# Innoptech/OpenFDCM

Measured on NVIDIA B200. Metric: template_matches_per_sec, higher is better.
Workload: dtype f32

## Files before the change

### include/fdcm_b200.h

```cpp
#ifndef FDCM_B200_H
#define FDCM_B200_H

#include <stdint.h>

#ifdef __cplusplus
extern "C" {
#endif

#define FDCM_B200_ABI_VERSION 3

typedef enum fdcm_status {
    FDCM_OK = 0,
    FDCM_ERR_INVALID = 1,
    FDCM_ERR_CUDA = 2,
    FDCM_ERR_NOMEM = 3,
    FDCM_ERR_OUT_OF_RANGE = 4,
    FDCM_ERR_CAPACITY = 5
} fdcm_status;

typedef enum fdcm_distance { FDCM_L2 = 0, FDCM_L2_SQUARED = 1, FDCM_L1 = 2 } fdcm_distance;

typedef struct fdcm_dt3_params {
    int32_t depth;
    float dt3_coeff;
    float padding;
    int32_t distance;
} fdcm_dt3_params;

typedef struct fdcm_match {
    int32_t tmpl_idx;
    float score;
    float transform[6];
} fdcm_match;

typedef enum fdcm_penalty_kind { FDCM_PENALTY_NONE = 0, FDCM_PENALTY_DEFAULT = 1, FDCM_PENALTY_EXPONENTIAL = 2 } fdcm_penalty_kind;

typedef struct fdcm_search_params {
    int32_t max_tmpl_lines;
    int32_t max_scene_lines;
    int32_t batch_size;
    int32_t penalty_kind;
    float penalty_tau;
    int32_t top_k;
    int32_t tmpl_idx_base;
    int32_t concentric;
    float center_x, center_y, low_radius, high_radius;
} fdcm_search_params;

typedef struct fdcm_dt3_info {
    int32_t depth;
    int32_t width, height;
    int32_t pitch;
    float scene_translation[2];
    int32_t distance;
    int32_t device;
    int32_t n_scene_lines;
    int32_t exact_dt_path;
} fdcm_dt3_info;

typedef struct fdcm_search_stats {
    int64_t n_hypotheses;
    int64_t n_valid;
    int64_t n_evaluations;
    int64_t n_lookups;
} fdcm_search_stats;

typedef struct fdcm_dt3 fdcm_dt3;
typedef struct fdcm_templates fdcm_templates;
typedef struct fdcm_comm fdcm_comm;
typedef struct fdcm_scene_batch fdcm_scene_batch;

const char* fdcm_last_error(void);
int32_t fdcm_abi_version(void);
fdcm_status fdcm_device_count(int32_t* n);
fdcm_status fdcm_set_stream(int32_t device, void* cuda_stream);

fdcm_status fdcm_dt3_build(const float* scene_xyxy, int32_t n_lines, const fdcm_dt3_params* params, int32_t device,
                           int32_t stage, fdcm_dt3** out);
fdcm_status fdcm_dt3_rebuild(fdcm_dt3* map, const float* scene_xyxy, int32_t n_lines);
fdcm_status fdcm_dt3_rebuild_async(fdcm_dt3* map, const float* scene_xyxy, int32_t n_lines);
fdcm_status fdcm_dt3_rerun(fdcm_dt3* map);
fdcm_status fdcm_dt3_rerun_async(fdcm_dt3* map);
fdcm_status fdcm_dt3_retain(fdcm_dt3* map);
fdcm_status fdcm_dt3_release(fdcm_dt3* map);
fdcm_status fdcm_dt3_get_info(const fdcm_dt3* map, fdcm_dt3_info* info);
fdcm_status fdcm_dt3_angles(const fdcm_dt3* map, float* keys);
fdcm_status fdcm_dt3_download_plane(const fdcm_dt3* map, int32_t plane, float* dst);
fdcm_status fdcm_dt3_download_mask(const fdcm_dt3* map, int32_t plane, uint8_t* dst);
fdcm_status fdcm_dt3_scene_bins(const fdcm_dt3* map, int32_t* bins);
fdcm_status fdcm_dt3_device_ptr(const fdcm_dt3* map, void** planes, uint64_t* n_bytes);

fdcm_status fdcm_dt3_minmax_translation(const fdcm_dt3* map, const float* tmpl_xyxy, int32_t n_lines,
                                        const float align_vec[2], float out_min_max[2]);
fdcm_status fdcm_dt3_evaluate(const fdcm_dt3* map, const float* tmpl_lines, const int32_t* tmpl_offsets, int32_t n_tmpl,
                              const float* translations, const int32_t* transl_offsets, float* scores);
fdcm_status fdcm_dt3_classify(const fdcm_dt3* map, const float* lines_xyxy, int32_t n_lines, int32_t* bins);

fdcm_status fdcm_templates_create(const float* tmpl_lines, const int32_t* tmpl_offsets, int32_t n_tmpl, int32_t device,
                                  fdcm_templates** out);
fdcm_status fdcm_templates_release(fdcm_templates* t);
fdcm_status fdcm_templates_lengths(const fdcm_templates* t, float* lengths);

#define FDCM_SCENE_RESIDENT (-1)
fdcm_status fdcm_search(const fdcm_dt3* map, const fdcm_templates* templates, const float* scene_xyxy, int32_t n_scene,
                        const fdcm_search_params* params, fdcm_match* out, int64_t capacity, int64_t* n_out);
#define FDCM_SELECT_MAX_ACROSS 1024
typedef struct fdcm_select_params {
    int32_t max_per_template;
    float radius;
    float max_angle;
    int32_t across_templates;
} fdcm_select_params;
fdcm_status fdcm_search_select(const fdcm_dt3* map, const fdcm_templates* templates, const float* scene_xyxy, int32_t n_scene,
                               const fdcm_search_params* params, const fdcm_select_params* select,
                               fdcm_match* out, int64_t capacity, int64_t* n_out);
fdcm_status fdcm_template_anchors(const float* tmpl_lines, const int32_t* tmpl_offsets, int32_t n_tmpl, float* anchors_xy);

#define FDCM_REFINE_MAX_STEPS 15
typedef struct fdcm_refine_params {
    int32_t levels;
    int32_t rot_steps;
    float rot_step;
    int32_t trans_steps;
    float trans_step;
} fdcm_refine_params;
fdcm_status fdcm_refine_matches(const fdcm_dt3* map, const fdcm_templates* templates, int32_t tmpl_idx_base, int32_t penalty_kind,
                                float penalty_tau, const fdcm_refine_params* refine, const fdcm_match* in, int64_t n,
                                fdcm_match* out);
fdcm_status fdcm_search_refine(const fdcm_dt3* map, const fdcm_templates* templates, const float* scene_xyxy, int32_t n_scene,
                               const fdcm_search_params* params, const fdcm_select_params* select,
                               const fdcm_refine_params* refine, fdcm_match* out, int64_t capacity, int64_t* n_out);
fdcm_status fdcm_refine_poses(const float transform[6], const float anchor[2], const fdcm_refine_params* refine, int32_t level,
                              float* out);

#define FDCM_DENSE_MAX_ROTATIONS 4096
typedef struct fdcm_dense_params {
    int32_t rotations;
    float rot_start;
    float rot_step;
    int32_t stride;
    int32_t cell;
    int32_t roi_on;
    float roi[4];
} fdcm_dense_params;
fdcm_status fdcm_search_dense(const fdcm_dt3* map, const fdcm_templates* templates, const fdcm_dense_params* dense, int32_t penalty_kind,
                              float penalty_tau, int32_t top_k, int32_t tmpl_idx_base, const fdcm_select_params* select,
                              const fdcm_refine_params* refine, fdcm_match* out, int64_t capacity, int64_t* n_out);
fdcm_status fdcm_dense_poses(const fdcm_dense_params* dense, const float anchor[2], const float shift[2], int32_t width, int32_t height,
                             int32_t rotation, float* out, int64_t capacity, int64_t* n_out, int32_t grid_wh[2]);

fdcm_status fdcm_optimize(const fdcm_dt3* map, const float* tmpl_lines, const int32_t* tmpl_offsets, int32_t n_tmpl,
                          const float* alignments, int32_t batch_size, uint8_t* has_value, float* scores,
                          float* translations);
fdcm_status fdcm_search_host(const fdcm_dt3* map, const float* tmpl_lines, const int32_t* tmpl_offsets, int32_t n_tmpl,
                             const float* scene_xyxy, int32_t n_scene, const fdcm_search_params* params,
                             fdcm_match* out, int64_t capacity, int64_t* n_out);
fdcm_status fdcm_search_last_hypotheses(const fdcm_dt3* map, int32_t* out, int64_t capacity, int64_t* n_out);
fdcm_status fdcm_search_last_stats(const fdcm_dt3* map, fdcm_search_stats* stats);

fdcm_status fdcm_default_search(const float* tmpl_xyxy, int32_t n_tmpl_lines, const float* scene_xyxy, int32_t n_scene,
                                int32_t max_tmpl_lines, int32_t max_scene_lines, int32_t* out_pairs, int32_t capacity,
                                int32_t* n_out);

fdcm_status fdcm_concentric_search(const float* tmpl_xyxy, int32_t n_tmpl_lines, const float* scene_xyxy, int32_t n_scene,
                                   int32_t max_tmpl_lines, int32_t max_scene_lines, float center_x, float center_y,
                                   float low_radius, float high_radius, int32_t* out_pairs, int32_t capacity, int32_t* n_out);

fdcm_status fdcm_debug_dt_rows(const uint16_t* g_rows, int32_t n_rows, int32_t n, int32_t literal, int32_t device, float* out);

fdcm_status fdcm_debug_sqrt_check(int32_t device, int64_t* n_mismatches, uint32_t* first_mismatch);

fdcm_status fdcm_orientation_bins(int32_t depth, const float* lines_xyxy, int32_t n_lines, int32_t* bins_atanf,
                                  int32_t* bins_table);

fdcm_status fdcm_penalize(int32_t penalty_kind, float tau, fdcm_match* matches, int64_t n, const float* lengths,
                          int64_t n_lengths);
fdcm_status fdcm_sort_matches(fdcm_match* matches, int64_t n);
fdcm_status fdcm_template_lengths(const float* tmpl_lines, const int32_t* tmpl_offsets, int32_t n_tmpl, float* lengths);

fdcm_status fdcm_scene_batch_create(const fdcm_dt3_params* params, int32_t device, fdcm_scene_batch** out);
fdcm_status fdcm_scene_batch_destroy(fdcm_scene_batch* batch);
fdcm_status fdcm_search_scenes(fdcm_scene_batch* batch, const float* scene_lines, const int32_t* scene_offsets, int32_t n_scenes,
                               const fdcm_templates* templates, const fdcm_search_params* params, fdcm_match* out, int32_t* n_out);
fdcm_status fdcm_search_scenes_select(fdcm_scene_batch* batch, const float* scene_lines, const int32_t* scene_offsets, int32_t n_scenes,
                                      const fdcm_templates* templates, const fdcm_search_params* params,
                                      const fdcm_select_params* select, fdcm_match* out, int32_t* n_out);

#define FDCM_COMM_ID_BYTES 128
fdcm_status fdcm_comm_unique_id(uint8_t id[FDCM_COMM_ID_BYTES]);
fdcm_status fdcm_comm_init(const uint8_t id[FDCM_COMM_ID_BYTES], int32_t rank, int32_t world, int32_t device, fdcm_comm** out);
fdcm_status fdcm_comm_destroy(fdcm_comm* comm);
fdcm_status fdcm_comm_info(const fdcm_comm* comm, int32_t* rank, int32_t* world);
fdcm_status fdcm_comm_shard(int32_t n_items, int32_t rank, int32_t world, int32_t* begin, int32_t* end);
fdcm_status fdcm_comm_search_topk(fdcm_comm* comm, const fdcm_dt3* map, const fdcm_templates* shard, const float* scene_xyxy,
                                  int32_t n_scene, const fdcm_search_params* params, fdcm_match* out, int64_t capacity,
                                  int64_t* n_out);
fdcm_status fdcm_comm_search_select(fdcm_comm* comm, const fdcm_dt3* map, const fdcm_templates* shard, const float* scene_xyxy,
                                    int32_t n_scene, const fdcm_search_params* params, const fdcm_select_params* select,
                                    fdcm_match* out, int64_t capacity, int64_t* n_out);
fdcm_status fdcm_comm_search_host_topk(fdcm_comm* comm, const fdcm_dt3* map, const float* tmpl_lines, const int32_t* tmpl_offsets,
                                       int32_t n_tmpl, const float* scene_xyxy, int32_t n_scene, const fdcm_search_params* params,
                                       fdcm_match* out, int64_t capacity, int64_t* n_out);
fdcm_status fdcm_comm_rebuild_broadcast(fdcm_comm* comm, fdcm_dt3* map, const float* scene_xyxy, int32_t n_lines, int32_t root);
fdcm_status fdcm_set_host_threads(int32_t n);

fdcm_status fdcm_profile_enable(int32_t on);
fdcm_status fdcm_profile_reset(void);
fdcm_status fdcm_profile_get(int32_t index, char* name, int32_t name_cap, double* total_ms, int64_t* launches,
                             double* bytes_per_launch);
fdcm_status fdcm_profile_count(int32_t* n);
int64_t fdcm_kernel_launch_count(void);

#ifdef __cplusplus
}
#endif
#endif
```

### openfdcm_b200/__init__.py

```python
import ctypes as C
import enum
import math

import numpy as np

from . import _lib
from .io import read, write
from ._lib import MATCH_DTYPE, FdcmError, check, lib, ptr

__all__ = [
    "distance", "Dt3CudaParameters", "Dt3Cuda", "build_cuda_featuremap", "ThreadPool", "DefaultSearch", "ConcentricRangeStrategy",
    "BatchOptimize", "DefaultOptimize", "DefaultMatch", "DefaultPenalty", "ExponentialPenalty", "Match",
    "TemplateSet", "SceneBatch", "DistinctMatches", "PoseRefinement", "DenseSearch", "search", "search_topk", "search_dense",
    "refine_matches", "penalize", "get_template_lengths",
    "get_template_anchors", "sort_matches", "evaluate",
    "minmax_translation", "get_feature_size", "establish_search_strategy", "optimize", "read", "write", "FdcmError", "MATCH_DTYPE",
]


class distance(enum.IntEnum):
    L2 = 0
    L2_SQUARED = 1
    L1 = 2


def _records(lines):
    a = np.asarray(lines, dtype=np.float32)
    if a.size == 0:
        return np.zeros((0, 4), np.float32)
    if a.ndim == 1 and a.size == 4:
        a = a.reshape(4, 1)
    if a.ndim != 2 or a.shape[0] != 4:
        raise ValueError(f"expected a (4,N) line array, got shape {a.shape}")
    return np.ascontiguousarray(a.T)


def _pack(templates):
    recs = [_records(t) for t in templates]
    off = np.zeros(len(recs) + 1, np.int32)
    for i, r in enumerate(recs):
        off[i + 1] = off[i] + r.shape[0]
    flat = np.concatenate(recs, axis=0) if recs else np.zeros((0, 4), np.float32)
    return np.ascontiguousarray(flat, np.float32), off


class Dt3CudaParameters:

    def __init__(self, depth=30, dt3Coeff=5.0, padding=2.2, distance=distance.L2, device=0):
        self.depth = int(depth)
        self.dt3_coeff = float(dt3Coeff)
        self.padding = float(padding)
        self.distance = distance
        self.device = int(device)

    def __repr__(self):
        return f"<Dt3CudaParameters: depth={self.depth}, dt3_coeff={self.dt3_coeff}, padding={self.padding}>"


class Dt3Cuda:

    def __init__(self, handle):
        self._h = C.c_void_p(handle)
        self._refresh()

    def _refresh(self):
        info = _lib.Dt3Info()
        check(lib().fdcm_dt3_get_info(self._h, C.byref(info)))
        self.info = info
        self.depth, self.width, self.height, self.pitch = info.depth, info.width, info.height, info.pitch
        self.device = info.device

    def __del__(self):
        h, self._h = getattr(self, "_h", None), None
        if h and lib is not None:
            lib().fdcm_dt3_release(h)

    def __copy__(self):
        check(lib().fdcm_dt3_retain(self._h))
        return Dt3Cuda(self._h.value)

    def get_scene_translation(self):
        return np.array(self.info.scene_translation[:], np.float32)

    def get_feature_size(self):
        return np.array([self.width, self.height], np.uint64)

    def angles(self):
        k = np.zeros(self.depth, np.float32)
        if self.depth:
            check(lib().fdcm_dt3_angles(self._h, ptr(k)))
        return k

    def plane(self, i):
        out = np.zeros((self.height, self.width), np.float32)
        check(lib().fdcm_dt3_download_plane(self._h, int(i), ptr(out)))
        return out

    def mask(self, i):
        out = np.zeros((self.height, self.width), np.uint8)
        check(lib().fdcm_dt3_download_mask(self._h, int(i), ptr(out)))
        return out

    def scene_bins(self):
        b = np.zeros(self.info.n_scene_lines, np.int32)
        if b.size:
            check(lib().fdcm_dt3_scene_bins(self._h, ptr(b)))
        return b

    def classify(self, lines):
        r = _records(lines)
        b = np.zeros(r.shape[0], np.int32)
        check(lib().fdcm_dt3_classify(self._h, ptr(r), r.shape[0], ptr(b)))
        return b

    def get_dt3_map(self):
        return {float(a): self.plane(i) for i, a in enumerate(self.angles())}

    def device_ptr(self):
        p, n = C.c_void_p(0), C.c_uint64(0)
        check(lib().fdcm_dt3_device_ptr(self._h, C.byref(p), C.byref(n)))
        return p.value, n.value

    def rebuild(self, scene, wait=True):
        r = _records(scene)
        check((lib().fdcm_dt3_rebuild if wait else lib().fdcm_dt3_rebuild_async)(self._h, ptr(r), r.shape[0]))
        self._refresh()

    def rerun(self, wait=True):
        check((lib().fdcm_dt3_rerun if wait else lib().fdcm_dt3_rerun_async)(self._h))

    def last_search_stats(self):
        st = _lib.SearchStats()
        check(lib().fdcm_search_last_stats(self._h, C.byref(st)))
        return {"n_hypotheses": st.n_hypotheses, "n_valid": st.n_valid, "n_evaluations": st.n_evaluations,
                "n_lookups": st.n_lookups}

    def last_hypotheses(self):
        n = C.c_int64(0)
        lib().fdcm_search_last_hypotheses(self._h, None, 0, C.byref(n))
        out = np.zeros((n.value, 4), np.int32)
        if n.value:
            check(lib().fdcm_search_last_hypotheses(self._h, ptr(out), n.value, C.byref(n)))
        return out

    def __repr__(self):
        t = self.info.scene_translation
        return f"<Dt3Cuda: scene translation=({t[0]}, {t[1]}), feature size=({self.width}, {self.height})>"


def build_cuda_featuremap(scene, params=None, pool=None, *, stage=0):
    params = params or Dt3CudaParameters()
    p = _lib.Dt3Params(params.depth, params.dt3_coeff, params.padding, int(params.distance))
    r = _records(scene)
    h = C.c_void_p(0)
    check(lib().fdcm_dt3_build(ptr(r), r.shape[0], C.byref(p), params.device, int(stage), C.byref(h)))
    return Dt3Cuda(h.value)


class ThreadPool:

    def __init__(self, num_threads=0):
        self.num_threads = int(num_threads)

    def get_thread_count(self):
        return self.num_threads


class DefaultSearch:

    def __init__(self, max_tmpl_lines, max_scene_lines):
        self.max_tmpl_lines, self.max_scene_lines = int(max_tmpl_lines), int(max_scene_lines)

    def get_max_tmpl_lines(self):
        return self.max_tmpl_lines

    def get_max_scene_lines(self):
        return self.max_scene_lines


class ConcentricRangeStrategy(DefaultSearch):

    def __init__(self, max_tmpl_lines, max_scene_lines, center_position, low_boundary, high_boundary):
        super().__init__(max_tmpl_lines, max_scene_lines)
        c = np.asarray(center_position, np.float32).reshape(2)
        self.center_position = c
        self.low_boundary, self.high_boundary = float(low_boundary), float(high_boundary)

    def get_center_position(self):
        return self.center_position

    def get_low_radius_boundary(self):
        return self.low_boundary

    def get_high_radius_boundary(self):
        return self.high_boundary


class BatchOptimize:

    def __init__(self, batch_size, pool=None, num_threads=None):
        if int(batch_size) < 1:
            raise ValueError("batch_size must be >= 1")
        self.batch_size = int(batch_size)

    def get_batch_size(self):
        return self.batch_size


class DefaultOptimize:
    batch_size = 0

    def __init__(self, pool=None, num_threads=None):
        pass


class DefaultMatch:
    """matchstrategies/defaultmatch.h."""


class DefaultPenalty:
    kind, tau = 1, 0.0


class ExponentialPenalty:
    kind = 2

    def __init__(self, tau):
        self.tau = float(tau)

    def get_tau(self):
        return self.tau


class Match:
    __slots__ = ("tmpl_idx", "score", "transform")

    def __init__(self, tmpl_idx, score, transform):
        self.tmpl_idx = int(tmpl_idx)
        self.score = float(score)
        self.transform = np.asarray(transform, np.float32).reshape(2, 3)

    def __repr__(self):
        return f"<Match tmplIdx={self.tmpl_idx}, score={self.score}, transform=\n{self.transform}>"


def _to_matches(rec):
    return [Match(r["tmpl_idx"], r["score"], r["transform"]) for r in rec]


def _to_records(matches):
    if isinstance(matches, np.ndarray) and matches.dtype == MATCH_DTYPE:
        return np.ascontiguousarray(matches).copy()
    rec = np.zeros(len(matches), MATCH_DTYPE)
    for i, m in enumerate(matches):
        rec[i] = (m.tmpl_idx, m.score, np.asarray(m.transform, np.float32).reshape(6))
    return rec


class TemplateSet:

    def __init__(self, templates, device=0):
        flat, off = _pack(templates)
        self.n_tmpl = len(off) - 1
        self.n_lines = int(off[-1])
        self.max_lines = int(np.diff(off).max()) if self.n_tmpl else 0
        h = C.c_void_p(0)
        check(lib().fdcm_templates_create(ptr(flat), ptr(off), self.n_tmpl, int(device), C.byref(h)))
        self._h = h
        self.device = int(device)

    def __del__(self):
        h, self._h = getattr(self, "_h", None), None
        if h and lib is not None:
            lib().fdcm_templates_release(h)
# ... 276 lines not shown
```

### openfdcm_b200/_lib.py

```python
import ctypes as C
import os

import numpy as np

_HERE = os.path.dirname(os.path.abspath(__file__))
LIB_PATH = os.path.join(_HERE, "libfdcm_b200.so")

FDCM_OK = 0
FDCM_ERR_INVALID, FDCM_ERR_CUDA, FDCM_ERR_NOMEM, FDCM_ERR_OUT_OF_RANGE, FDCM_ERR_CAPACITY = 1, 2, 3, 4, 5
FDCM_SCENE_RESIDENT = -1

MATCH_DTYPE = np.dtype([("tmpl_idx", "<i4"), ("score", "<f4"), ("transform", "<f4", (6,))])
assert MATCH_DTYPE.itemsize == 32


class Dt3Params(C.Structure):
    _fields_ = [("depth", C.c_int32), ("dt3_coeff", C.c_float), ("padding", C.c_float), ("distance", C.c_int32)]


class SearchParams(C.Structure):
    _fields_ = [("max_tmpl_lines", C.c_int32), ("max_scene_lines", C.c_int32), ("batch_size", C.c_int32),
                ("penalty_kind", C.c_int32), ("penalty_tau", C.c_float), ("top_k", C.c_int32),
                ("tmpl_idx_base", C.c_int32), ("concentric", C.c_int32), ("center_x", C.c_float), ("center_y", C.c_float),
                ("low_radius", C.c_float), ("high_radius", C.c_float)]


class SelectParams(C.Structure):
    _fields_ = [("max_per_template", C.c_int32), ("radius", C.c_float), ("max_angle", C.c_float), ("across_templates", C.c_int32)]


class RefineParams(C.Structure):
    _fields_ = [("levels", C.c_int32), ("rot_steps", C.c_int32), ("rot_step", C.c_float), ("trans_steps", C.c_int32),
                ("trans_step", C.c_float)]


class DenseParams(C.Structure):
    _fields_ = [("rotations", C.c_int32), ("rot_start", C.c_float), ("rot_step", C.c_float), ("stride", C.c_int32), ("cell", C.c_int32),
                ("roi_on", C.c_int32), ("roi", C.c_float * 4)]


class Dt3Info(C.Structure):
    _fields_ = [("depth", C.c_int32), ("width", C.c_int32), ("height", C.c_int32), ("pitch", C.c_int32),
                ("scene_translation", C.c_float * 2), ("distance", C.c_int32), ("device", C.c_int32),
                ("n_scene_lines", C.c_int32), ("exact_dt_path", C.c_int32)]


class SearchStats(C.Structure):
    _fields_ = [("n_hypotheses", C.c_int64), ("n_valid", C.c_int64), ("n_evaluations", C.c_int64),
                ("n_lookups", C.c_int64)]


_P = C.c_void_p
SIGNATURES = {
    "fdcm_last_error": (C.c_char_p, []),
    "fdcm_abi_version": (C.c_int32, []),
    "fdcm_device_count": (C.c_int, [C.POINTER(C.c_int32)]),
    "fdcm_set_stream": (C.c_int, [C.c_int32, _P]),
    "fdcm_dt3_build": (C.c_int, [_P, C.c_int32, C.POINTER(Dt3Params), C.c_int32, C.c_int32, C.POINTER(_P)]),
    "fdcm_dt3_rebuild": (C.c_int, [_P, _P, C.c_int32]),
    "fdcm_dt3_rebuild_async": (C.c_int, [_P, _P, C.c_int32]),
    "fdcm_dt3_rerun": (C.c_int, [_P]),
    "fdcm_dt3_rerun_async": (C.c_int, [_P]),
    "fdcm_dt3_retain": (C.c_int, [_P]),
    "fdcm_dt3_release": (C.c_int, [_P]),
    "fdcm_dt3_get_info": (C.c_int, [_P, C.POINTER(Dt3Info)]),
    "fdcm_dt3_angles": (C.c_int, [_P, _P]),
    "fdcm_dt3_download_plane": (C.c_int, [_P, C.c_int32, _P]),
    "fdcm_dt3_download_mask": (C.c_int, [_P, C.c_int32, _P]),
    "fdcm_dt3_scene_bins": (C.c_int, [_P, _P]),
    "fdcm_dt3_device_ptr": (C.c_int, [_P, C.POINTER(_P), C.POINTER(C.c_uint64)]),
    "fdcm_dt3_minmax_translation": (C.c_int, [_P, _P, C.c_int32, _P, _P]),
    "fdcm_dt3_evaluate": (C.c_int, [_P, _P, _P, C.c_int32, _P, _P, _P]),
    "fdcm_dt3_classify": (C.c_int, [_P, _P, C.c_int32, _P]),
    "fdcm_templates_create": (C.c_int, [_P, _P, C.c_int32, C.c_int32, C.POINTER(_P)]),
    "fdcm_templates_release": (C.c_int, [_P]),
    "fdcm_templates_lengths": (C.c_int, [_P, _P]),
    "fdcm_search": (C.c_int, [_P, _P, _P, C.c_int32, C.POINTER(SearchParams), _P, C.c_int64, C.POINTER(C.c_int64)]),
    "fdcm_search_select": (C.c_int, [_P, _P, _P, C.c_int32, C.POINTER(SearchParams), C.POINTER(SelectParams), _P, C.c_int64,
                                     C.POINTER(C.c_int64)]),
    "fdcm_template_anchors": (C.c_int, [_P, _P, C.c_int32, _P]),
    "fdcm_refine_matches": (C.c_int, [_P, _P, C.c_int32, C.c_int32, C.c_float, C.POINTER(RefineParams), _P, C.c_int64, _P]),
    "fdcm_search_refine": (C.c_int, [_P, _P, _P, C.c_int32, C.POINTER(SearchParams), C.POINTER(SelectParams), C.POINTER(RefineParams), _P,
                                     C.c_int64, C.POINTER(C.c_int64)]),
    "fdcm_refine_poses": (C.c_int, [_P, _P, C.POINTER(RefineParams), C.c_int32, _P]),
    "fdcm_search_dense": (C.c_int, [_P, _P, C.POINTER(DenseParams), C.c_int32, C.c_float, C.c_int32, C.c_int32, C.POINTER(SelectParams),
                                    C.POINTER(RefineParams), _P, C.c_int64, C.POINTER(C.c_int64)]),
    "fdcm_dense_poses": (C.c_int, [C.POINTER(DenseParams), _P, _P, C.c_int32, C.c_int32, C.c_int32, _P, C.c_int64, C.POINTER(C.c_int64),
                                   _P]),
    "fdcm_optimize": (C.c_int, [_P, _P, _P, C.c_int32, _P, C.c_int32, _P, _P, _P]),
    "fdcm_search_host": (C.c_int, [_P, _P, _P, C.c_int32, _P, C.c_int32, C.POINTER(SearchParams), _P, C.c_int64,
                                   C.POINTER(C.c_int64)]),
    "fdcm_search_last_hypotheses": (C.c_int, [_P, _P, C.c_int64, C.POINTER(C.c_int64)]),
    "fdcm_search_last_stats": (C.c_int, [_P, C.POINTER(SearchStats)]),
    "fdcm_default_search": (C.c_int, [_P, C.c_int32, _P, C.c_int32, C.c_int32, C.c_int32, _P, C.c_int32,
                                      C.POINTER(C.c_int32)]),
    "fdcm_debug_dt_rows": (C.c_int, [_P, C.c_int32, C.c_int32, C.c_int32, C.c_int32, _P]),
    "fdcm_debug_sqrt_check": (C.c_int, [C.c_int32, C.POINTER(C.c_int64), C.POINTER(C.c_uint32)]),
    "fdcm_concentric_search": (C.c_int, [_P, C.c_int32, _P, C.c_int32, C.c_int32, C.c_int32, C.c_float, C.c_float, C.c_float,
                                         C.c_float, _P, C.c_int32, C.POINTER(C.c_int32)]),
    "fdcm_orientation_bins": (C.c_int, [C.c_int32, _P, C.c_int32, _P, _P]),
    "fdcm_penalize": (C.c_int, [C.c_int32, C.c_float, _P, C.c_int64, _P, C.c_int64]),
    "fdcm_sort_matches": (C.c_int, [_P, C.c_int64]),
    "fdcm_template_lengths": (C.c_int, [_P, _P, C.c_int32, _P]),
    "fdcm_profile_enable": (C.c_int, [C.c_int32]),
    "fdcm_profile_reset": (C.c_int, []),
    "fdcm_profile_get": (C.c_int, [C.c_int32, C.c_char_p, C.c_int32, C.POINTER(C.c_double), C.POINTER(C.c_int64),
                                   C.POINTER(C.c_double)]),
    "fdcm_profile_count": (C.c_int, [C.POINTER(C.c_int32)]),
    "fdcm_kernel_launch_count": (C.c_int64, []),
    "fdcm_comm_unique_id": (C.c_int, [_P]),
    "fdcm_comm_init": (C.c_int, [_P, C.c_int32, C.c_int32, C.c_int32, C.POINTER(_P)]),
    "fdcm_comm_destroy": (C.c_int, [_P]),
    "fdcm_comm_info": (C.c_int, [_P, C.POINTER(C.c_int32), C.POINTER(C.c_int32)]),
    "fdcm_comm_shard": (C.c_int, [C.c_int32, C.c_int32, C.c_int32, C.POINTER(C.c_int32), C.POINTER(C.c_int32)]),
    "fdcm_comm_search_topk": (C.c_int, [_P, _P, _P, _P, C.c_int32, C.POINTER(SearchParams), _P, C.c_int64, C.POINTER(C.c_int64)]),
    "fdcm_comm_search_select": (C.c_int, [_P, _P, _P, _P, C.c_int32, C.POINTER(SearchParams), C.POINTER(SelectParams), _P, C.c_int64,
                                          C.POINTER(C.c_int64)]),
    "fdcm_comm_search_host_topk": (C.c_int, [_P, _P, _P, _P, C.c_int32, _P, C.c_int32, C.POINTER(SearchParams), _P, C.c_int64,
                                             C.POINTER(C.c_int64)]),
    "fdcm_comm_rebuild_broadcast": (C.c_int, [_P, _P, _P, C.c_int32, C.c_int32]),
    "fdcm_set_host_threads": (C.c_int, [C.c_int32]),
    "fdcm_scene_batch_create": (C.c_int, [C.POINTER(Dt3Params), C.c_int32, C.POINTER(_P)]),
    "fdcm_scene_batch_destroy": (C.c_int, [_P]),
    "fdcm_search_scenes": (C.c_int, [_P, _P, _P, C.c_int32, _P, C.POINTER(SearchParams), _P, _P]),
    "fdcm_search_scenes_select": (C.c_int, [_P, _P, _P, C.c_int32, _P, C.POINTER(SearchParams), C.POINTER(SelectParams), _P, _P]),
}


class FdcmError(RuntimeError):
    def __init__(self, status, message):
        super().__init__(f"libfdcm_b200 status {status}: {message}")
        self.status = status


_lib = None


def lib():
    global _lib
    if _lib is None:
        if not os.path.exists(LIB_PATH):
            raise ImportError(f"{LIB_PATH} is missing: build it with `make -C openfdcm_b200/csrc` "
                              "(or __graft_entry__.build()); there is no CPU fallback")
        l = C.CDLL(LIB_PATH)
        for name, (res, args) in SIGNATURES.items():
            fn = getattr(l, name)
            fn.restype = res
            fn.argtypes = args
        _lib = l
    return _lib


def check(status):
    if status != FDCM_OK:
        msg = lib().fdcm_last_error()
        raise FdcmError(status, msg.decode() if msg else "")


def ptr(a):
    return a.ctypes.data_as(C.c_void_p) if a is not None else None
```

### openfdcm_b200/csrc/common.cuh

```cuda
#pragma once
#include <cuda_runtime.h>
#include <cfloat>
#include <cstdint>

namespace fdcm {

constexpr int kMaxDepthDev = 64;
constexpr int kMaxPropSteps = 4 * kMaxDepthDev;
constexpr uint16_t kNoEdge16 = 0xFFFFu;

struct MapDims {
    int D, H, W, pitch;
    int wwords;
    size_t plane_elems;
};

struct PropParams {
    int n_steps;
    float w[kMaxPropSteps];
    uint8_t c1[kMaxPropSteps];
    uint8_t c2[kMaxPropSteps];
};

struct IntegralParams {
    float rx[kMaxDepthDev], ry[kMaxDepthDev];
    int mode[kMaxDepthDev];
};

struct SlopeTableDev {
    int n_thr;
    int nan_bin;
    float thr[kMaxDepthDev + 8];
    uint8_t piece_bin[kMaxDepthDev + 9];
};

__device__ __forceinline__ long long round_to_ll(float x) { return (long long)roundf(x); }

__device__ __forceinline__ float signed_pick_dev(float x, bool negate) { return x == 0.f ? 0.f : (negate ? -x : x); }

__device__ __forceinline__ void rasterize_vector_dev(float vx, float vy, float& ox, float& oy) {
    const float t = vy / vx;
    if (t >= -1.0f && t < 1.0f) {
        const bool c = vx < 0;
        ox = c ? -1.f : 1.f;
        oy = signed_pick_dev(t, c);
        return;
    }
    const bool c = vy < 0;
    const float inv = 1.f / t;
    ox = signed_pick_dev(inv, c);
    oy = c ? -1.f : 1.f;
}

__device__ __forceinline__ int bin_of_slope_dev(const SlopeTableDev& t, float slope) {
    if (slope != slope) return t.nan_bin;
    int lo = 0, hi = t.n_thr;
    while (lo < hi) {
        const int mid = (lo + hi) >> 1;
        if (t.thr[mid] <= slope) lo = mid + 1; else hi = mid;
    }
    return t.piece_bin[lo];
}

}
```

### openfdcm_b200/csrc/dt3_kernels.cu

```cuda
#include <cstdlib>

#include "common.cuh"
#include "kernels.h"

namespace fdcm {

__device__ __forceinline__ int outcode_dev(float x, float y, float xmax, float ymax) {
    int code = 0;
    if (x < 0.f) code |= 1; else if (x > xmax) code |= 2;
    if (y < 0.f) code |= 4; else if (y > ymax) code |= 8;
    return code;
}

__device__ bool clip_line_dev(float& x1, float& y1, float& x2, float& y2, float xmax, float ymax) {
    int c1 = outcode_dev(x1, y1, xmax, ymax);
    int c2 = outcode_dev(x2, y2, xmax, ymax);
    for (int it = 0; it < 16; ++it) {
        if (c1 == 0 && c2 == 0) return true;
        if (c1 & c2) return false;
        if (c1 != 0) {
            if (c1 & 8)      { x1 = x1 + (x2 - x1) * (ymax - y1) / (y2 - y1); y1 = ymax; }
            else if (c1 & 4) { x1 = x1 + (x2 - x1) * (0.f - y1) / (y2 - y1); y1 = 0.f; }
            else if (c1 & 2) { y1 = y1 + (y2 - y1) * (xmax - x1) / (x2 - x1); x1 = xmax; }
            else if (c1 & 1) { y1 = y1 + (y2 - y1) * (0.f - x1) / (x2 - x1); x1 = 0.f; }
// ... 51 lines not shown
    if (rel_eq_zero(rx)) {
        const int size = (int)(lvy / ry) + 1;
        const LinSpacedDev ly(size, p1y, p2y);
        const long long x = round_to_ll(p1x);
        for (int i = lane; i < size; i += 32) set_edge(mask, dm, plane, x, round_to_ll(ly.at(i)));
        return;
    }
    if (rel_eq_zero(ry)) {
        const int size = (int)(lvx / rx) + 1;
        const LinSpacedDev lx(size, p1x, p2x);
        const long long y = round_to_ll(p1y);
        for (int i = lane; i < size; i += 32) set_edge(mask, dm, plane, round_to_ll(lx.at(i)), y);
        return;
    }
    const float a = lvx / rx, b = lvy / ry;
    const int size = (int)((a < b) ? b : a) + 1;
    const LinSpacedDev lx(size, p1x, p2x), ly(size, p1y, p2y);
    for (int i = lane; i < size; i += 32) set_edge(mask, dm, plane, round_to_ll(lx.at(i)), round_to_ll(ly.at(i)));
}


struct EnvEntry { int v; float z; };
enum { kSrcPlane = 0, kSrcMask = 1, kSrcG16 = 2 };

template <int kSrc>
__global__ void __launch_bounds__(128) dt_pass_literal_kernel(const void* __restrict__ src, float* planes, MapDims dm,
                                                              EnvEntry* stack, int n, int n_lines, size_t elem_stride,
                                                              size_t line_stride) {
    const int l = blockIdx.x * blockDim.x + threadIdx.x;
    const int d = blockIdx.y;
    if (l >= n_lines) return;
    const size_t base = (size_t)d * dm.plane_elems + (size_t)l * line_stride;
    float* out = planes + base;
    const uint16_t* gin = kSrc == kSrcG16 ? reinterpret_cast<const uint16_t*>(src) + base : nullptr;
    const uint32_t* mrow = kSrc == kSrcMask ? reinterpret_cast<const uint32_t*>(src) + (size_t)d * dm.H * dm.wwords + (l >> 5) : nullptr;
    const uint32_t mbit = 1u << (l & 31);
    EnvEntry* st = stack + base;
    auto F = [&](int q) -> float {
        if (kSrc == kSrcG16) {
            const unsigned gv = gin[(size_t)q * elem_stride];
            return gv == kNoEdge16 ? FLT_MAX : (float)(gv * gv);
        }
        if (kSrc == kSrcMask) return (mrow[(size_t)q * dm.wwords] & mbit) ? 0.f : FLT_MAX;
        return out[(size_t)q * elem_stride];
    };
    int k = 0, vk = 0;
    float fvk = F(0), zk = -INFINITY;
    st[0] = EnvEntry{0, -INFINITY};
    for (int q = 1; q < n; ++q) {
        const float fq = F(q);
        const float sqq = (float)((long long)q * q);
        while (true) {
            const float s = (fq + sqq - fvk - (float)((long long)vk * vk)) / (float)(2LL * q - 2LL * vk);
            if (s > zk) {
                ++k;
                st[(size_t)k * elem_stride] = EnvEntry{q, s};
                vk = q; fvk = fq; zk = s;
                break;
            }
            --k;
            const EnvEntry e = st[(size_t)k * elem_stride];
            vk = e.v; zk = e.z; fvk = F(vk);
        }
    }
    int k2 = 0, v = 0;
    float znext = (k >= 1) ? st[elem_stride].z : INFINITY;
    for (int q = 0; q < n; ++q) {
        while (znext < (float)q) {
            ++k2;
            v = st[(size_t)k2 * elem_stride].v;
            znext = (k2 + 1 <= k) ? st[(size_t)(k2 + 1) * elem_stride].z : INFINITY;
        }
        const long long dq = (long long)q - v;
        const float srcv = (kSrc != kSrcPlane && v >= q) ? F(v) : out[(size_t)v * elem_stride];
        out[(size_t)q * elem_stride] = srcv + (float)(dq * dq);
    }
}

__global__ void __launch_bounds__(256) transpose_square_kernel(float* __restrict__ planes, MapDims dm, int ntiles) {
    __shared__ float A[32][33], B[32][33];
    int t = blockIdx.x, ti = 0;
    while (t >= ntiles - ti) { t -= ntiles - ti; ++ti; }
    const int tj = ti + t;
    float* P = planes + (size_t)blockIdx.y * dm.plane_elems;
    const int lx = threadIdx.x & 31, ly = threadIdx.x >> 5;
    const int n = dm.W;
    for (int r = ly; r < 32; r += 8) {
        const int ya = ti * 32 + r, xa = tj * 32 + lx;
        const int yb = tj * 32 + r, xb = ti * 32 + lx;
        A[r][lx] = (ya < n && xa < n) ? P[(size_t)ya * dm.pitch + xa] : 0.f;
        B[r][lx] = (yb < n && xb < n) ? P[(size_t)yb * dm.pitch + xb] : 0.f;
    }
    __syncthreads();
    for (int r = ly; r < 32; r += 8) {
        const int ya = ti * 32 + r, xa = tj * 32 + lx;
        const int yb = tj * 32 + r, xb = ti * 32 + lx;
        if (ya < n && xa < n) P[(size_t)ya * dm.pitch + xa] = B[lx][r];
        if (ti != tj && yb < n && xb < n) P[(size_t)yb * dm.pitch + xb] = A[lx][r];
    }
}

__global__ void __launch_bounds__(256) sqrt_kernel(float* __restrict__ planes, size_t total) {
    const size_t i = (size_t)blockIdx.x * blockDim.x + threadIdx.x;
    if (i < total) planes[i] = sqrtf(planes[i]);
}

template <int D>
__global__ void __launch_bounds__(128) propagate_kernel(float* __restrict__ planes, MapDims dm,
                                                        const __grid_constant__ PropParams pp, int sqrt_first) {
    const size_t i = (size_t)blockIdx.x * blockDim.x + threadIdx.x;
    if (i >= dm.plane_elems || (int)(i % dm.pitch) >= dm.W) return;
    float v[D];
#pragma unroll
    for (int d = 0; d < D; ++d) v[d] = planes[(size_t)d * dm.plane_elems + i];
    if (sqrt_first) {
#pragma unroll
        for (int d = 0; d < D; ++d) v[d] = sqrtf(v[d]);
    }
    constexpr int fwd = (3 * D + 1) / 2;
    constexpr int bwd = D + (3 * D) / 2;
#pragma unroll
    for (int c = 0; c < fwd; ++c) {
        const int c1 = (D + ((c - 1) % D)) % D;
        const int c2 = c % D;
        v[c2] = fminf(v[c2], v[c1] + pp.w[c]);
    }
#pragma unroll
    for (int j = 0; j < bwd; ++j) {
        const int c = D - j;
        const int c1 = (D + ((c + 1) % D)) % D;
        const int c2 = (D + (c % D)) % D;
        v[c2] = fminf(v[c2], v[c1] + pp.w[fwd + j]);
    }
#pragma unroll
    for (int d = 0; d < D; ++d) planes[(size_t)d * dm.plane_elems + i] = v[d];
}

__global__ void __launch_bounds__(128) propagate_generic_kernel(float* __restrict__ planes, MapDims dm,
                                                                const __grid_constant__ PropParams pp, int sqrt_first) {
    const size_t i = (size_t)blockIdx.x * blockDim.x + threadIdx.x;
    if (i >= dm.plane_elems || (int)(i % dm.pitch) >= dm.W) return;
    float v[kMaxDepthDev];
    for (int d = 0; d < dm.D; ++d) {
        const float x = planes[(size_t)d * dm.plane_elems + i];
        v[d] = sqrt_first ? sqrtf(x) : x;
    }
    for (int s = 0; s < pp.n_steps; ++s) {
        const int c1 = pp.c1[s], c2 = pp.c2[s];
        v[c2] = fminf(v[c2], v[c1] + pp.w[s]);
    }
    for (int d = 0; d < dm.D; ++d) planes[(size_t)d * dm.plane_elems + i] = v[d];
}

static inline unsigned cdiv(size_t a, size_t b) { return (unsigned)((a + b - 1) / b); }

void launch_raster(const float* d_lines, const int32_t* d_bins, int n_lines, const MapDims& dm, uint32_t* d_mask,
                   cudaStream_t s) {
    if (n_lines <= 0) return;
    raster_kernel<<<cdiv((size_t)n_lines * 32, 256), 256, 0, s>>>(reinterpret_cast<const float4*>(d_lines), d_bins, n_lines,
                                                                   dm, d_mask);
}

void launch_dt_pass_literal(int src_kind, bool along_rows, const void* d_src, float* d_planes, const MapDims& dm, void* d_stack,
                            cudaStream_t s) {
    const int n = along_rows ? dm.W : dm.H;
    const int n_lines = along_rows ? dm.H : dm.W;
    const size_t es = along_rows ? 1 : (size_t)dm.pitch;
    const size_t ls = along_rows ? (size_t)dm.pitch : 1;
    dim3 grid(cdiv(n_lines, 128), dm.D);
    if (src_kind == kSrcG16)
        dt_pass_literal_kernel<kSrcG16><<<grid, 128, 0, s>>>(d_src, d_planes, dm, (EnvEntry*)d_stack, n, n_lines, es, ls);
    else if (src_kind == kSrcMask)
        dt_pass_literal_kernel<kSrcMask><<<grid, 128, 0, s>>>(d_src, d_planes, dm, (EnvEntry*)d_stack, n, n_lines, es, ls);
    else
        dt_pass_literal_kernel<kSrcPlane><<<grid, 128, 0, s>>>(d_src, d_planes, dm, (EnvEntry*)d_stack, n, n_lines, es, ls);
}

void launch_transpose_square(float* d_planes, const MapDims& dm, cudaStream_t s) {
    const int nt = (dm.W + 31) / 32;
    dim3 grid((unsigned)((size_t)nt * (nt + 1) / 2), dm.D);
    transpose_square_kernel<<<grid, 256, 0, s>>>(d_planes, dm, nt);
}

void launch_sqrt(float* d_planes, const MapDims& dm, cudaStream_t s) {
    const size_t total = (size_t)dm.D * dm.plane_elems;
    sqrt_kernel<<<cdiv(total, 256), 256, 0, s>>>(d_planes, total);
}

void launch_propagate(float* d_planes, const MapDims& dm, const PropParams& pp, bool sqrt_first, cudaStream_t s) {
    const unsigned grid = cdiv(dm.plane_elems, 128);
    switch (dm.D) {
        case 30: propagate_kernel<30><<<grid, 128, 0, s>>>(d_planes, dm, pp, sqrt_first ? 1 : 0); break;
        case 4: propagate_kernel<4><<<grid, 128, 0, s>>>(d_planes, dm, pp, sqrt_first ? 1 : 0); break;
        default: propagate_generic_kernel<<<grid, 128, 0, s>>>(d_planes, dm, pp, sqrt_first ? 1 : 0); break;
    }
}

}
```

### openfdcm_b200/csrc/fdcm_api.cu

```cuda
#include <algorithm>
#include <atomic>
#include <condition_variable>
#include <functional>
#include <cmath>
#include <cstdio>
#include <cstdlib>
#include <cstring>
#include <map>
#include <mutex>
#include <string>
#include <thread>
#include <vector>

#include "host_math.hpp"
#include "kernels.h"

using namespace fdcm;

static thread_local std::string g_last_error;

static fdcm_status fail(fdcm_status st, const std::string& msg) {
    g_last_error = msg;
    return st;
}
// ... 63 lines not shown
        CUDA_TRY(cudaStreamCreateWithPriority(&ns, cudaStreamNonBlocking, prio_hi));
        o = g_aux_streams.emplace(device, ns).first;
    }
    *s = o->second;
    return FDCM_OK;
}

extern "C" fdcm_status fdcm_set_stream(int32_t device, void* cuda_stream) {
    std::lock_guard<std::mutex> lk(g_mutex);
    if (cuda_stream) g_user_streams[device] = (cudaStream_t)cuda_stream;
    else g_user_streams.erase(device);
    return FDCM_OK;
}

struct ProfEntry { double total_ms = 0; long long launches = 0; double bytes = 0; };
struct ProfPending { const char* name; cudaEvent_t a, b; double bytes; int device; };
static bool g_prof_on = false;
static std::vector<std::string> g_prof_order;
static std::map<std::string, ProfEntry> g_prof;
static std::vector<ProfPending> g_prof_pending;
static std::map<int, std::vector<cudaEvent_t>> g_prof_events;
static cudaEvent_t prof_event_get(int device) {
    auto& pool = g_prof_events[device];
    cudaEvent_t e = nullptr;
    if (!pool.empty()) {
        e = pool.back();
        pool.pop_back();
    } else {
        cudaEventCreate(&e);
    }
    return e;
}
static void prof_event_put(int device, cudaEvent_t e) { g_prof_events[device].push_back(e); }

struct KernelScope {
    cudaStream_t s;
    bool on;
    ProfPending p;
    KernelScope(const char* name, double bytes, cudaStream_t stream, int n_kernels = 1) : s(stream), on(g_prof_on) {
        g_launches.fetch_add(n_kernels, std::memory_order_relaxed);
        if (on) {
            p.name = name;
            p.bytes = bytes;
            p.device = 0;
            cudaGetDevice(&p.device);
            {
                std::lock_guard<std::mutex> lk(g_mutex);
                p.a = prof_event_get(p.device);
                p.b = prof_event_get(p.device);
            }
            cudaEventRecord(p.a, s);
        }
    }
    ~KernelScope() {
        if (on) {
            cudaEventRecord(p.b, s);
            std::lock_guard<std::mutex> lk(g_mutex);
            g_prof_pending.push_back(p);
        }
    }
};

extern "C" fdcm_status fdcm_profile_enable(int32_t on) { g_prof_on = on != 0; return FDCM_OK; }
extern "C" fdcm_status fdcm_profile_reset(void) {
    std::lock_guard<std::mutex> lk(g_mutex);
    g_prof.clear();
    g_prof_order.clear();
    return FDCM_OK;
}
static void prof_resolve() {
    std::lock_guard<std::mutex> lk(g_mutex);
    std::vector<ProfPending> keep;
    bool not_ready = false;
    for (auto& p : g_prof_pending) {
        if (cudaEventQuery(p.b) != cudaSuccess) { keep.push_back(p); not_ready = true; continue; }
        float ms = 0.f;
        if (cudaEventElapsedTime(&ms, p.a, p.b) == cudaSuccess) {
            if (!g_prof.count(p.name)) g_prof_order.push_back(p.name);
            auto& e = g_prof[p.name];
            e.total_ms += ms;
            e.launches += 1;
            e.bytes = p.bytes;
        }
        prof_event_put(p.device, p.a);
        prof_event_put(p.device, p.b);
    }
    g_prof_pending.swap(keep);
    if (not_ready && cudaPeekAtLastError() == cudaErrorNotReady) cudaGetLastError();
}

extern "C" fdcm_status fdcm_profile_count(int32_t* n) {
    if (!n) return fail(FDCM_ERR_INVALID, "n is null");
    prof_resolve();
    std::lock_guard<std::mutex> lk(g_mutex);
    *n = (int32_t)g_prof_order.size();
    return FDCM_OK;
}
extern "C" fdcm_status fdcm_profile_get(int32_t index, char* name, int32_t name_cap, double* total_ms, int64_t* launches,
                                        double* bytes_per_launch) {
    std::lock_guard<std::mutex> lk(g_mutex);
    if (index < 0 || index >= (int32_t)g_prof_order.size()) return fail(FDCM_ERR_INVALID, "profile index out of range");
    const std::string& nm = g_prof_order[index];
    const ProfEntry& e = g_prof[nm];
    if (name && name_cap > 0) {
        std::strncpy(name, nm.c_str(), name_cap - 1);
        name[name_cap - 1] = 0;
    }
    if (total_ms) *total_ms = e.total_ms;
    if (launches) *launches = e.launches;
    if (bytes_per_launch) *bytes_per_launch = e.bytes;
    return FDCM_OK;
}
extern "C" int64_t fdcm_kernel_launch_count(void) { return g_launches.load(); }

struct DevBuf {
    void* p = nullptr;
    size_t cap = 0;
    cudaError_t reserve(size_t bytes) {
        if (bytes <= cap) return cudaSuccess;
        if (p) cudaFree(p);
        p = nullptr;
        cap = 0;
        cudaError_t e = cudaMalloc(&p, bytes);
        if (e == cudaSuccess) cap = bytes;
        return e;
    }
    void release() {
        if (p) cudaFree(p);
        p = nullptr;
        cap = 0;
    }
    template <class T> T* as() const { return reinterpret_cast<T*>(p); }
};

struct fdcm_dt3 {
    std::atomic<int> refs{1};
    fdcm_dt3_params params{};
    int device = 0;
    int stage = 0;
    MapDims dm{};
    float shift[2] = {0.f, 0.f};
    bool exact = true;
    int col_lo = 0, col_hi = 0;
    int row_lo = 0, row_hi = 0;
    int tables_depth = -1;
    float tables_coeff = 0.f;
    int n_lines = 0;
    std::vector<float> keys;
    std::vector<int32_t> scene_bins;
    SlopeTable table;
    SlopeTableDev table_dev{};
    PropParams prop{};
    IntegralParams integ{};
    DevBuf planes, mask, stack, lines, bins, band_info, band_spill, integ_items;
    IntegralPlanDev integ_plan{};
    int plan_W = -1, plan_H = -1, plan_D = -1, plan_pitch = -1;
    const void* plan_planes = nullptr;
    int plan_tables_depth = -1;
    int n_sms = 148;
    cudaEvent_t ev_fork = nullptr, ev_join = nullptr;
    cudaEvent_t ev_written = nullptr;
    bool band_path = false, band_l1 = false;
    mutable std::mutex search_mutex;
    mutable DevBuf s_scene, s_sorted_len, s_sorted_idx, s_hyp_off, s_rec, s_valid, s_hyp, s_counters, s_topk_score, s_topk_idx,
        s_topk_out, s_topk_n, s_keys, s_keys2, s_idx, s_perm, s_sort_tmp;
    mutable DevBuf s_sel_keys, s_sel_keys2, s_sel_vals, s_sel_vals2, s_sel_surv, s_sel_acc, s_sel_tmp;
    mutable DevBuf s_ref_state, s_ref_keys, s_ref_io;
    mutable DevBuf s_denom;
    mutable uint64_t denom_set = 0;
    mutable int denom_kind = -1;
    mutable float denom_tau = 0.f;
    mutable DevBuf s_dense_keys, s_dense_rot;
    mutable float s_scene_min[2] = {0.f, 0.f}, s_scene_max[2] = {0.f, 0.f};
    mutable std::mutex host_tset_mutex;
    mutable fdcm_templates* host_tset = nullptr;
    mutable int32_t s_scene_n = 0;
    mutable int32_t s_sorted_n = 0;
    mutable bool s_resident_is_build = false;
    mutable bool s_filter_on = false;
    mutable float s_filter[4] = {0.f, 0.f, 0.f, 0.f};
    std::vector<float> h_build_scene;
    mutable int64_t last_n_hyp = 0;
    mutable fdcm_search_stats last_stats{};
    mutable void* h_scene_stage = nullptr;
    mutable size_t h_scene_stage_cap = 0;
    mutable cudaEvent_t scene_stage_ev = nullptr;
    mutable void* h_pinned = nullptr;
    mutable size_t h_pinned_cap = 0;

    ~fdcm_dt3() {
        cudaSetDevice(device);
        for (DevBuf* b : {&planes, &mask, &stack, &lines, &bins, &band_info, &band_spill, &integ_items, &s_scene, &s_sorted_len, &s_sorted_idx, &s_hyp_off, &s_rec,
                          &s_valid, &s_hyp, &s_counters, &s_topk_score, &s_topk_idx, &s_topk_out, &s_topk_n, &s_keys, &s_keys2, &s_idx,
                          &s_perm, &s_sort_tmp, &s_sel_keys, &s_sel_keys2, &s_sel_vals, &s_sel_vals2, &s_sel_surv, &s_sel_acc,
                          &s_sel_tmp, &s_ref_state, &s_ref_keys, &s_ref_io, &s_denom, &s_dense_keys, &s_dense_rot})
            b->release();
        if (h_pinned) cudaFreeHost(h_pinned);
        if (ev_fork) cudaEventDestroy(ev_fork);
        if (ev_join) cudaEventDestroy(ev_join);
        if (ev_written) cudaEventDestroy(ev_written);
        if (h_scene_stage) cudaFreeHost(h_scene_stage);
        if (scene_stage_ev) cudaEventDestroy(scene_stage_ev);
        destroy_host_tset();
    }
    void destroy_host_tset();
};

constexpr int64_t kMaxSide = 16384;

struct SceneFilter { bool on; float cx, cy, lo, hi; };

static fdcm_status map_wait(const fdcm_dt3* m, cudaStream_t s) {
    if (m->ev_written) CUDA_TRY(cudaStreamWaitEvent(s, m->ev_written, 0));
    return FDCM_OK;
}
static fdcm_status map_written(fdcm_dt3* m, cudaStream_t s) {
    if (!m->ev_written) CUDA_TRY(cudaEventCreateWithFlags(&m->ev_written, cudaEventDisableTiming));
    CUDA_TRY(cudaEventRecord(m->ev_written, s));
    return FDCM_OK;
}

static std::vector<int32_t> filter_in_range(const float* lines, int32_t n, const SceneFilter& f) {
    std::vector<int32_t> idx;
    for (int32_t i = 0; i < n; ++i) {
        const float* l = lines + 4 * (size_t)i;
        const float mx = (l[2] + l[0]) / 2 - f.cx, my = (l[3] + l[1]) / 2 - f.cy;
        const float rad = std::sqrt(mx * mx + my * my);
        if (rad > (f.lo - std::numeric_limits<float>::epsilon()) && rad < f.hi) idx.push_back(i);
    }
    return idx;
}

static fdcm_status upload_search_scene(const fdcm_dt3* m, const float* scene, int32_t n_scene, const SceneFilter& flt, cudaStream_t s) {
    std::vector<int32_t> subset;
    if (flt.on) subset = filter_in_range(scene, n_scene, flt);
    else {
        subset.resize((size_t)n_scene);
        for (int i = 0; i < n_scene; ++i) subset[(size_t)i] = i;
    }
    const int ns = (int)subset.size();
    std::vector<float> slen((size_t)ns);
    for (int i = 0; i < ns; ++i) slen[(size_t)i] = line_length(scene + 4 * (size_t)subset[(size_t)i]);
    const std::vector<long> sidx = argsort_desc(slen.data(), ns);
    std::vector<float> sorted_len((size_t)ns);
    std::vector<int32_t> sorted_idx((size_t)ns);
    for (int i = 0; i < ns; ++i) {
        sorted_len[(size_t)i] = slen[(size_t)sidx[(size_t)i]];
        sorted_idx[(size_t)i] = subset[(size_t)sidx[(size_t)i]];
    }
    m->s_scene_n = 0;
    m->s_sorted_n = 0;
    m->s_scene_min[0] = m->s_scene_max[0] = scene[0];
    m->s_scene_min[1] = m->s_scene_max[1] = scene[1];
    for (int64_t i = 0; i < 2 * (int64_t)n_scene; ++i)
        for (int a = 0; a < 2; ++a) {
            const float v = scene[2 * i + a];
            if (v < m->s_scene_min[a]) m->s_scene_min[a] = v;
            if (v > m->s_scene_max[a]) m->s_scene_max[a] = v;
        }
    CUDA_TRY(m->s_scene.reserve((size_t)n_scene * 16));
    CUDA_TRY(m->s_sorted_len.reserve(std::max<size_t>(4, (size_t)ns * 4)));
    CUDA_TRY(m->s_sorted_idx.reserve(std::max<size_t>(4, (size_t)ns * 4)));
    const size_t need = (size_t)n_scene * 16 + (size_t)ns * 8;
    if (!m->scene_stage_ev) CUDA_TRY(cudaEventCreateWithFlags(&m->scene_stage_ev, cudaEventDisableTiming));
    else CUDA_TRY(cudaEventSynchronize(m->scene_stage_ev));
    if (m->h_scene_stage_cap < need) {
        if (m->h_scene_stage) cudaFreeHost(m->h_scene_stage);
        m->h_scene_stage = nullptr;
        m->h_scene_stage_cap = 0;
        CUDA_TRY(cudaMallocHost(&m->h_scene_stage, need));
        m->h_scene_stage_cap = need;
    }
    unsigned char* st = static_cast<unsigned char*>(m->h_scene_stage);
    std::memcpy(st, scene, (size_t)n_scene * 16);
    CUDA_TRY(cudaMemcpyAsync(m->s_scene.p, st, (size_t)n_scene * 16, cudaMemcpyHostToDevice, s));
    if (ns) {
        std::memcpy(st + (size_t)n_scene * 16, sorted_len.data(), (size_t)ns * 4);
        std::memcpy(st + (size_t)n_scene * 16 + (size_t)ns * 4, sorted_idx.data(), (size_t)ns * 4);
        CUDA_TRY(cudaMemcpyAsync(m->s_sorted_len.p, st + (size_t)n_scene * 16, (size_t)ns * 4, cudaMemcpyHostToDevice, s));
        CUDA_TRY(cudaMemcpyAsync(m->s_sorted_idx.p, st + (size_t)n_scene * 16 + (size_t)ns * 4, (size_t)ns * 4, cudaMemcpyHostToDevice, s));
    }
    CUDA_TRY(cudaEventRecord(m->scene_stage_ev, s));
    m->s_scene_n = n_scene;
    m->s_sorted_n = ns;
    m->s_filter_on = flt.on;
    m->s_filter[0] = flt.cx; m->s_filter[1] = flt.cy; m->s_filter[2] = flt.lo; m->s_filter[3] = flt.hi;
    return FDCM_OK;
}

static fdcm_status run_build_kernels(fdcm_dt3* m, cudaStream_t s);

namespace fdcm {
bool encode_planes_map(CUtensorMap* out, const void* planes, int W, int H, int D, int pitch, int bx, int by, int bz) {
    typedef CUresult (*EncodeFn)(CUtensorMap*, CUtensorMapDataType, cuuint32_t, void*, const cuuint64_t*, const cuuint64_t*,
                                 const cuuint32_t*, const cuuint32_t*, CUtensorMapInterleave, CUtensorMapSwizzle,
                                 CUtensorMapL2promotion, CUtensorMapFloatOOBfill);
    static EncodeFn fn = [] {
        void* p = nullptr;
        cudaDriverEntryPointQueryResult q;
        if (cudaGetDriverEntryPoint("cuTensorMapEncodeTiled", &p, cudaEnableDefault, &q) != cudaSuccess || q != cudaDriverEntryPointSuccess)
            p = nullptr;
        return (EncodeFn)p;
    }();
    if (!fn) return false;
    const cuuint64_t dims[3] = {(cuuint64_t)W, (cuuint64_t)H, (cuuint64_t)D};
    const cuuint64_t strides[2] = {(cuuint64_t)pitch * 4, (cuuint64_t)pitch * 4 * (cuuint64_t)H};
    const cuuint32_t box[3] = {(cuuint32_t)bx, (cuuint32_t)by, (cuuint32_t)bz};
    const cuuint32_t estr[3] = {1, 1, 1};
    return fn(out, CU_TENSOR_MAP_DATA_TYPE_FLOAT32, 3, const_cast<void*>(planes), dims, strides, box, estr, CU_TENSOR_MAP_INTERLEAVE_NONE,
              CU_TENSOR_MAP_SWIZZLE_NONE, CU_TENSOR_MAP_L2_PROMOTION_L2_128B, CU_TENSOR_MAP_FLOAT_OOB_FILL_NONE) == CUDA_SUCCESS;
}
}

static fdcm_status build_integral_plan(fdcm_dt3* m, cudaStream_t s) {
    const MapDims& dm = m->dm;
    const bool same = m->plan_W == dm.W && m->plan_H == dm.H && m->plan_D == dm.D && m->plan_pitch == dm.pitch &&
                      m->plan_planes == m->planes.p && m->plan_tables_depth == m->tables_depth;
    if (same) return FDCM_OK;
    m->plan_W = -1;
    const int rlen = std::max(dm.W, dm.H);
    std::vector<int32_t> rtab((size_t)dm.D * rlen);
    struct Item { int work; int4 it; };
    std::vector<Item> items;
    const int CW = integral_strip_chains(), RB = integral_tile_steps();
    for (int d = 0; d < dm.D; ++d) {
        const int mode = m->integ.mode[d];
        const float r = mode == 1 ? m->integ.ry[d] : m->integ.rx[d];
        int32_t* R = rtab.data() + (size_t)d * rlen;
        for (int i = 0; i < rlen; ++i) R[i] = (int32_t)(long long)std::round((float)i * r);
        if (mode != 1 && mode != 2) continue;
        const int n_major = mode == 1 ? dm.W : dm.H, n_minor = mode == 1 ? dm.H : dm.W;
        const int Rend = R[n_major - 1];
        const int cmin = Rend > 0 ? -Rend : 0, cmax = (Rend < 0 ? -Rend : 0) + n_minor - 1;
        const int nblk = (n_major + RB - 1) / RB;
        for (int c0 = cmin; c0 <= cmax; c0 += CW) {
            int b_lo = nblk, b_hi = 0;
            for (int b = 0; b < nblk; ++b) {
                const int i0 = b * RB, i1 = std::min(n_major, i0 + RB);
                const int rlo = std::min(R[i0], R[i1 - 1]), rhi = std::max(R[i0], R[i1 - 1]);
                if (c0 + CW - 1 + rhi >= 0 && c0 + rlo <= n_minor - 1) { b_lo = std::min(b_lo, b); b_hi = std::max(b_hi, b + 1); }
            }
            if (b_lo < b_hi) items.push_back(Item{b_hi - b_lo, make_int4(d, c0, b_lo, b_hi)});
        }
    }
    std::stable_sort(items.begin(), items.end(), [](const Item& a, const Item& b) { return a.work > b.work; });
    std::vector<int4> flat(items.size());
    for (size_t i = 0; i < items.size(); ++i) flat[i] = items[i].it;
    CUDA_TRY(m->integ_items.reserve(std::max<size_t>(16, flat.size() * sizeof(int4))));
    if (!flat.empty()) CUDA_TRY(cudaMemcpyAsync(m->integ_items.p, flat.data(), flat.size() * sizeof(int4), cudaMemcpyHostToDevice, s));
    CUDA_TRY(cudaStreamSynchronize(s));
    IntegralPlanDev& pl = m->integ_plan;
    pl.items4 = m->integ_items.as<int4>();
    pl.n_items = (int)flat.size();
    if (!integral_tma_encode(m->planes.p, dm, &pl.map_y, &pl.map_x))
        return fail(FDCM_ERR_CUDA, "cuTensorMapEncodeTiled failed for the feature-map planes");
    int sms = 0;
    if (cudaDeviceGetAttribute(&sms, cudaDevAttrMultiProcessorCount, m->device) == cudaSuccess && sms > 0) m->n_sms = sms;
    m->plan_W = dm.W; m->plan_H = dm.H; m->plan_D = dm.D; m->plan_pitch = dm.pitch;
    m->plan_planes = m->planes.p;
    m->plan_tables_depth = m->tables_depth;
    return FDCM_OK;
}

static fdcm_status prepare_and_upload(fdcm_dt3* m, const float* scene, int32_t n_lines, cudaStream_t s) {
    m->n_lines = n_lines;
    m->scene_bins.clear();
    if (n_lines == 0) {
        m->s_scene_n = 0;
        m->s_sorted_n = 0;
        m->h_build_scene.clear();
        m->dm = MapDims{0, 0, 0, 0, 0, 0};
        m->shift[0] = m->shift[1] = 0.f;
        m->keys.clear();
        return FDCM_OK;
    }
    int64_t size[2];
    scene_centered_translation(scene, n_lines, m->params.padding, m->shift, size);
    if (size[0] <= 0 || size[0] > kMaxSide || size[1] != size[0])
        return fail(FDCM_ERR_INVALID, "feature size out of the supported range (1.." + std::to_string(kMaxSide) + "): " + std::to_string(size[0]));
    m->keys = angle_keys(m->params.depth);
    const int D = (int)m->keys.size();
    MapDims dm;
    dm.D = D;
    dm.W = (int)size[0];
    dm.H = (int)size[1];
    dm.pitch = (dm.W + 31) / 32 * 32;
    dm.wwords = dm.pitch / 32;
    dm.plane_elems = (size_t)dm.H * dm.pitch;
    m->dm = dm;
    m->exact = 2.0 * (double)(dm.W - 1) * (double)(dm.W - 1) < 16777216.0;

    std::vector<float> ts((size_t)4 * n_lines);
    m->scene_bins.resize(n_lines);
    for (int64_t i = 0; i < 2 * (int64_t)n_lines; ++i) {
        ts[2 * i] = scene[2 * i] + m->shift[0];
        ts[2 * i + 1] = scene[2 * i + 1] + m->shift[1];
    }
    for (int i = 0; i < n_lines; ++i) m->scene_bins[i] = bin_of_line(m->keys.data(), D, &ts[4 * (size_t)i]);
    {
        float mnx = ts[0], mxx = ts[0], mny = ts[1], mxy = ts[1];
        for (int64_t i = 0; i < 2 * (int64_t)n_lines; ++i) {
            mnx = std::min(mnx, ts[2 * i]);
            mxx = std::max(mxx, ts[2 * i]);
            mny = std::min(mny, ts[2 * i + 1]);
            mxy = std::max(mxy, ts[2 * i + 1]);
        }
        {
            const double lo = std::floor((double)mny) - 1.0, hi = std::ceil((double)mxy) + 1.0;
            m->row_lo = (lo < 0.0 || !(lo == lo)) ? 0 : (lo > dm.H - 1 ? dm.H - 1 : (int)lo);
            m->row_hi = (!(hi == hi) || hi > dm.H - 1) ? dm.H - 1 : (hi < 0.0 ? 0 : (int)hi);
        }
        const double lo = std::floor((double)mnx) - 1.0, hi = std::ceil((double)mxx) + 1.0;
        m->col_lo = (lo < 0.0 || !(lo == lo)) ? 0 : (lo > dm.W - 1 ? dm.W - 1 : (int)lo);
        m->col_hi = (!(hi == hi) || hi > dm.W - 1) ? dm.W - 1 : (hi < 0.0 ? 0 : (int)hi);
    }

    if (m->tables_depth != D || m->tables_coeff != m->params.dt3_coeff) {
    m->table = build_slope_table(m->keys.data(), D);
    if ((int)m->table.thr.size() > kMaxDepthDev + 8) return fail(FDCM_ERR_INVALID, "slope table too large");
    m->table_dev.n_thr = (int)m->table.thr.size();
    m->table_dev.nan_bin = m->table.nan_bin;
    for (size_t i = 0; i < m->table.thr.size(); ++i) m->table_dev.thr[i] = m->table.thr[i];
    for (size_t i = 0; i < m->table.piece_bin.size(); ++i) m->table_dev.piece_bin[i] = (uint8_t)m->table.piece_bin[i];
    const std::vector<PropStep> steps = propagation_schedule(m->keys, m->params.dt3_coeff);
    m->prop.n_steps = (int)steps.size();
    for (size_t i = 0; i < steps.size(); ++i) {
        m->prop.w[i] = steps[i].w;
        m->prop.c1[i] = (uint8_t)steps[i].c1;
        m->prop.c2[i] = (uint8_t)steps[i].c2;
    }
    for (int d = 0; d < D; ++d) {
        const IntegralDir id = integral_direction(m->keys[d]);
        m->integ.rx[d] = id.rx;
        m->integ.ry[d] = id.ry;
        m->integ.mode[d] = id.mode;
    }
    m->tables_depth = D;
    m->tables_coeff = m->params.dt3_coeff;
    }

    const size_t n_px = (size_t)D * dm.plane_elems;
    CUDA_TRY(m->planes.reserve(n_px * sizeof(float)));
    CUDA_TRY(m->mask.reserve((size_t)D * dm.H * dm.wwords * sizeof(uint32_t) + 256));
    if (dt_band_smem_bytes(dm) > 200 * 1024) return fail(FDCM_ERR_INVALID, "feature size too large for the band kernels");
    const bool band_path = m->exact && m->params.distance != FDCM_L1;
    const bool band_l1 = m->params.distance == FDCM_L1;
    m->band_path = band_path;
    m->band_l1 = band_l1;
    if (band_path || band_l1) CUDA_TRY(m->band_info.reserve(dt_band_info_bytes(dm)));
    if (band_path) CUDA_TRY(m->band_spill.reserve(dt_band_spill_bytes(dm, m->col_hi - m->col_lo + 1)));
    if (m->params.distance != FDCM_L1 && !band_path) CUDA_TRY(m->stack.reserve(n_px * 8));
    CUDA_TRY(m->lines.reserve((size_t)n_lines * 16));
    CUDA_TRY(m->bins.reserve((size_t)n_lines * 4));
    CUDA_TRY(cudaMemcpyAsync(m->lines.p, ts.data(), (size_t)n_lines * 16, cudaMemcpyHostToDevice, s));
    CUDA_TRY(cudaMemcpyAsync(m->bins.p, m->scene_bins.data(), (size_t)n_lines * 4, cudaMemcpyHostToDevice, s));
    return build_integral_plan(m, s);
}

static fdcm_status upload_build_scene(fdcm_dt3* m, const float* scene, int32_t n_lines, cudaStream_t s) {
    if (n_lines == 0) return FDCM_OK;
    m->h_build_scene.assign(scene, scene + 4 * (size_t)n_lines);
    m->s_resident_is_build = true;
    return upload_search_scene(m, scene, n_lines, SceneFilter{false, 0, 0, 0, 0}, s);
}

static fdcm_status run_build_kernels(fdcm_dt3* m, cudaStream_t s) {
    if (m->n_lines == 0) return FDCM_OK;
    const MapDims& dm = m->dm;
    const double N = (double)dm.D * dm.H * dm.W * 4.0;
    const size_t mask_bytes = (size_t)dm.D * dm.H * dm.wwords * sizeof(uint32_t);
    {
        KernelScope k("mask_clear", (double)mask_bytes, s, 0);
        CUDA_TRY(cudaMemsetAsync(m->mask.p, 0, mask_bytes + 256, s));
    }
    {
        KernelScope k("raster", 0.0, s);
        launch_raster(m->lines.as<float>(), m->bins.as<int32_t>(), m->n_lines, dm, m->mask.as<uint32_t>(), s);
    }
    const int dist = m->params.distance;
    bool fused_propagate = false;
    if (m->band_l1) {
        {
            KernelScope k("dt_col_band", (double)mask_bytes + (double)dt_band_info_bytes(dm), s);
            launch_dt_col_band(m->mask.as<uint32_t>(), dm, m->band_info.p, s);
        }
        fused_propagate = m->stage != 1 && dt_fill_propagate_supported(dm);
        if (fused_propagate) {
            KernelScope k("dt_l1_propagate", (double)dt_band_info_bytes(dm) + N, s);
            launch_dt_l1_propagate(m->band_info.p, m->planes.as<float>(), dm, m->prop, s);
        } else {
            KernelScope k("dt_row_l1_band", (double)dt_band_info_bytes(dm) + N, s);
            launch_dt_row_l1_band(m->band_info.p, m->planes.as<float>(), dm, s);
        }
    } else if (m->band_path) {
        {
            KernelScope k("dt_col_band", (double)mask_bytes + (double)dt_band_info_bytes(dm), s);
            launch_dt_col_band(m->mask.as<uint32_t>(), dm, m->band_info.p, s);
        }
        fused_propagate = m->stage != 1 && dt_fill_propagate_supported(dm);
        int ys0 = 0, ys1 = dm.H;
        dt_band_scene_rows(dm, m->row_lo, m->row_hi, &ys0, &ys1);
        const bool split = fused_propagate && (ys0 > 0 || ys1 < dm.H) && ys1 > ys0;
        if (split) {
            cudaStream_t sa;
            if (fdcm_status st = get_aux_stream(m->device, &sa)) return st;
            if (!m->ev_fork) CUDA_TRY(cudaEventCreateWithFlags(&m->ev_fork, cudaEventDisableTiming));
            if (!m->ev_join) CUDA_TRY(cudaEventCreateWithFlags(&m->ev_join, cudaEventDisableTiming));
            CUDA_TRY(cudaEventRecord(m->ev_fork, s));
            CUDA_TRY(cudaStreamWaitEvent(sa, m->ev_fork, 0));
            {
                KernelScope k("dt_row_envelope", (double)dt_band_info_bytes(dm), sa);
                launch_dt_row_envelope(m->band_info.p, nullptr, dm, m->band_spill.p, m->col_lo, m->col_hi, m->row_lo, m->row_hi, 1, sa);
            }
            {
                KernelScope k("dt_resolve", 2.0 * (double)dt_band_info_bytes(dm), sa);
                launch_dt_resolve(dm, m->band_spill.p, m->col_lo, m->col_hi, ys0, ys1, 0, 0, sa);
            }
            {
                KernelScope k("dt_fill_propagate", N * (double)(ys1 - ys0) / dm.H, sa);
                launch_dt_fill_propagate(m->planes.as<float>(), dm, m->band_spill.p, m->col_lo, m->col_hi, m->prop, dist == FDCM_L2, ys0, ys1, 0,
                                         0, sa);
            }
            CUDA_TRY(cudaEventRecord(m->ev_join, sa));
            {
                KernelScope k("dt_row_envelope_far", (double)dt_band_info_bytes(dm), s);
                launch_dt_row_envelope(m->band_info.p, nullptr, dm, m->band_spill.p, m->col_lo, m->col_hi, m->row_lo, m->row_hi, 2, s);
            }
            {
                KernelScope k("dt_resolve_far", 2.0 * (double)dt_band_info_bytes(dm), s);
                launch_dt_resolve(dm, m->band_spill.p, m->col_lo, m->col_hi, 0, ys0, ys1, dm.H, s);
            }
            {
                KernelScope k("dt_fill_propagate_far", N * (double)(dm.H - (ys1 - ys0)) / dm.H, s);
                launch_dt_fill_propagate(m->planes.as<float>(), dm, m->band_spill.p, m->col_lo, m->col_hi, m->prop, dist == FDCM_L2, 0, ys0, ys1,
                                         dm.H, s);
            }
            CUDA_TRY(cudaStreamWaitEvent(s, m->ev_join, 0));
        } else {
            {
                KernelScope k("dt_row_envelope", (double)dt_band_info_bytes(dm), s);
                launch_dt_row_envelope(m->band_info.p, nullptr, dm, m->band_spill.p, m->col_lo, m->col_hi, m->row_lo, m->row_hi, 0, s);
            }
            if (fused_propagate) {
                {
                    KernelScope k("dt_resolve", 2.0 * (double)dt_band_info_bytes(dm), s);
                    launch_dt_resolve(dm, m->band_spill.p, m->col_lo, m->col_hi, 0, dm.H, 0, 0, s);
                }
                KernelScope k("dt_fill_propagate", N, s);
                launch_dt_fill_propagate(m->planes.as<float>(), dm, m->band_spill.p, m->col_lo, m->col_hi, m->prop, dist == FDCM_L2, 0, dm.H, 0, 0,
                                         s);
            } else {
                KernelScope k("dt_row_fill", N, s);
                launch_dt_row_fill(m->planes.as<float>(), dm, m->band_spill.p, m->col_lo, m->col_hi, s);
            }
        }
    } else {
        {
            KernelScope k("dt_col_literal", (double)mask_bytes + N, s);
            launch_dt_pass_literal(1, false, m->mask.p, m->planes.as<float>(), dm, m->stack.p, s);
        }
        {
            KernelScope k("transpose", 2 * N, s);
            launch_transpose_square(m->planes.as<float>(), dm, s);
        }
        {
            KernelScope k("dt_row_literal", 2 * N, s);
            launch_dt_pass_literal(0, false, nullptr, m->planes.as<float>(), dm, m->stack.p, s);
        }
        {
            KernelScope k("transpose", 2 * N, s);
            launch_transpose_square(m->planes.as<float>(), dm, s);
        }
    }
    const bool need_sqrt = dist == FDCM_L2;
    if (m->stage == 1) {
        if (need_sqrt) {
            KernelScope k("sqrt", 2 * N, s);
            launch_sqrt(m->planes.as<float>(), dm, s);
        }
    } else {
        if (!fused_propagate) {
            KernelScope k("propagate", 2 * N, s);
            launch_propagate(m->planes.as<float>(), dm, m->prop, need_sqrt, s);
        }
        if (m->stage == 0) {
            KernelScope k("integral", 2 * N, s, 1);
            IntegralPlanDev pl = m->integ_plan;
            pl.counter = reinterpret_cast<int*>(m->mask.as<unsigned char>() + mask_bytes);
            launch_integral_tma(m->planes.as<float>(), dm, m->integ, pl, m->n_sms, s);
        }
    }
    CUDA_TRY(cudaGetLastError());
    return FDCM_OK;
}

static fdcm_status validate_params(const fdcm_dt3_params* p) {
    if (!p) return fail(FDCM_ERR_INVALID, "params is null");
    if (p->depth < 1 || p->depth > kMaxDepth) return fail(FDCM_ERR_INVALID, "depth must be in 1..64");
    if (p->distance < 0 || p->distance > 2) return fail(FDCM_ERR_INVALID, "unknown distance");
    return FDCM_OK;
}

extern "C" fdcm_status fdcm_dt3_build(const float* scene_xyxy, int32_t n_lines, const fdcm_dt3_params* params, int32_t device,
                                      int32_t stage, fdcm_dt3** out) {
    if (!out) return fail(FDCM_ERR_INVALID, "out is null");
    *out = nullptr;
    if (fdcm_status st = validate_params(params)) return st;
    if (n_lines < 0 || (n_lines > 0 && !scene_xyxy)) return fail(FDCM_ERR_INVALID, "bad scene");
    if (stage < 0 || stage > 2) return fail(FDCM_ERR_INVALID, "bad stage");
    CUDA_TRY(cudaSetDevice(device));
    cudaStream_t s;
    if (fdcm_status st = get_stream(device, &s)) return st;
    fdcm_dt3* m = new (std::nothrow) fdcm_dt3();
    if (!m) return fail(FDCM_ERR_NOMEM, "host allocation failed");
    m->params = *params;
    m->device = device;
    m->stage = stage;
    fdcm_status st = prepare_and_upload(m, scene_xyxy, n_lines, s);
    if (st == FDCM_OK) st = run_build_kernels(m, s);
    if (st == FDCM_OK) st = upload_build_scene(m, scene_xyxy, n_lines, s);
    if (st == FDCM_OK) st = map_written(m, s);
    if (st == FDCM_OK) {
        cudaError_t e = cudaStreamSynchronize(s);
        if (e != cudaSuccess) st = fail(FDCM_ERR_CUDA, std::string("build: ") + cudaGetErrorString(e));
    }
    prof_resolve();
    if (st != FDCM_OK) {
        delete m;
        return st;
    }
    *out = m;
    return FDCM_OK;
}

static void invalidate_map(fdcm_dt3* m) {
    m->n_lines = 0;
    m->scene_bins.clear();
    m->keys.clear();
    m->dm = MapDims{0, 0, 0, 0, 0, 0};
    m->shift[0] = m->shift[1] = 0.f;
    m->s_scene_n = 0;
    m->s_sorted_n = 0;
    m->s_resident_is_build = false;
    m->h_build_scene.clear();
    m->last_n_hyp = 0;
}

static fdcm_status rebuild_impl(fdcm_dt3* m, const float* scene_xyxy, int32_t n_lines, bool wait) {
    if (!m) return fail(FDCM_ERR_INVALID, "map is null");
    if (n_lines < 0 || (n_lines > 0 && !scene_xyxy)) return fail(FDCM_ERR_INVALID, "bad scene");
    CUDA_TRY(cudaSetDevice(m->device));
    cudaStream_t s;
    if (fdcm_status st = get_stream(m->device, &s)) return st;
    std::lock_guard<std::mutex> lk(m->search_mutex);
    fdcm_status st = map_wait(m, s);
    if (st == FDCM_OK) st = prepare_and_upload(m, scene_xyxy, n_lines, s);
    if (st == FDCM_OK) st = run_build_kernels(m, s);
    if (st == FDCM_OK) st = upload_build_scene(m, scene_xyxy, n_lines, s);
    if (st == FDCM_OK) st = map_written(m, s);
    if (st != FDCM_OK) {
        const std::string msg = g_last_error;
        cudaStreamSynchronize(s);
        invalidate_map(m);
        g_last_error = msg;
    }
    if (st == FDCM_OK && wait) {
        cudaError_t e = cudaStreamSynchronize(s);
        if (e != cudaSuccess) st = fail(FDCM_ERR_CUDA, std::string("rebuild: ") + cudaGetErrorString(e));
        prof_resolve();
    }
    return st;
}

extern "C" fdcm_status fdcm_dt3_rebuild(fdcm_dt3* m, const float* scene_xyxy, int32_t n_lines) {
    return rebuild_impl(m, scene_xyxy, n_lines, true);
}

extern "C" fdcm_status fdcm_dt3_rebuild_async(fdcm_dt3* m, const float* scene_xyxy, int32_t n_lines) {
    return rebuild_impl(m, scene_xyxy, n_lines, false);
}

extern "C" fdcm_status fdcm_dt3_rerun(fdcm_dt3* m) {
    if (!m) return fail(FDCM_ERR_INVALID, "map is null");
    CUDA_TRY(cudaSetDevice(m->device));
    cudaStream_t s;
    if (fdcm_status st = get_stream(m->device, &s)) return st;
    std::lock_guard<std::mutex> lk(m->search_mutex);
    fdcm_status st = map_wait(m, s);
    if (st == FDCM_OK) st = run_build_kernels(m, s);
    if (st == FDCM_OK) st = map_written(m, s);
    if (st == FDCM_OK) {
        cudaError_t e = cudaStreamSynchronize(s);
        if (e != cudaSuccess) st = fail(FDCM_ERR_CUDA, std::string("rerun: ") + cudaGetErrorString(e));
    }
    prof_resolve();
    return st;
}

extern "C" fdcm_status fdcm_dt3_rerun_async(fdcm_dt3* m) {
    if (!m) return fail(FDCM_ERR_INVALID, "map is null");
    CUDA_TRY(cudaSetDevice(m->device));
    cudaStream_t s;
    if (fdcm_status st = get_stream(m->device, &s)) return st;
    std::lock_guard<std::mutex> lk(m->search_mutex);
    if (fdcm_status st = map_wait(m, s)) return st;
    if (fdcm_status st = run_build_kernels(m, s)) return st;
    return map_written(m, s);
}

extern "C" fdcm_status fdcm_dt3_retain(fdcm_dt3* m) {
    if (!m) return fail(FDCM_ERR_INVALID, "map is null");
    m->refs.fetch_add(1);
    return FDCM_OK;
}

extern "C" fdcm_status fdcm_dt3_release(fdcm_dt3* m) {
    if (!m) return FDCM_OK;
    if (m->refs.fetch_sub(1) == 1) delete m;
    return FDCM_OK;
}

extern "C" fdcm_status fdcm_dt3_get_info(const fdcm_dt3* m, fdcm_dt3_info* info) {
    if (!m || !info) return fail(FDCM_ERR_INVALID, "null argument");
    info->depth = m->dm.D;
    info->width = m->dm.W;
    info->height = m->dm.H;
    info->pitch = m->dm.pitch;
    info->scene_translation[0] = m->shift[0];
    info->scene_translation[1] = m->shift[1];
    info->distance = m->params.distance;
    info->device = m->device;
    info->n_scene_lines = m->n_lines;
    info->exact_dt_path = m->exact ? 1 : 0;
    return FDCM_OK;
}

extern "C" fdcm_status fdcm_dt3_angles(const fdcm_dt3* m, float* keys) {
    if (!m || !keys) return fail(FDCM_ERR_INVALID, "null argument");
    std::memcpy(keys, m->keys.data(), m->keys.size() * sizeof(float));
    return FDCM_OK;
}

extern "C" fdcm_status fdcm_dt3_download_plane(const fdcm_dt3* m, int32_t plane, float* dst) {
    if (!m || !dst) return fail(FDCM_ERR_INVALID, "null argument");
    if (plane < 0 || plane >= m->dm.D) return fail(FDCM_ERR_INVALID, "plane out of range");
    CUDA_TRY(cudaSetDevice(m->device));
    cudaStream_t s;
    if (fdcm_status st = get_stream(m->device, &s)) return st;
    std::lock_guard<std::mutex> lk(m->search_mutex);
    if (fdcm_status st = map_wait(m, s)) return st;
    const float* src = m->planes.as<float>() + (size_t)plane * m->dm.plane_elems;
    CUDA_TRY(cudaMemcpy2DAsync(dst, (size_t)m->dm.W * 4, src, (size_t)m->dm.pitch * 4, (size_t)m->dm.W * 4, m->dm.H,
                               cudaMemcpyDeviceToHost, s));
    CUDA_TRY(cudaStreamSynchronize(s));
    return FDCM_OK;
}

extern "C" fdcm_status fdcm_dt3_download_mask(const fdcm_dt3* m, int32_t plane, uint8_t* dst) {
    if (!m || !dst) return fail(FDCM_ERR_INVALID, "null argument");
    if (plane < 0 || plane >= m->dm.D) return fail(FDCM_ERR_INVALID, "plane out of range");
    CUDA_TRY(cudaSetDevice(m->device));
    cudaStream_t s;
    if (fdcm_status st = get_stream(m->device, &s)) return st;
    std::lock_guard<std::mutex> lk(m->search_mutex);
    if (fdcm_status st = map_wait(m, s)) return st;
    std::vector<uint32_t> w((size_t)m->dm.H * m->dm.wwords);
    CUDA_TRY(cudaMemcpyAsync(w.data(), m->mask.as<uint32_t>() + (size_t)plane * m->dm.H * m->dm.wwords, w.size() * 4,
                             cudaMemcpyDeviceToHost, s));
    CUDA_TRY(cudaStreamSynchronize(s));
    for (int y = 0; y < m->dm.H; ++y)
        for (int x = 0; x < m->dm.W; ++x)
            dst[(size_t)y * m->dm.W + x] = (w[(size_t)y * m->dm.wwords + (x >> 5)] >> (x & 31)) & 1u;
    return FDCM_OK;
}

extern "C" fdcm_status fdcm_dt3_scene_bins(const fdcm_dt3* m, int32_t* bins) {
    if (!m || !bins) return fail(FDCM_ERR_INVALID, "null argument");
    std::memcpy(bins, m->scene_bins.data(), m->scene_bins.size() * sizeof(int32_t));
    return FDCM_OK;
}

extern "C" fdcm_status fdcm_dt3_device_ptr(const fdcm_dt3* m, void** planes, uint64_t* n_bytes) {
    if (!m || !planes) return fail(FDCM_ERR_INVALID, "null argument");
    *planes = m->planes.p;
    if (n_bytes) *n_bytes = (uint64_t)m->dm.D * m->dm.plane_elems * 4;
    return FDCM_OK;
}

extern "C" fdcm_status fdcm_dt3_minmax_translation(const fdcm_dt3* m, const float* tmpl, int32_t n_lines, const float align_vec[2],
                                                   float out[2]) {
    if (!m || !align_vec || !out || (n_lines > 0 && !tmpl)) return fail(FDCM_ERR_INVALID, "null argument");
    const int64_t fs[2] = {m->dm.W, m->dm.H};
    minmax_translation(tmpl, n_lines, align_vec, fs, m->shift, out);
    return FDCM_OK;
}

static MapView map_view(const fdcm_dt3* m) {
    MapView v;
    v.planes = m->planes.as<float>();
    v.dm = m->dm;
    v.shift_x = m->shift[0];
    v.shift_y = m->shift[1];
    return v;
}

extern "C" fdcm_status fdcm_dt3_evaluate(const fdcm_dt3* m, const float* tmpl_lines, const int32_t* tmpl_offsets, int32_t n_tmpl,
                                         const float* translations, const int32_t* transl_offsets, float* scores) {
    if (!m || !tmpl_offsets || !transl_offsets) return fail(FDCM_ERR_INVALID, "null argument");
    if (n_tmpl <= 0) return FDCM_OK;
    const int64_t n_lines = tmpl_offsets[n_tmpl], n_scores = transl_offsets[n_tmpl];
    if (n_scores <= 0) return FDCM_OK;
    if (!scores || !translations || (n_lines > 0 && !tmpl_lines)) return fail(FDCM_ERR_INVALID, "null argument");
    if (m->dm.D == 0) return fail(FDCM_ERR_INVALID, "evaluate on an empty feature map");
    CUDA_TRY(cudaSetDevice(m->device));
    cudaStream_t s;
    if (fdcm_status st = get_stream(m->device, &s)) return st;
    std::lock_guard<std::mutex> lk(m->search_mutex);
    if (fdcm_status st = map_wait(m, s)) return st;
    std::vector<int32_t> owner((size_t)n_scores);
    for (int t = 0; t < n_tmpl; ++t)
        for (int i = transl_offsets[t]; i < transl_offsets[t + 1]; ++i) owner[i] = t;
    DevBuf dl, doff, dtr, down, dsc;
    auto cleanup = [&]() { for (DevBuf* b : {&dl, &doff, &dtr, &down, &dsc}) b->release(); };
    cudaError_t e = cudaSuccess;
    if (e == cudaSuccess) e = dl.reserve(std::max<size_t>(16, (size_t)n_lines * 16));
    if (e == cudaSuccess) e = doff.reserve((size_t)(n_tmpl + 1) * 4);
    if (e == cudaSuccess) e = dtr.reserve((size_t)n_scores * 8);
    if (e == cudaSuccess) e = down.reserve((size_t)n_scores * 4);
    if (e == cudaSuccess) e = dsc.reserve((size_t)n_scores * 4);
    if (e == cudaSuccess && n_lines) e = cudaMemcpyAsync(dl.p, tmpl_lines, (size_t)n_lines * 16, cudaMemcpyHostToDevice, s);
    if (e == cudaSuccess) e = cudaMemcpyAsync(doff.p, tmpl_offsets, (size_t)(n_tmpl + 1) * 4, cudaMemcpyHostToDevice, s);
    if (e == cudaSuccess) e = cudaMemcpyAsync(dtr.p, translations, (size_t)n_scores * 8, cudaMemcpyHostToDevice, s);
    if (e == cudaSuccess) e = cudaMemcpyAsync(down.p, owner.data(), (size_t)n_scores * 4, cudaMemcpyHostToDevice, s);
    if (e == cudaSuccess) {
        KernelScope k("evaluate", 0.0, s);
        launch_evaluate(map_view(m), m->table_dev, dl.as<float4>(), doff.as<int32_t>(), dtr.as<float2>(), nullptr, down.as<int32_t>(),
                        n_scores, dsc.as<float>(), s);
    }
    if (e == cudaSuccess) e = cudaGetLastError();
    if (e == cudaSuccess) e = cudaMemcpyAsync(scores, dsc.p, (size_t)n_scores * 4, cudaMemcpyDeviceToHost, s);
    if (e == cudaSuccess) e = cudaStreamSynchronize(s);
    prof_resolve();
    cleanup();
    if (e != cudaSuccess) return fail(FDCM_ERR_CUDA, std::string("evaluate: ") + cudaGetErrorString(e));
    return FDCM_OK;
}

extern "C" fdcm_status fdcm_dt3_classify(const fdcm_dt3* m, const float* lines, int32_t n, int32_t* bins) {
    if (!m || (n > 0 && (!lines || !bins))) return fail(FDCM_ERR_INVALID, "null argument");
    if (n <= 0) return FDCM_OK;
    if (m->dm.D == 0) return fail(FDCM_ERR_INVALID, "classify on an empty feature map");
    CUDA_TRY(cudaSetDevice(m->device));
    cudaStream_t s;
    if (fdcm_status st = get_stream(m->device, &s)) return st;
    std::lock_guard<std::mutex> lk(m->search_mutex);
    if (fdcm_status st = map_wait(m, s)) return st;
    DevBuf dl, db;
    cudaError_t e = dl.reserve((size_t)n * 16);
    if (e == cudaSuccess) e = db.reserve((size_t)n * 4);
    if (e == cudaSuccess) e = cudaMemcpyAsync(dl.p, lines, (size_t)n * 16, cudaMemcpyHostToDevice, s);
    if (e == cudaSuccess) {
        KernelScope k("classify", 0.0, s);
        launch_classify(m->table_dev, dl.as<float4>(), n, db.as<int32_t>(), s);
    }
    if (e == cudaSuccess) e = cudaGetLastError();
    if (e == cudaSuccess) e = cudaMemcpyAsync(bins, db.p, (size_t)n * 4, cudaMemcpyDeviceToHost, s);
    if (e == cudaSuccess) e = cudaStreamSynchronize(s);
    prof_resolve();
    dl.release();
    db.release();
    if (e != cudaSuccess) return fail(FDCM_ERR_CUDA, std::string("classify: ") + cudaGetErrorString(e));
    return FDCM_OK;
}

template <class T>
struct PinnedVec {
    T* p = nullptr;
    size_t cap = 0;
    cudaError_t resize(size_t n) {
        if (n <= cap) return cudaSuccess;
        if (p) cudaFreeHost(p);
        p = nullptr;
        cap = 0;
        const size_t want = n + n / 4 + 64;
        cudaError_t e = cudaMallocHost(reinterpret_cast<void**>(&p), want * sizeof(T));
        if (e == cudaSuccess) cap = want;
        return e;
    }
    T* data() { return p; }
    ~PinnedVec() { if (p) cudaFreeHost(p); }
};

struct fdcm_templates {
    int device = 0;
    int32_t n_tmpl = 0;
    int32_t max_lines = 0;
    int64_t n_lines = 0;
    std::vector<int32_t> offsets;
    std::vector<float> lengths;
    PinnedVec<float> h_line_len;
    PinnedVec<int32_t> h_argsort;
    PinnedVec<float> h_anchors;
    DevBuf lines, offs, argsort, line_len, anchors;
    uint64_t load_id = 0;
    std::mutex mu;
    cudaEvent_t ready = nullptr;
    std::atomic<bool> upload_pending{false};
    void* h_stage = nullptr;
    size_t h_stage_cap = 0;
    cudaError_t stage_reserve(size_t bytes) {
        if (bytes <= h_stage_cap) return cudaSuccess;
        if (h_stage) cudaFreeHost(h_stage);
        h_stage = nullptr;
        h_stage_cap = 0;
        cudaError_t e = cudaMallocHost(&h_stage, bytes);
        if (e == cudaSuccess) h_stage_cap = bytes;
        return e;
    }
    ~fdcm_templates() {
        cudaSetDevice(device);
        if (ready) cudaEventDestroy(ready);
        if (h_stage) cudaFreeHost(h_stage);
        for (DevBuf* b : {&lines, &offs, &argsort, &line_len, &anchors}) b->release();
    }
};

class HostPool {
    std::vector<std::thread> workers_;
    std::mutex mu_;
    std::condition_variable cv_, done_cv_;
    std::function<void(int, int)> job_;
    int n_items_ = 0, chunk_ = 1, generation_ = 0, pending_ = 0;
    std::atomic<int> next_{0};
    bool stop_ = false;

    void run() {
        int seen = 0;
        for (;;) {
            std::function<void(int, int)> job;
            int n, chunk;
            {
                std::unique_lock<std::mutex> lk(mu_);
                cv_.wait(lk, [&] { return stop_ || generation_ != seen; });
                if (stop_) return;
                seen = generation_;
                job = job_;
                n = n_items_;
                chunk = chunk_;
            }
            for (;;) {
                const int b = next_.fetch_add(chunk);
                if (b >= n) break;
// ... 843 lines not shown
    if (fdcm_status st = check_dense(dense)) return st;
    if (penalty_kind < 0 || penalty_kind > 2) return fail(FDCM_ERR_INVALID, "bad penalty kind");
    if (top_k < 1) return fail(FDCM_ERR_INVALID, "dense search: top_k must be >= 1");
    if (sel)
        if (fdcm_status st = check_select(sel, top_k, false)) return st;
    if (sel && sel->max_per_template == 0 && !(sel->radius > 0.f)) sel = nullptr;
    if (ref) {
        if (fdcm_status st = check_refine(ref)) return st;
        if (top_k > kRefineMaxMatches) return fail(FDCM_ERR_INVALID, "pose refinement: top_k must be in 1.." + std::to_string(kRefineMaxMatches));
    }
    if (tc->device != m->device) return fail(FDCM_ERR_INVALID, "templates and feature map live on different devices");
    if (m->stage != 0) return fail(FDCM_ERR_INVALID, "feature map was built with a debug stage");
    fdcm_templates* t = const_cast<fdcm_templates*>(tc);
    if (t->n_tmpl == 0 || m->dm.D == 0 || m->dm.W == 0 || m->dm.H == 0) return FDCM_OK;
    std::lock_guard<std::mutex> lk(m->search_mutex);
    CUDA_TRY(cudaSetDevice(m->device));
    cudaStream_t s;
    if (fdcm_status st = get_stream(m->device, &s)) return st;
    if (fdcm_status st = map_wait(m, s)) return st;
    if (fdcm_status st = templates_ready(t, s)) return st;
    int smem_optin = 0;
    if (fdcm_status st = search_smem_optin(m->device, t->max_lines, &smem_optin)) return st;
    const DenseGrid g = dense_grid(dense, m->shift, m->dm.W, m->dm.H);
    if (g.nx == 0 || g.ny == 0) return FDCM_OK;
    const int cell = std::min(dense->cell, std::max(g.nx, g.ny));
    const int cells_x = (g.nx + cell - 1) / cell, cells_y = (g.ny + cell - 1) / cell;
    const int64_t per_tmpl = (int64_t)dense->rotations * cells_y * cells_x;
    const int64_t limit = ((int64_t)1 << 31) - 1;
    if (per_tmpl > limit || per_tmpl * t->n_tmpl > limit)
        return fail(FDCM_ERR_INVALID, "dense search: " + std::to_string(per_tmpl) + " records per template x " + std::to_string(t->n_tmpl) +
                                          " templates; at most 2^31 - 1 records (use fewer rotations or templates, a larger cell or stride, or a region)");
    const int64_t H = per_tmpl * t->n_tmpl;

    std::vector<int64_t> hyp_off((size_t)t->n_tmpl + 1);
    for (int i = 0; i <= t->n_tmpl; ++i) hyp_off[(size_t)i] = (int64_t)i * per_tmpl;
    std::vector<float> rot(2 * (size_t)dense->rotations);
    for (int r = 0; r < dense->rotations; ++r) dense_rotation(dense, r, &rot[2 * (size_t)r], &rot[2 * (size_t)r + 1]);
    CUDA_TRY(m->s_rec.reserve((size_t)H * sizeof(fdcm_match)));
    CUDA_TRY(m->s_valid.reserve((size_t)H));
    CUDA_TRY(m->s_hyp_off.reserve(hyp_off.size() * 8));
    CUDA_TRY(m->s_dense_keys.reserve((size_t)H * 8));
    CUDA_TRY(m->s_dense_rot.reserve(rot.size() * 4));
    CUDA_TRY(cudaMemcpyAsync(m->s_dense_rot.p, rot.data(), rot.size() * 4, cudaMemcpyHostToDevice, s));
    const float* d_denom = nullptr;
    if (fdcm_status st = stage_uploads(m, t, hyp_off.data(), hyp_off.size(), penalty_kind, penalty_tau, s, &d_denom)) return st;
    DenseLaunch dl;
    dl.lines = t->lines.as<float4>();
    dl.offsets = t->offs.as<int32_t>();
    dl.anchors = t->anchors.as<float2>();
    dl.rot = m->s_dense_rot.as<float2>();
    dl.denom = d_denom;
    dl.n_tmpl = t->n_tmpl;
    dl.rotations = dense->rotations;
    dl.tmpl_idx_base = tmpl_idx_base;
    dl.lo_x = g.lo_x;
    dl.lo_y = g.lo_y;
    dl.stride = dense->stride;
    dl.nx = g.nx;
    dl.ny = g.ny;
    dl.cell = cell;
    dl.cells_x = cells_x;
    dl.cells_y = cells_y;
    const int cell_rows = std::min(cell, g.ny);
    dl.band = std::max(1, std::min(cells_y, (32 + cell_rows - 1) / cell_rows));
    dl.n_bands = (cells_y + dl.band - 1) / dl.band;
    dl.n_rec = H;
    dl.keys = m->s_dense_keys.as<unsigned long long>();
    dl.rec = m->s_rec.as<fdcm_match>();
    dl.valid = m->s_valid.as<uint8_t>();
    CUDA_TRY(cudaMemsetAsync(dl.keys, 0xFF, (size_t)H * 8, s));
    {
        KernelScope k("dense_eval", 0.0, s);
        CUDA_TRY(launch_dense_eval(map_view(m), m->table_dev, dl, t->max_lines, smem_optin, s));
    }
    {
        KernelScope k("dense_finish", (double)H * (8 + sizeof(fdcm_match) + 1), s);
        launch_dense_finish(map_view(m), dl, s);
    }
    const int k = top_k;
    CUDA_TRY(m->s_topk_out.reserve((size_t)k * sizeof(fdcm_match)));
    CUDA_TRY(m->s_topk_n.reserve(4));
    if (sel) {
        fdcm_search_params sp{};
        sp.top_k = k;
        sp.tmpl_idx_base = tmpl_idx_base;
        if (fdcm_status st = run_select(m, t, &sp, sel, H, s)) return st;
    } else {
        const int blocks = topk_ws_blocks(H);
        CUDA_TRY(m->s_topk_score.reserve((size_t)blocks * k * 4));
        CUDA_TRY(m->s_topk_idx.reserve((size_t)blocks * k * 8));
        KernelScope ks("topk", 0.0, s, 2);
        launch_topk(dl.rec, dl.valid, H, k, m->s_topk_score.as<float>(), m->s_topk_idx.as<int64_t>(), blocks, m->s_topk_out.as<fdcm_match>(),
                    m->s_topk_n.as<int>(), s);
    }
    CUDA_TRY(cudaGetLastError());
    if (ref)
        if (fdcm_status st = run_refine(m, t, tmpl_idx_base, d_denom, ref, m->s_topk_out.as<fdcm_match>(), m->s_topk_n.as<int>(), k,
                                        m->s_topk_out.as<fdcm_match>(), smem_optin, s))
            return st;
    const fdcm_status result = finish_topk(m, nullptr, k, s, nullptr, out, capacity, n_out);
    prof_resolve();
    return result;
}

extern "C" fdcm_status fdcm_dense_poses(const fdcm_dense_params* dense, const float anchor[2], const float shift[2], int32_t width,
                                        int32_t height, int32_t rotation, float* out, int64_t capacity, int64_t* n_out, int32_t grid_wh[2]) {
    if (fdcm_status st = check_dense(dense)) return st;
    if (!anchor || !shift || !n_out || !grid_wh) return fail(FDCM_ERR_INVALID, "null argument");
    if (width < 0 || height < 0) return fail(FDCM_ERR_INVALID, "width and height must be >= 0");
    if (rotation < 0 || rotation >= dense->rotations) return fail(FDCM_ERR_INVALID, "rotation must be in 0..rotations - 1");
    const DenseGrid g = dense_grid(dense, shift, width, height);
    grid_wh[0] = g.nx;
    grid_wh[1] = g.ny;
    const int64_t n = (int64_t)g.nx * g.ny;
    *n_out = n;
    if (n > capacity || (n > 0 && !out)) return fail(FDCM_ERR_CAPACITY, "output buffer too small");
    float c, s;
    dense_rotation(dense, rotation, &c, &s);
    for (int v = 0; v < g.ny; ++v)
        for (int u = 0; u < g.nx; ++u)
            dense_pose(c, s, anchor[0], anchor[1], g.lo_x + u * dense->stride, g.lo_y + v * dense->stride, shift[0], shift[1],
                       out + 6 * ((size_t)v * g.nx + u));
    return FDCM_OK;
}

extern "C" fdcm_status fdcm_comm_search_topk(fdcm_comm* comm, const fdcm_dt3* m, const fdcm_templates* shard, const float* scene,
                                             int32_t n_scene, const fdcm_search_params* p, fdcm_match* out, int64_t capacity,
                                             int64_t* n_out) {
    if (!comm) return fail(FDCM_ERR_INVALID, "comm is null");
    return search_impl(m, shard, scene, n_scene, p, out, capacity, n_out, comm, nullptr);
}

extern "C" fdcm_status fdcm_comm_search_select(fdcm_comm* comm, const fdcm_dt3* m, const fdcm_templates* shard, const float* scene,
                                               int32_t n_scene, const fdcm_search_params* p, const fdcm_select_params* select,
                                               fdcm_match* out, int64_t capacity, int64_t* n_out) {
    if (!comm) return fail(FDCM_ERR_INVALID, "comm is null");
    if (!select) return fail(FDCM_ERR_INVALID, "select is null");
    return search_impl(m, shard, scene, n_scene, p, out, capacity, n_out, comm, select);
}

extern "C" fdcm_status fdcm_comm_rebuild_broadcast(fdcm_comm* comm, fdcm_dt3* m, const float* scene_xyxy, int32_t n_lines, int32_t root) {
    if (!comm || !m) return fail(FDCM_ERR_INVALID, "null argument");
    if (root < 0 || root >= comm->world) return fail(FDCM_ERR_INVALID, "bad root");
    if (n_lines < 0 || (n_lines > 0 && !scene_xyxy)) return fail(FDCM_ERR_INVALID, "bad scene");
    if (m->stage != 0) return fail(FDCM_ERR_INVALID, "feature map was built with a debug stage");
    CUDA_TRY(cudaSetDevice(m->device));
    cudaStream_t s;
    if (fdcm_status st = get_stream(m->device, &s)) return st;
    std::lock_guard<std::mutex> lk(m->search_mutex);
    fdcm_status st = map_wait(m, s);
    if (st == FDCM_OK) st = prepare_and_upload(m, scene_xyxy, n_lines, s);
    if (st == FDCM_OK && comm->rank == root) st = run_build_kernels(m, s);
    if (st == FDCM_OK && n_lines > 0) {
        const size_t bytes = (size_t)m->dm.D * m->dm.plane_elems * sizeof(float);
        ncclResult_t r = nccl_api().Broadcast(m->planes.p, m->planes.p, bytes, ncclChar, root, comm->comm, s);
        if (r != ncclSuccess) st = fail(FDCM_ERR_CUDA, std::string("ncclBroadcast: ") + nccl_api().GetErrorString(r));
    }
    if (st == FDCM_OK) st = upload_build_scene(m, scene_xyxy, n_lines, s);
    if (st == FDCM_OK) st = map_written(m, s);
    if (st == FDCM_OK && cudaStreamSynchronize(s) != cudaSuccess) st = fail(FDCM_ERR_CUDA, "rebuild_broadcast: stream failed");
    prof_resolve();
    if (st != FDCM_OK) {
        const std::string msg = g_last_error;
        invalidate_map(m);
        g_last_error = msg;
    }
    return st;
}


struct fdcm_scene_batch {
    int device = 0;
    fdcm_dt3_params params{};
    fdcm_dt3* maps[2] = {nullptr, nullptr};
    cudaStream_t build_stream = nullptr;
    ~fdcm_scene_batch() {
        cudaSetDevice(device);
        for (int i = 0; i < 2; ++i)
            if (maps[i]) fdcm_dt3_release(maps[i]);
        if (build_stream) cudaStreamDestroy(build_stream);
    }
};

extern "C" fdcm_status fdcm_scene_batch_create(const fdcm_dt3_params* params, int32_t device, fdcm_scene_batch** out) {
    if (!out) return fail(FDCM_ERR_INVALID, "out is null");
    *out = nullptr;
    if (fdcm_status st = validate_params(params)) return st;
    CUDA_TRY(cudaSetDevice(device));
    fdcm_scene_batch* b = new (std::nothrow) fdcm_scene_batch();
    if (!b) return fail(FDCM_ERR_NOMEM, "host allocation failed");
    b->device = device;
    b->params = *params;
    cudaError_t e = cudaStreamCreateWithFlags(&b->build_stream, cudaStreamNonBlocking);
    for (int i = 0; i < 2 && e == cudaSuccess; ++i) {
        b->maps[i] = new (std::nothrow) fdcm_dt3();
        if (!b->maps[i]) { delete b; return fail(FDCM_ERR_NOMEM, "host allocation failed"); }
        b->maps[i]->params = *params;
        b->maps[i]->device = device;
        b->maps[i]->stage = 0;
    }
    if (e != cudaSuccess) {
        delete b;
        return fail(FDCM_ERR_CUDA, std::string("scene_batch_create: ") + cudaGetErrorString(e));
    }
    *out = b;
    return FDCM_OK;
}

extern "C" fdcm_status fdcm_scene_batch_destroy(fdcm_scene_batch* b) {
    delete b;
    return FDCM_OK;
}

static fdcm_status batch_queue_build(fdcm_scene_batch* b, int slot, const float* scene, int32_t n_lines) {
    fdcm_dt3* m = b->maps[slot];
    std::lock_guard<std::mutex> lk(m->search_mutex);
    fdcm_status st = map_wait(m, b->build_stream);
    if (st == FDCM_OK) st = prepare_and_upload(m, scene, n_lines, b->build_stream);
    if (st == FDCM_OK) st = run_build_kernels(m, b->build_stream);
    if (st == FDCM_OK) st = upload_build_scene(m, scene, n_lines, b->build_stream);
    if (st == FDCM_OK) st = map_written(m, b->build_stream);
    if (st != FDCM_OK) {
        const std::string msg = g_last_error;
        cudaStreamSynchronize(b->build_stream);
        invalidate_map(m);
        g_last_error = msg;
        return st;
    }
    return FDCM_OK;
}

static fdcm_status search_scenes_impl(fdcm_scene_batch* b, const float* scene_lines, const int32_t* scene_offsets, int32_t n_scenes,
                                      const fdcm_templates* templates, const fdcm_search_params* p, const fdcm_select_params* sel,
                                      fdcm_match* out, int32_t* n_out) {
    if (!b || !p || n_scenes < 0) return fail(FDCM_ERR_INVALID, "bad argument");
    if (n_scenes == 0) return FDCM_OK;
    if (!scene_offsets || !templates || !out || !n_out) return fail(FDCM_ERR_INVALID, "null argument");
    if (p->top_k <= 0) return fail(FDCM_ERR_INVALID, "fdcm_search_scenes needs top_k > 0 (fixed-size result per scene)");
    for (int s = 0; s < n_scenes; ++s)
        if (scene_offsets[s + 1] < scene_offsets[s]) return fail(FDCM_ERR_INVALID, "scene offsets must be non-decreasing");
    if (scene_offsets[n_scenes] > 0 && !scene_lines) return fail(FDCM_ERR_INVALID, "scene_lines is null");
    CUDA_TRY(cudaSetDevice(b->device));
    auto scene_ptr = [&](int s) { return scene_lines + 4 * (size_t)scene_offsets[s]; };
    auto scene_n = [&](int s) { return scene_offsets[s + 1] - scene_offsets[s]; };
    if (fdcm_status st = batch_queue_build(b, 0, scene_ptr(0), scene_n(0))) return st;
    for (int s = 0; s < n_scenes; ++s) {
        const int slot = s & 1;
        if (s + 1 < n_scenes)
            if (fdcm_status st = batch_queue_build(b, slot ^ 1, scene_ptr(s + 1), scene_n(s + 1))) return st;
        int64_t n = 0;
        fdcm_search_params ps = *p;
        const fdcm_status st = search_impl(b->maps[slot], templates, nullptr, FDCM_SCENE_RESIDENT, &ps, out + (size_t)s * p->top_k, p->top_k, &n, nullptr,
                                           sel);
        if (st != FDCM_OK) return st;
        n_out[s] = (int32_t)n;
    }
    return FDCM_OK;
}

extern "C" fdcm_status fdcm_search_scenes(fdcm_scene_batch* b, const float* scene_lines, const int32_t* scene_offsets, int32_t n_scenes,
                                          const fdcm_templates* templates, const fdcm_search_params* p, fdcm_match* out, int32_t* n_out) {
    return search_scenes_impl(b, scene_lines, scene_offsets, n_scenes, templates, p, nullptr, out, n_out);
}

extern "C" fdcm_status fdcm_search_scenes_select(fdcm_scene_batch* b, const float* scene_lines, const int32_t* scene_offsets, int32_t n_scenes,
                                                 const fdcm_templates* templates, const fdcm_search_params* p, const fdcm_select_params* select,
                                                 fdcm_match* out, int32_t* n_out) {
    if (!select) return fail(FDCM_ERR_INVALID, "select is null");
    if (p)
        if (fdcm_status st = check_select(select, p->top_k, false)) return st;
    return search_scenes_impl(b, scene_lines, scene_offsets, n_scenes, templates, p, select, out, n_out);
}

extern "C" fdcm_status fdcm_optimize(const fdcm_dt3* m, const float* tmpl_lines, const int32_t* tmpl_offsets, int32_t n_tmpl,
                                     const float* alignments, int32_t batch_size, uint8_t* has_value, float* scores,
                                     float* translations) {
    if (!m || n_tmpl < 0 || batch_size < 0) return fail(FDCM_ERR_INVALID, "bad argument");
    if (n_tmpl == 0) return FDCM_OK;
    if (!tmpl_offsets || !alignments || !has_value || !scores || !translations) return fail(FDCM_ERR_INVALID, "null argument");
    if (m->dm.D == 0) return fail(FDCM_ERR_INVALID, "optimize on an empty feature map");
    if (m->stage != 0) return fail(FDCM_ERR_INVALID, "feature map was built with a debug stage");
    const int64_t n_lines = tmpl_offsets[n_tmpl];
    if (n_lines > 0 && !tmpl_lines) return fail(FDCM_ERR_INVALID, "tmpl_lines is null");
    CUDA_TRY(cudaSetDevice(m->device));
    cudaStream_t s;
    if (fdcm_status st = get_stream(m->device, &s)) return st;
    std::lock_guard<std::mutex> lk(m->search_mutex);
    if (fdcm_status st = map_wait(m, s)) return st;
    int max_lines = 1;
    for (int t = 0; t < n_tmpl; ++t) max_lines = std::max(max_lines, tmpl_offsets[t + 1] - tmpl_offsets[t]);
    int smem_optin = 0;
    if (fdcm_status st = search_smem_optin(m->device, max_lines, &smem_optin)) return st;
    DevBuf dl, doff, dal, drec, dval, dcnt;
    auto cleanup = [&]() { for (DevBuf* b : {&dl, &doff, &dal, &drec, &dval, &dcnt}) b->release(); };
    std::vector<fdcm_match> rec((size_t)n_tmpl);
    cudaError_t e = dl.reserve(std::max<size_t>(16, (size_t)n_lines * 16));
    if (e == cudaSuccess) e = doff.reserve((size_t)(n_tmpl + 1) * 4);
    if (e == cudaSuccess) e = dal.reserve((size_t)n_tmpl * 8);
    if (e == cudaSuccess) e = drec.reserve((size_t)n_tmpl * sizeof(fdcm_match));
    if (e == cudaSuccess) e = dval.reserve((size_t)n_tmpl);
    if (e == cudaSuccess) e = dcnt.reserve(3 * 8);
    if (e == cudaSuccess && n_lines) e = cudaMemcpyAsync(dl.p, tmpl_lines, (size_t)n_lines * 16, cudaMemcpyHostToDevice, s);
    if (e == cudaSuccess) e = cudaMemcpyAsync(doff.p, tmpl_offsets, (size_t)(n_tmpl + 1) * 4, cudaMemcpyHostToDevice, s);
    if (e == cudaSuccess) e = cudaMemcpyAsync(dal.p, alignments, (size_t)n_tmpl * 8, cudaMemcpyHostToDevice, s);
    if (e == cudaSuccess) e = cudaMemsetAsync(dcnt.p, 0, 3 * 8, s);
    if (e == cudaSuccess) {
        TemplatesView tv{};
        tv.lines = dl.as<float4>();
        tv.offsets = doff.as<int32_t>();
// ... 217 lines not shown
```

### openfdcm_b200/csrc/integral_tma.cu

```cuda
#include "common.cuh"
#include "kernels.h"
#include "tma.cuh"

namespace fdcm {

constexpr int kICW = 128;
constexpr int kIRB = 32;
constexpr int kIYBoxW = kICW + kIRB + 4;
constexpr int kIXBoxW = 36;
constexpr int kIXBoxH = kICW + kIRB;
constexpr int kIStages = 2;
constexpr int kIStageFloats = kIXBoxW * kIXBoxH > kIYBoxW * kIRB ? kIXBoxW * kIXBoxH : kIYBoxW * kIRB;
constexpr int kIConsumerWarps = kICW / 32;
constexpr int kIThreads = kICW + 32;
static_assert((kIStageFloats * 4) % 128 == 0, "TMA destinations must stay 128-byte aligned");

__device__ __forceinline__ float lds_f32(uint32_t addr) {
    float v;
    asm("ld.shared.f32 %0, [%1];" : "=f"(v) : "r"(addr));
    return v;
}

__global__ void __launch_bounds__(kIThreads, 4)
integral_tma_kernel(const __grid_constant__ CUtensorMap map_y, const __grid_constant__ CUtensorMap map_x,
                    float* __restrict__ planes, MapDims dm, const __grid_constant__ IntegralParams ip,
                    const int4* __restrict__ items, int n_items,
                    int* __restrict__ counter) {
    extern __shared__ __align__(128) float stages[];
    __shared__ __align__(8) uint64_t bars[2 * kIStages];
    __shared__ int s_item;
    __shared__ int s_xtbl[kIConsumerWarps][kIRB + 8];
    __shared__ int s_xoff[kIConsumerWarps][kIRB + 8];
    const int tid = threadIdx.x, warp = tid >> 5, lane = tid & 31;
    const uint32_t full0 = smem_u32(bars), empty0 = smem_u32(bars + kIStages);
    const uint32_t stage0 = smem_u32(stages);
    if (tid < kIConsumerWarps * (kIRB + 8)) {
        (&s_xtbl[0][0])[tid] = 0;
        (&s_xoff[0][0])[tid] = 0;
    }
    if (tid == 0) {
        for (int s = 0; s < kIStages; ++s) {
            mbar_init(full0 + 8u * s, 1);
            mbar_init(empty0 + 8u * s, kIConsumerWarps);
        }
        mbar_init_fence();
        prefetch_tensormap(&map_y);
        prefetch_tensormap(&map_x);
    }
    __syncthreads();
    uint32_t it = 0;
    for (;;) {
        if (tid == 0) s_item = atomicAdd(counter, 1);
        __syncthreads();
        const int item = s_item;
        __syncthreads();
        if (item >= n_items) break;
        const int d = items[item].x, c0 = items[item].y, b_lo = items[item].z, b_hi = items[item].w;
        const int mode = ip.mode[d];
        const float rslope = mode == 1 ? ip.ry[d] : ip.rx[d];
        auto R = [&](int i) { return (int)roundf((float)i * rslope); };
        float* P = planes + (size_t)d * dm.plane_elems;
        const int n_major = mode == 1 ? dm.W : dm.H;
        const int nblk = b_hi - b_lo;

        if (warp == kIConsumerWarps) {
            if (lane == 0) {
                const bool rev = (mode == 1 ? ip.rx[d] : ip.ry[d]) < 0;
                auto origin = [&](int b, int& cx, int& cy) {
                    const int i0 = b * kIRB, i1 = min(n_major, i0 + kIRB);
                    const int minor0 = c0 + min(R(i0), R(i1 - 1));
                    const int major0 = rev ? n_major - kIRB - i0 : i0;
                    if (mode == 1) { cx = major0 & ~3; cy = minor0; }
                    else { cx = minor0 & ~3; cy = major0; }
                };
                const CUtensorMap* map = mode == 1 ? &map_x : &map_y;
                const uint32_t bytes = mode == 1 ? kIXBoxW * kIXBoxH * 4 : kIYBoxW * kIRB * 4;
                int cx, cy;
                for (int b = b_lo; b < b_hi; ++b, ++it) {
                    const uint32_t st = it % kIStages, ph = (it / kIStages) & 1u;
                    origin(b, cx, cy);
                    mbar_wait_backoff(empty0 + 8u * st, ph ^ 1u, 200);
                    mbar_arrive_expect_tx(full0 + 8u * st, bytes);
                    tma_load_3d(stage0 + st * (kIStageFloats * 4), map, cx, cy, d, full0 + 8u * st);
                }
            } else {
                it += nblk;
            }
            it = __shfl_sync(0xffffffffu, it, 0);
            continue;
        }

        const int c = c0 + tid;
        float acc = 0.f;
        bool have = false;
        if (mode == 2) {
            const bool rev = ip.ry[d] < 0;
            for (int b = b_lo; b < b_hi; ++b, ++it) {
                const uint32_t st = it % kIStages, ph = (it / kIStages) & 1u;
                const int i0 = b * kIRB, nk = min(dm.H - i0, kIRB);
                const int Rl = R(min(i0 + lane, dm.H - 1));
                const int Ra = __shfl_sync(0xffffffffu, Rl, 0), Rb = __shfl_sync(0xffffffffu, Rl, nk - 1);
                const int Rmin = min(Ra, Rb);
                const float* tile = stages + (size_t)st * kIStageFloats + tid - Rmin + ((c0 + Rmin) & 3);
                const int ystep = rev ? -dm.pitch : dm.pitch;
                float* row = P + (long long)(rev ? dm.H - 1 - i0 : i0) * dm.pitch + c;
                const int tstep = rev ? -kIYBoxW : kIYBoxW;
                tile += rev ? (kIRB - 1) * kIYBoxW : 0;
                const bool inside = (unsigned)(c + Ra) < (unsigned)dm.W && (unsigned)(c + Rb) < (unsigned)dm.W;
                const bool fast = __all_sync(0xffffffffu, inside && have);
                mbar_wait_backoff(full0 + 8u * st, ph, 40);
                uint32_t ta = smem_u32(tile);
                asm volatile("" : "+r"(ta), "+l"(row));
                __builtin_assume(__isGlobal(row));
                const int tsb = rev ? -kIYBoxW * 4 : kIYBoxW * 4;
                constexpr int kHalf = kIRB / 2;
                if (fast && nk == kIRB) {
#pragma unroll
                    for (int k0 = 0; k0 < kIRB; k0 += kHalf) {
                        float v[kHalf];
                        int go[kHalf];
#pragma unroll
                        for (int i = 0; i < kHalf; ++i) {
                            const int k = k0 + i;
                            const int Rk = __shfl_sync(0xffffffffu, Rl, k);
                            v[i] = lds_f32(ta + (uint32_t)(Rk << 2) + (uint32_t)(k * tsb));
                            go[i] = k * ystep + Rk;
                        }
#pragma unroll
                        for (int i = 0; i < kHalf; ++i) {
                            acc = v[i] + acc;
                            row[go[i]] = acc;
                        }
                    }
                } else {
#pragma unroll
                    for (int k0 = 0; k0 < kIRB; k0 += kHalf) {
                        float v[kHalf];
                        int go[kHalf];
                        unsigned in = 0u;
#pragma unroll
                        for (int i = 0; i < kHalf; ++i) {
                            const int k = k0 + i;
                            const int Rk = __shfl_sync(0xffffffffu, Rl, k);
                            const bool ok = k < nk && (unsigned)(c + Rk) < (unsigned)dm.W;
                            v[i] = 0.f;
                            if (ok) v[i] = lds_f32(ta + (uint32_t)(Rk << 2) + (uint32_t)(k * tsb));
                            go[i] = k * ystep + Rk;
                            in |= ok ? 1u << i : 0u;
                        }
#pragma unroll
                        for (int i = 0; i < kHalf; ++i) {
                            const bool ok = (in >> i) & 1u;
                            const bool st_ok = ok && have;
                            acc = st_ok ? v[i] + acc : (ok ? v[i] : acc);
                            if (st_ok) row[go[i]] = acc;
                            if (k0 + i < nk) have = ok;
                        }
                    }
                }
                __syncwarp();
                if (lane == 0) mbar_arrive(empty0 + 8u * st);
            }
        } else {
            const bool fwd = !(ip.rx[d] < 0);
            const int grp = lane >> 3;
            for (int b = b_lo; b < b_hi; ++b, ++it) {
                const uint32_t st = it % kIStages, ph = (it / kIStages) & 1u;
                const int i0 = b * kIRB, ncols = min(dm.W - i0, kIRB);
                const int Rl = R(min(i0 + lane, dm.W - 1));
                const int Ra = __shfl_sync(0xffffffffu, Rl, 0), Rb = __shfl_sync(0xffffffffu, Rl, ncols - 1);
                const int Rmin = min(Ra, Rb);
                const int offl = Rl - Rmin;
                const int ybase = c0 + Rmin;
                float* tile = stages + (size_t)st * kIStageFloats;
                const int xb = fwd ? i0 : dm.W - kIRB - i0;
                const int xoff = xb & 3;
                const int mb = xoff + (fwd ? 0 : kIRB - 1), ms = fwd ? 1 : -1;
                const bool interior = ncols == kIRB && ybase >= 0 && ybase + kIXBoxH <= dm.H;
                const bool fast = __all_sync(0xffffffffu, have) && interior;
                mbar_wait_backoff(full0 + 8u * st, ph, 40);
                if (fast) {
                    s_xtbl[warp][lane + 3] = (offl * kIXBoxW + mb + ms * lane) * 4;
                    __syncwarp();
                    const int* tl = &s_xtbl[warp][3 - grp];
                    char* lb = reinterpret_cast<char*>(tile) + tid * (kIXBoxW * 4);
                    constexpr int kSlots = kIRB + 3, kChunk = 12;
#pragma unroll
                    for (int s0 = 0; s0 < kSlots; s0 += kChunk) {
                        float v[kChunk];
                        float* a[kChunk];
#pragma unroll
                        for (int i = 0; i < kChunk; ++i) {
                            const int s = s0 + i;
                            if (s < kSlots) {
                                const bool ok = (s >= 3 && s < kIRB) || (unsigned)(s - grp) < (unsigned)kIRB;
                                a[i] = reinterpret_cast<float*>(lb + tl[s]);
                                if (ok) v[i] = *a[i];
                            }
                        }
#pragma unroll
                        for (int i = 0; i < kChunk; ++i) {
                            const int s = s0 + i;
                            if (s < kSlots) {
                                const bool ok = (s >= 3 && s < kIRB) || (unsigned)(s - grp) < (unsigned)kIRB;
                                if (ok) { acc = v[i] + acc; v[i] = acc; }
                            }
                        }
#pragma unroll
                        for (int i = 0; i < kChunk; ++i) {
                            const int s = s0 + i;
                            if (s < kSlots) {
                                const bool ok = (s >= 3 && s < kIRB) || (unsigned)(s - grp) < (unsigned)kIRB;
                                if (ok) *a[i] = v[i];
                            }
                        }
                    }
                } else {
                    s_xtbl[warp][lane + 3] = (offl * kIXBoxW + mb + ms * lane) * 4;
                    s_xoff[warp][lane + 3] = offl;
                    __syncwarp();
                    const int* tl = &s_xtbl[warp][3 - grp];
                    const int* ol = &s_xoff[warp][3 - grp];
                    char* lb = reinterpret_cast<char*>(tile) + tid * (kIXBoxW * 4);
                    const int y0 = ybase + tid;
                    constexpr int kSlots = kIRB + 3, kChunk = 12;
#pragma unroll
                    for (int s0 = 0; s0 < kSlots; s0 += kChunk) {
                        float v[kChunk];
                        float* a[kChunk];
                        unsigned in = 0u, jv = 0u;
#pragma unroll
                        for (int i = 0; i < kChunk; ++i) {
                            const int s = s0 + i;
                            if (s < kSlots) {
                                const bool jok = (unsigned)(s - grp) < (unsigned)ncols;
                                const bool ok = jok && (unsigned)(y0 + ol[s]) < (unsigned)dm.H;
                                a[i] = reinterpret_cast<float*>(lb + tl[s]);
                                v[i] = 0.f;
                                if (ok) v[i] = *a[i];
                                jv |= jok ? 1u << i : 0u;
                                in |= ok ? 1u << i : 0u;
                            }
                        }
                        unsigned stm = 0u;
#pragma unroll
                        for (int i = 0; i < kChunk; ++i) {
                            if (s0 + i < kSlots) {
                                const bool ok = (in >> i) & 1u;
                                const bool st_ok = ok && have;
                                acc = st_ok ? v[i] + acc : (ok ? v[i] : acc);
                                v[i] = acc;
                                stm |= st_ok ? 1u << i : 0u;
                                if ((jv >> i) & 1u) have = ok;
                            }
                        }
#pragma unroll
                        for (int i = 0; i < kChunk; ++i) {
                            if (s0 + i < kSlots) {
                                if ((stm >> i) & 1u) *a[i] = v[i];
                            }
                        }
                    }
                }
                named_bar_sync(1, kICW);
                const int jl = fwd ? lane : kIRB - 1 - lane;
                const int off_m = __shfl_sync(0xffffffffu, offl, jl);
                const int x = xb + lane;
                const bool col_ok = jl < ncols;
                if (interior && xoff == 0) {
                    const int off_lo = Ra < Rb ? 0 : Ra - Rb, off_hi = Ra < Rb ? Rb - Ra : 0;
                    const int full_lo = max(off_lo, off_hi), full_hi = kICW + min(off_lo, off_hi);
                    const int sub = lane >> 3, l8 = lane & 7;
                    {
                        constexpr int kG = 4;
                        const int r0 = full_lo + warp * 4 + sub;
                        float* g4 = P + (long long)(ybase + r0) * dm.pitch + xb + 4 * l8;
#pragma unroll
                        for (int h = 0; h < kICW / (kIConsumerWarps * 4 * kG); ++h) {
                            float4 v[kG];
#pragma unroll
                            for (int i = 0; i < kG; ++i) {
                                const int r = r0 + (h * kG + i) * kIConsumerWarps * 4;
                                if (r < full_hi) v[i] = *reinterpret_cast<const float4*>(tile + r * kIXBoxW + 4 * l8);
                            }
#pragma unroll
                            for (int i = 0; i < kG; ++i) {
                                const int r = r0 + (h * kG + i) * kIConsumerWarps * 4;
                                if (r < full_hi) *reinterpret_cast<float4*>(g4 + (h * kG + i) * kIConsumerWarps * 4 * dm.pitch) = v[i];
                            }
                        }
                    }
                    float* gcol = P + (long long)ybase * dm.pitch + x;
#pragma unroll
                    for (int part = 0; part < 2; ++part) {
                        constexpr int kR = kIRB / kIConsumerWarps;
                        const int rb = part == 0 ? warp : full_hi + warp, re = part == 0 ? full_lo : kIXBoxH;
                        float w[kR];
#pragma unroll
                        for (int i = 0; i < kR; ++i) {
                            const int r = rb + i * kIConsumerWarps;
                            if (r < re && (unsigned)(r - off_m) < (unsigned)kICW) w[i] = tile[r * kIXBoxW + lane];
                        }
#pragma unroll
                        for (int i = 0; i < kR; ++i) {
                            const int r = rb + i * kIConsumerWarps;
                            if (r < re && (unsigned)(r - off_m) < (unsigned)kICW) gcol[r * dm.pitch] = w[i];
                        }
                    }
                } else {
                    float* gp = P + (long long)(ybase + warp) * dm.pitch + x;
                    const float* tp = tile + warp * kIXBoxW + lane + xoff;
#pragma unroll 4
                    for (int r = warp; r < kIXBoxH; r += kIConsumerWarps, gp += (size_t)kIConsumerWarps * dm.pitch, tp += kIConsumerWarps * kIXBoxW)
                        if (col_ok && (unsigned)(r - off_m) < (unsigned)kICW && (unsigned)(ybase + r) < (unsigned)dm.H) *gp = *tp;
                }
                fence_proxy_async();
                __syncwarp();
                if (lane == 0) mbar_arrive(empty0 + 8u * st);
            }
        }
    }
}

size_t integral_tma_smem_bytes() { return (size_t)kIStages * kIStageFloats * sizeof(float); }
int integral_strip_chains() { return kICW; }
int integral_tile_steps() { return kIRB; }

bool integral_tma_encode(const void* planes, const MapDims& dm, CUtensorMap* map_y, CUtensorMap* map_x) {
    return encode_planes_map(map_y, planes, dm.W, dm.H, dm.D, dm.pitch, kIYBoxW, kIRB, 1) &&
           encode_planes_map(map_x, planes, dm.W, dm.H, dm.D, dm.pitch, kIXBoxW, kIXBoxH, 1);
}

void launch_integral_tma(float* d_planes, const MapDims& dm, const IntegralParams& ip, const IntegralPlanDev& plan, int n_sms,
                         cudaStream_t s) {
    if (plan.n_items <= 0) return;
    const size_t smem = integral_tma_smem_bytes();
    cudaFuncSetAttribute(integral_tma_kernel, cudaFuncAttributeMaxDynamicSharedMemorySize, (int)smem);
    int per_sm = 2;
    if (cudaOccupancyMaxActiveBlocksPerMultiprocessor(&per_sm, integral_tma_kernel, kIThreads, smem) != cudaSuccess || per_sm < 1) per_sm = 2;
    const int grid = plan.n_items < per_sm * n_sms ? plan.n_items : per_sm * n_sms;
    integral_tma_kernel<<<grid, kIThreads, smem, s>>>(plan.map_y, plan.map_x, d_planes, dm, ip, plan.items4,
                                                      plan.n_items, plan.counter);
}

}
```

### openfdcm_b200/csrc/kernels.h

```cpp
#pragma once
#include <cuda.h>

#include "common.cuh"
#include "../../include/fdcm_b200.h"

namespace fdcm {

void launch_raster(const float* d_lines, const int32_t* d_bins, int n_lines, const MapDims& dm, uint32_t* d_mask, cudaStream_t s);
void launch_dt_pass_literal(int src_kind, bool along_rows, const void* d_src, float* d_planes, const MapDims& dm, void* d_stack,
                            cudaStream_t s);
void launch_transpose_square(float* d_planes, const MapDims& dm, cudaStream_t s);
void launch_sqrt(float* d_planes, const MapDims& dm, cudaStream_t s);
void launch_propagate(float* d_planes, const MapDims& dm, const PropParams& pp, bool sqrt_first, cudaStream_t s);

struct IntegralPlanDev {
    const int4* items4;
    int n_items;
    int* counter;
    CUtensorMap map_y, map_x;
};
size_t integral_tma_smem_bytes();
int integral_strip_chains();
int integral_tile_steps();
bool integral_tma_encode(const void* planes, const MapDims& dm, CUtensorMap* map_y, CUtensorMap* map_x);
void launch_integral_tma(float* d_planes, const MapDims& dm, const IntegralParams& ip, const IntegralPlanDev& plan, int n_sms,
                         cudaStream_t s);

int dt_band_count(const MapDims& dm);
size_t dt_band_info_bytes(const MapDims& dm);
size_t dt_band_spill_bytes(const MapDims& dm, int maxdepth);
void launch_dt_col_band(const uint32_t* d_mask, const MapDims& dm, void* d_info, cudaStream_t s);
void launch_dt_row_envelope(const void* d_info, const uint16_t* d_g, const MapDims& dm, void* d_ws, int win_lo, int win_hi, int row_lo,
                            int row_hi, int which, cudaStream_t s);
void dt_band_scene_rows(const MapDims& dm, int row_lo, int row_hi, int* y0, int* y1);
void launch_dt_row_fill(float* d_planes, const MapDims& dm, void* d_ws, int win_lo, int win_hi, cudaStream_t s);
bool dt_fill_propagate_supported(const MapDims& dm);
void launch_dt_resolve(const MapDims& dm, void* d_ws, int win_lo, int win_hi, int ya0, int ya1, int yb0, int yb1, cudaStream_t s);
void launch_dt_fill_propagate(float* d_planes, const MapDims& dm, void* d_ws, int win_lo, int win_hi, const PropParams& pp,
                              bool sqrt_first, int ya0, int ya1, int yb0, int yb1, cudaStream_t s);

void launch_dt_row_l1_band(const void* d_info, float* d_planes, const MapDims& dm, cudaStream_t s);
void launch_dt_l1_propagate(const void* d_info, float* d_planes, const MapDims& dm, const PropParams& pp, cudaStream_t s);
size_t dt_band_smem_bytes(const MapDims& dm);
cudaError_t run_sqrt_check(unsigned long long* h_bad, uint32_t* h_first, cudaStream_t s);

struct MapView {
    const float* planes;
    MapDims dm;
    float shift_x, shift_y;
};

struct TemplatesView {
    const float4* lines;
    const int32_t* offsets;
    const int32_t* argsort;
    const float* line_len;
    const float* denom;
    int32_t n_tmpl;
    int32_t max_lines;
};

struct SceneView {
    const float4* lines;
    const float* sorted_len;
    const int32_t* sorted_idx;
    int32_t n;
};

struct SearchLaunch {
    int32_t max_tmpl_lines, max_scene_lines, batch;
    int32_t tmpl_idx_base;
    const int64_t* hyp_off;
    int64_t n_hyp;
    const int32_t* perm;
    const int4* hyp_ready;
    const float2* direct_align;
};

struct SearchOutputs {
    fdcm_match* rec;
    uint8_t* valid;
    int4* hyp;
    unsigned long long* counters;
};

constexpr int kSearchCellW = 128, kSearchCellH = 384;
size_t search_order_temp_bytes(int64_t n_hyp);
void launch_search_order(const TemplatesView& tv, const SceneView& sv, const SearchLaunch& sl, uint32_t* d_keys, uint32_t* d_keys_out,
                         int32_t* d_idx, int32_t* d_perm, void* d_temp, size_t temp_bytes, float minx, float miny, int cells_x,
                         int key_bits, int4* d_hyp, cudaStream_t s);

int search_max_template_lines(int smem_optin);
cudaError_t launch_search(const MapView& map, const SlopeTableDev& table, const TemplatesView& tv, const SceneView& sv,
                          const SearchLaunch& sl, const SearchOutputs& out, int smem_optin, cudaStream_t s);

void launch_topk(const fdcm_match* d_rec, const uint8_t* d_valid, int64_t n, int k, float* d_ws_score, int64_t* d_ws_idx,
                 int ws_blocks, fdcm_match* d_out, int* d_n_out, cudaStream_t s);
int topk_ws_blocks(int64_t n);
void launch_topk_merge(const fdcm_match* d_gathered, int n_cand, int k, fdcm_match* d_out, int* d_n_out, cudaStream_t s);
void launch_topk_invalid(fdcm_match* d_out, int k, int* d_n_out, cudaStream_t s);

struct SelectLaunch {
    const fdcm_match* rec;
    const uint8_t* valid;
    const int64_t* hyp_off;
    const float2* anchors;
    int64_t n_hyp;
    int32_t n_tmpl, tmpl_idx_base;
    int32_t top_k;
    int32_t cap;
    int32_t radius_on, any_angle;
    float r2, cos_thr;
};
constexpr int kSelectMaxAcross = FDCM_SELECT_MAX_ACROSS;
size_t select_temp_bytes(int64_t n_hyp);
void launch_select_sort(const SelectLaunch& p, bool by_template, uint64_t* keys_in, uint64_t* keys_out, int32_t* vals_in,
                        int32_t* vals_out, void* d_temp, size_t temp_bytes, cudaStream_t s);
void launch_select_greedy(const SelectLaunch& p, const uint64_t* sorted_keys, const int32_t* sorted_h, uint32_t* surv_keys, float4* acc,
                          cudaStream_t s);
void launch_select_topk(const SelectLaunch& p, const uint32_t* surv_keys, uint32_t* keys_out, const int32_t* vals_in, int32_t* vals_out,
                        void* d_temp, size_t temp_bytes, fdcm_match* d_out, int* d_n_out, cudaStream_t s);
void launch_select_walk(const SelectLaunch& p, const uint64_t* sorted_keys, const int32_t* sorted_h, fdcm_match* d_out, int* d_n_out,
                        cudaStream_t s);

constexpr int kRefineSide = 2 * FDCM_REFINE_MAX_STEPS + 1;
struct RefineLevel {
    float ci[kRefineSide], si[kRefineSide];
    float h;
};
struct RefineState { float c[6]; float raw; int32_t valid; };
struct RefineLaunch {
    const fdcm_match* in;
    const int* d_n;
    int32_t n;
    const float4* lines;
    const int32_t* offsets;
    const float2* anchors;
    const float* denom;
    int32_t tmpl_idx_base;
    int32_t n_r, n_t;
    RefineState* state;
    unsigned long long* keys;
};
struct RefineRot { float r0, r1, r3, r4, bx, by; };
__host__ __device__ inline RefineRot refine_rotation(const float* c, float ax, float ay, int i, float ci, float si) {
    if (i == 0) return RefineRot{c[0], c[1], c[3], c[4], c[2], c[5]};
    const float px = (c[0] * ax + c[1] * ay) + c[2], py = (c[3] * ax + c[4] * ay) + c[5];
    const float ux = c[2] - px, uy = c[5] - py;
    return RefineRot{ci * c[0] - si * c[3], ci * c[1] - si * c[4], si * c[0] + ci * c[3], si * c[1] + ci * c[4],
                     (ci * ux - si * uy) + px, (si * ux + ci * uy) + py};
}
void launch_refine_init(const RefineLaunch& p, cudaStream_t s);
cudaError_t launch_refine_eval(const MapView& map, const SlopeTableDev& table, const RefineLaunch& p, const RefineLevel& lv,
                               int max_lines, int smem_optin, cudaStream_t s);
void launch_refine_advance(const RefineLaunch& p, const RefineLevel& lv, fdcm_match* out, cudaStream_t s);

struct DenseLaunch {
    const float4* lines;
    const int32_t* offsets;
    const float2* anchors;
    const float2* rot;
    const float* denom;
    int32_t n_tmpl, rotations, tmpl_idx_base;
    int32_t lo_x, lo_y, stride;
    int32_t nx, ny;
    int32_t cell, cells_x, cells_y;
    int32_t band;
    int32_t n_bands;
    int64_t n_rec;
    unsigned long long* keys;
    fdcm_match* rec;
    uint8_t* valid;
};
__host__ __device__ inline float dense_tx(float c, float s, float ax, float ay, int gx, float shift_x) {
    return ((float)gx - shift_x) - (c * ax - s * ay);
}
__host__ __device__ inline float dense_ty(float c, float s, float ax, float ay, int gy, float shift_y) {
    return ((float)gy - shift_y) - (s * ax + c * ay);
// ... 16 lines not shown
```

### openfdcm_b200/csrc/search_kernels.cu

```cuda
#include <climits>
#include <cstdlib>

#include <cub/device/device_radix_sort.cuh>

#include "common.cuh"
#include "kernels.h"

namespace fdcm {

struct Rigid { float r00, r01, tx, r10, r11, ty; };

__device__ __forceinline__ void unit_vec_dev(const float4 l, float& ux, float& uy) {
    const float dx = l.z - l.x, dy = l.w - l.y;
    const float z = dx * dx + dy * dy;
    if (z > 0.f) {
        const float n = sqrtf(z);
        ux = dx / n;
        uy = dy / n;
    } else {
        ux = dx;
        uy = dy;
    }
}

// ... 63 lines not shown
        for (int j = 0; j < 4; ++j) {
            const bool sg = signbit(m[j]);
            const float pos = sg ? inf : m[j];
            const float neg = sg ? m[j] : -inf;
            pos_nan |= (pos != pos);
            neg_nan |= (neg != neg);
            if (neg > neg_max) neg_max = neg;
            if (pos < pos_min) pos_min = pos;
        }
        E0[a] = neg_nan ? nan : neg_max;
        E1[a] = pos_nan ? nan : pos_min;
    }
    const bool f0 = isfinite(E0[0]) && isfinite(E1[0]);
    const bool f1 = isfinite(E0[1]) && isfinite(E1[1]);
    if (f0 && f1) { lo = fmaxf(E0[0], E0[1]); hi = fminf(E1[0], E1[1]); }
    else if (f0) { lo = E0[0]; hi = E1[0]; }
    else { lo = E0[1]; hi = E1[1]; }
}

__device__ __forceinline__ long long trunc_ll(float x) { return (long long)x; }

struct HypDecode { int t, l0, L, tline, sline, rev; };
__device__ __forceinline__ HypDecode decode_hypothesis(long long h, const TemplatesView& tv, const SceneView& sv, const SearchLaunch& sl) {
    HypDecode r;
    int lo = 0, hi = tv.n_tmpl;
    while (hi - lo > 1) {
        const int mid = (lo + hi) >> 1;
        if (sl.hyp_off[mid] <= h) lo = mid; else hi = mid;
    }
    r.t = lo;
    const int loc = (int)(h - sl.hyp_off[r.t]);
    r.l0 = tv.offsets[r.t];
    r.L = tv.offsets[r.t + 1] - r.l0;
    const int nS = min(sv.n, sl.max_scene_lines);
    const int rank = loc / (2 * nS);
    const int slot = (loc >> 1) % nS;
    r.rev = loc & 1;
    r.tline = tv.argsort[r.l0 + rank];
    const float value = tv.line_len[r.l0 + r.tline];
    int b0 = 0, b1 = sv.n;
    while (b0 < b1) {
        const int mid = (b0 + b1) >> 1;
        if (sv.sorted_len[mid] > value) b0 = mid + 1; else b1 = mid;
    }
    int closest;
    if (b0 == 0) closest = 0;
    else if (b0 == sv.n) closest = sv.n - 1;
    else closest = fabsf(value - sv.sorted_len[b0]) < fabsf(value - sv.sorted_len[b0 - 1]) ? b0 : b0 - 1;
    int rb = max(0, closest - sl.max_scene_lines / 2);
    const int re = min(rb + sl.max_scene_lines, sv.n);
    rb = max(0, re - sl.max_scene_lines);
    r.sline = sv.sorted_idx[rb + slot];
    return r;
}

__global__ void search_key_kernel(const __grid_constant__ TemplatesView tv, const __grid_constant__ SceneView sv,
                                  const __grid_constant__ SearchLaunch sl, float minx, float miny, int cells_x,
                                  uint32_t* __restrict__ keys, int32_t* __restrict__ idx, int4* __restrict__ hyp) {
    const long long h = (long long)blockIdx.x * blockDim.x + threadIdx.x;
    if (h >= sl.n_hyp) return;
    const HypDecode d = decode_hypothesis(h, tv, sv, sl);
    hyp[h] = make_int4(d.t + sl.tmpl_idx_base, d.tline, d.sline, d.rev);
    const float4 s = sv.lines[d.sline];
    const int cx = min(max((int)(((s.x + s.z) * 0.5f - minx) * (1.f / (float)kSearchCellW)), 0), cells_x - 1);
    const int cy = min(max((int)(((s.y + s.w) * 0.5f - miny) * (1.f / (float)kSearchCellH)), 0), 4095);
    keys[h] = (uint32_t)(cy * cells_x + cx);
    idx[h] = (int32_t)h;
}

size_t search_order_temp_bytes(int64_t n_hyp) {
    size_t bytes = 0;
    cub::DeviceRadixSort::SortPairs(nullptr, bytes, (const uint32_t*)nullptr, (uint32_t*)nullptr, (const int32_t*)nullptr,
                                    (int32_t*)nullptr, (int)n_hyp);
    return bytes;
}

void launch_search_order(const TemplatesView& tv, const SceneView& sv, const SearchLaunch& sl, uint32_t* d_keys, uint32_t* d_keys_out,
                         int32_t* d_idx, int32_t* d_perm, void* d_temp, size_t temp_bytes, float minx, float miny, int cells_x,
                         int key_bits, int4* d_hyp, cudaStream_t s) {
    search_key_kernel<<<(unsigned)((sl.n_hyp + 255) / 256), 256, 0, s>>>(tv, sv, sl, minx, miny, cells_x, d_keys, d_idx, d_hyp);
    cub::DeviceRadixSort::SortPairs(d_temp, temp_bytes, d_keys, d_keys_out, d_idx, d_perm, (int)sl.n_hyp, 0, key_bits, s);
}

__global__ void __launch_bounds__(128, 6) search_warp_kernel(const __grid_constant__ MapView map,
                                                          const __grid_constant__ SlopeTableDev table,
                                                          const __grid_constant__ TemplatesView tv,
                                                          const __grid_constant__ SceneView sv,
                                                          const __grid_constant__ SearchLaunch sl,
                                                          const __grid_constant__ SearchOutputs out) {
    extern __shared__ __align__(16) uint8_t s_raw[];
    const int lane = threadIdx.x & 31, warp = threadIdx.x >> 5;
    const long long slot_idx = (long long)blockIdx.x * (blockDim.x >> 5) + warp;
    if (slot_idx >= sl.n_hyp) return;
    const long long h = sl.perm ? (long long)sl.perm[slot_idx] : slot_idx;
    const size_t per_warp = (size_t)tv.max_lines * 16 + (((size_t)tv.max_lines + 15) & ~(size_t)15);
    float4* apts = reinterpret_cast<float4*>(s_raw + (size_t)warp * per_warp);
    uint8_t* bins = reinterpret_cast<uint8_t*>(apts + tv.max_lines);
    unsigned long long n_eval = 0;
    bool valid = false;

    int t, l0, L;
    float avx, avy;
    Rigid T;
    if (sl.direct_align) {
        t = (int)h;
        l0 = tv.offsets[t];
        L = tv.offsets[t + 1] - l0;
        T = Rigid{1.f, 0.f, 0.f, 0.f, 1.f, 0.f};
        avx = sl.direct_align[h].x;
        avy = sl.direct_align[h].y;
    } else {
        HypDecode d;
        if (sl.hyp_ready) {
            const int4 q = sl.hyp_ready[h];
            d.t = q.x - sl.tmpl_idx_base; d.tline = q.y; d.sline = q.z; d.rev = q.w;
            d.l0 = tv.offsets[d.t];
            d.L = tv.offsets[d.t + 1] - d.l0;
        } else {
            d = decode_hypothesis(h, tv, sv, sl);
            if (lane == 0) out.hyp[h] = make_int4(d.t + sl.tmpl_idx_base, d.tline, d.sline, d.rev);
        }
        t = d.t; l0 = d.l0; L = d.L;
        T = align_dev(tv.lines[l0 + d.tline], sv.lines[d.sline], d.rev, avx, avy);
    }
    const float4* TL = tv.lines + l0;
    const float asum = fabsf(avx) + fabsf(avy);
    const bool null_vec = (double)asum <= (double)FLT_EPSILON + 1e-10 * (double)asum;
    if (!null_vec) {
        float svx, svy;
        rasterize_vector_dev(avx, avy, svx, svy);
        float mnx = INFINITY, mny = INFINITY, mxx = -INFINITY, mxy = -INFINITY;
        for (int i = lane; i < L; i += 32) {
            const float4 p = __ldg(TL + i);
            float ax, ay, bx, by;
            xform(T, p.x, p.y, ax, ay);
            xform(T, p.z, p.w, bx, by);
            mnx = fminf(mnx, fminf(ax, bx)); mxx = fmaxf(mxx, fmaxf(ax, bx));
            mny = fminf(mny, fminf(ay, by)); mxy = fmaxf(mxy, fmaxf(ay, by));
            apts[i] = make_float4(ax, ay, bx, by);
            bins[i] = (uint8_t)bin_of_slope_dev(table, (by - ay) / (bx - ax));
        }
#pragma unroll
        for (int o = 16; o > 0; o >>= 1) {
            mnx = fminf(mnx, __shfl_xor_sync(0xffffffffu, mnx, o)); mxx = fmaxf(mxx, __shfl_xor_sync(0xffffffffu, mxx, o));
            mny = fminf(mny, __shfl_xor_sync(0xffffffffu, mny, o)); mxy = fmaxf(mxy, __shfl_xor_sync(0xffffffffu, mxy, o));
        }
        __syncwarp();
        float min_mul, max_mul;
        minmax_dev(mnx + map.shift_x, mny + map.shift_y, mxx + map.shift_x, mxy + map.shift_y, (float)map.dm.W,
                   (float)map.dm.H, svx, svy, min_mul, max_mul);
        if (isfinite(min_mul) && isfinite(max_mul)) {
            const float* planes = map.planes;
            const unsigned pitch = (unsigned)map.dm.pitch;
            const unsigned last = (unsigned)(map.dm.plane_elems - 1);
            const int maxm = (int)min(max(trunc_ll(max_mul), -70000LL), 70000LL), minm = (int)min(max(trunc_ll(min_mul), -70000LL), 70000LL);
            auto score_of = [&](int mult) -> float {
                const float m = (float)mult;
                const float offx = map.shift_x + m * svx, offy = map.shift_y + m * svy;
                return eigen_sum_lazy(L, [&](int i) {
                    const float4 a = apts[i];
                    const int x1 = (int)(a.x + offx), y1 = (int)(a.y + offy), x2 = (int)(a.z + offx), y2 = (int)(a.w + offy);
                    const unsigned i1 = min((unsigned)y1 * pitch + (unsigned)x1, last), i2 = min((unsigned)y2 * pitch + (unsigned)x2, last);
                    const float* P = planes + (size_t)bins[i] * map.dm.plane_elems;
                    return fabsf(__ldg(P + i1) - __ldg(P + i2));
                });
            };
            int c_lo = 0, c_n = 0;
            float c_score = 0.f;
            auto fill_cache = [&](int lo, int hi) {
                c_lo = lo;
                c_n = hi - lo + 1;
                if (lane < c_n) c_score = score_of(lo + lane);
                __syncwarp();
            };
            const int B = sl.batch;
            const int span = B >= 8 ? min(B, 32) : 32;
            auto score_at = [&](int j, int dir) -> float {
                if (j < c_lo || j >= c_lo + c_n) {
                    if (dir > 0) fill_cache(j, min(maxm, j + span - 1));
                    else fill_cache(max(minm, j - span + 1), j);
                }
                return __shfl_sync(0xffffffffu, c_score, j - c_lo);
            };
            {
                int lo, hi;
                if (2 * span + 1 <= 32) { lo = max(minm, -span); hi = min(maxm, span); }
                else if (span >= 16) { lo = 0; hi = min(maxm, min(span, 31)); }
                else { lo = max(minm, -15); hi = min(maxm, 16); }
                if (lo > 0) lo = 0;
                if (hi < 0) hi = 0;
                fill_cache(lo, hi);
            }
            float back = score_at(0, 1);
            n_eval += 1;
            float best = back, best_tx = 0.f, best_ty = 0.f;
            for (int dir = 1; dir >= -1; dir -= 2) {
                const int lim = dir > 0 ? maxm : -minm;
                for (int kk = 1; kk <= lim; kk += B) {
                    const int jend = min(kk + B - 1, lim);
                    float bmin = 0.f, blast = 0.f;
                    int barg = kk;
                    (void)score_at(dir * kk, dir);
                    const int la = dir * kk - c_lo, lb = dir * jend - c_lo;
                    const bool inside = min(la, lb) >= 0 && max(la, lb) < c_n;
                    const unsigned bmask = inside ? (0xFFFFFFFFu >> (31 - max(la, lb))) & (0xFFFFFFFFu << min(la, lb)) : 0u;
                    const bool in_batch = (bmask >> lane) & 1u;
                    if (inside && __ballot_sync(0xffffffffu, in_batch && !(c_score >= 0.f)) == 0u) {
                        const unsigned key = in_batch ? __float_as_uint(c_score) : 0xFFFFFFFFu;
                        const unsigned kmin = __reduce_min_sync(0xffffffffu, key);
                        const unsigned hit = __ballot_sync(0xffffffffu, in_batch && key == kmin);
                        const int lmin = dir > 0 ? __ffs(hit) - 1 : 31 - __clz(hit);
                        bmin = __uint_as_float(kmin);
                        barg = dir * (c_lo + lmin);
                        blast = __shfl_sync(0xffffffffu, c_score, lb);
                    } else {
                        for (int j = kk; j <= jend; ++j) {
                            const float sj = score_at(dir * j, dir);
                            if (j == kk || sj < bmin) { bmin = sj; barg = j; }
                            blast = sj;
                        }
                    }
                    n_eval += (unsigned long long)(jend - kk + 1);
                    if (bmin > back) break;
                    back = bmin;
                    if (bmin < best) {
                        best = bmin;
                        best_tx = (float)(dir * barg) * svx;
                        best_ty = (float)(dir * barg) * svy;
                    }
                    if (bmin < blast) break;
                }
            }
            valid = true;
            if (lane == 0) {
                fdcm_match m;
                m.tmpl_idx = t + sl.tmpl_idx_base;
                m.score = tv.denom ? best / tv.denom[t] : best;
                m.transform[0] = T.r00; m.transform[1] = T.r01; m.transform[2] = T.tx + best_tx;
                m.transform[3] = T.r10; m.transform[4] = T.r11; m.transform[5] = T.ty + best_ty;
                out.rec[h] = m;
            }
        }
    }
    if (lane == 0) {
        out.valid[h] = valid ? 1 : 0;
        atomicAdd(out.counters + 0, n_eval);
        atomicAdd(out.counters + 1, n_eval * 2ull * (unsigned long long)L);
        atomicAdd(out.counters + 2, valid ? 1ull : 0ull);
    }
}

static size_t search_smem_per_warp(int max_lines) { return (size_t)max_lines * 16 + (((size_t)max_lines + 15) & ~(size_t)15); }

int search_max_template_lines(int smem_optin) {
    int L = smem_optin / 17;
    while (search_smem_per_warp(L + 1) <= (size_t)smem_optin) ++L;
    while (L > 0 && search_smem_per_warp(L) > (size_t)smem_optin) --L;
    return L;
}

cudaError_t launch_search(const MapView& map, const SlopeTableDev& table, const TemplatesView& tv, const SceneView& sv,
                          const SearchLaunch& sl, const SearchOutputs& out, int smem_optin, cudaStream_t s) {
    if (sl.n_hyp <= 0) return cudaSuccess;
    const size_t per_warp = search_smem_per_warp(tv.max_lines);
    int hyps = 4;
    while (hyps > 1 && (size_t)hyps * per_warp > (size_t)smem_optin) hyps >>= 1;
    const size_t smem = (size_t)hyps * per_warp;
    if (smem > (size_t)smem_optin) return cudaErrorInvalidValue;
    if (smem > 48 * 1024) {
        const cudaError_t e = cudaFuncSetAttribute(search_warp_kernel, cudaFuncAttributeMaxDynamicSharedMemorySize, (int)smem);
        if (e != cudaSuccess) return e;
    }
    const unsigned grid = (unsigned)((sl.n_hyp + hyps - 1) / hyps);
    search_warp_kernel<<<grid, hyps * 32, smem, s>>>(map, table, tv, sv, sl, out);
    return cudaGetLastError();
}

struct Key { float s; long long i; };
__device__ __forceinline__ bool key_less(const Key& a, const Key& b) { return a.s < b.s || (a.s == b.s && a.i < b.i); }

__device__ Key block_min_key(Key k, Key* s_keys) {
#pragma unroll
    for (int o = 16; o > 0; o >>= 1) {
        Key other;
        other.s = __shfl_down_sync(0xffffffffu, k.s, o);
        other.i = __shfl_down_sync(0xffffffffu, k.i, o);
        if (key_less(other, k)) k = other;
    }
    const int warp = threadIdx.x >> 5, lane = threadIdx.x & 31;
    if (lane == 0) s_keys[warp] = k;
    __syncthreads();
    if (warp == 0) {
        const int nw = blockDim.x >> 5;
        k = lane < nw ? s_keys[lane] : Key{INFINITY, LLONG_MAX};
#pragma unroll
        for (int o = 16; o > 0; o >>= 1) {
            Key other;
            other.s = __shfl_down_sync(0xffffffffu, k.s, o);
            other.i = __shfl_down_sync(0xffffffffu, k.i, o);
            if (key_less(other, k)) k = other;
        }
        if (lane == 0) s_keys[0] = k;
    }
    __syncthreads();
    k = s_keys[0];
    __syncthreads();
    return k;
}

__global__ void __launch_bounds__(1024) topk_level1_kernel(const fdcm_match* __restrict__ rec, const uint8_t* __restrict__ valid,
                                                           long long n, long long chunk, int k, float* __restrict__ ws_score,
                                                           long long* __restrict__ ws_idx) {
    __shared__ Key s_keys[32];
    const long long begin = (long long)blockIdx.x * chunk;
    const long long end = min(n, begin + chunk);
    Key last{-INFINITY, -1};
// ... 188 lines not shown
        float4 me = make_float4(0.f, 0.f, 0.f, 0.f);
        if (live && p.radius_on) {
            me = match_anchor(p.rec[h], anchor);
            for (int j = 0; j < n_acc && live; ++j) live = !anchors_near(acc[b + j], me, p);
        }
        for (;;) {
            const unsigned alive = __ballot_sync(0xffffffffu, live);
            if (alive == 0u || n_acc == lim) break;
            const int ld = __ffs(alive) - 1;
            const float4 a = make_float4(__shfl_sync(0xffffffffu, me.x, ld), __shfl_sync(0xffffffffu, me.y, ld),
                                         __shfl_sync(0xffffffffu, me.z, ld), __shfl_sync(0xffffffffu, me.w, ld));
            if (lane == ld) {
                surv_keys[h] = key;
                if (p.radius_on) acc[b + n_acc] = me;
                live = false;
            } else if (live && p.radius_on && anchors_near(a, me, p)) {
                live = false;
            }
            ++n_acc;
        }
        __syncwarp();
        if (last_chunk) break;
    }
}

void launch_select_greedy(const SelectLaunch& p, const uint64_t* sorted_keys, const int32_t* sorted_h, uint32_t* surv_keys, float4* acc,
                          cudaStream_t s) {
    cudaMemsetAsync(surv_keys, 0xFF, (size_t)p.n_hyp * 4, s);
    select_greedy_kernel<<<(unsigned)((p.n_tmpl + 3) / 4), 128, 0, s>>>(p, sorted_keys, sorted_h, surv_keys, acc);
}

__global__ void select_gather_kernel(const uint32_t* __restrict__ skeys, const int32_t* __restrict__ sh, long long n,
                                     const fdcm_match* __restrict__ rec, int k, fdcm_match* __restrict__ out, int* __restrict__ n_out) {
    __shared__ int s_n;
    if (threadIdx.x == 0) s_n = 0;
    __syncthreads();
    int mine = 0;
    for (int q = threadIdx.x; q < k; q += blockDim.x) {
        if (q < n && skeys[q] != kInvalidKey) {
            out[q] = rec[sh[q]];
            ++mine;
        } else {
            write_invalid(out + q);
        }
    }
    atomicAdd(&s_n, mine);
    __syncthreads();
    if (threadIdx.x == 0) *n_out = s_n;
}

void launch_select_topk(const SelectLaunch& p, const uint32_t* surv_keys, uint32_t* keys_out, const int32_t* vals_in, int32_t* vals_out,
                        void* d_temp, size_t temp_bytes, fdcm_match* d_out, int* d_n_out, cudaStream_t s) {
    cub::DeviceRadixSort::SortPairs(d_temp, temp_bytes, surv_keys, keys_out, vals_in, vals_out, (int)p.n_hyp, 0, 32, s);
    select_gather_kernel<<<1, 256, 0, s>>>(keys_out, vals_out, p.n_hyp, p.rec, p.top_k, d_out, d_n_out);
}

__global__ void __launch_bounds__(1024) select_walk_kernel(const __grid_constant__ SelectLaunch p, const uint64_t* __restrict__ skeys,
                                                           const int32_t* __restrict__ sh, fdcm_match* __restrict__ out,
                                                           int* __restrict__ n_out) {
    __shared__ float4 s_acc[kSelectMaxAcross];
    __shared__ int s_tmpl[kSelectMaxAcross];
    __shared__ unsigned s_live[32];
    const int tid = threadIdx.x, lane = tid & 31, warp = tid >> 5, n_warps = blockDim.x >> 5;
    int n_acc = 0;
    for (long long base = 0; base < p.n_hyp && n_acc < p.top_k; base += blockDim.x) {
        const long long i = base + tid;
        const uint32_t key = i < p.n_hyp ? (uint32_t)skeys[i] : kInvalidKey;
        bool live = key != kInvalidKey;
        const bool last_chunk = __syncthreads_or(!live) != 0;
        int h = 0, t = -1, same = 0;
        float4 me = make_float4(0.f, 0.f, 0.f, 0.f);
        if (live) {
            h = sh[i];
            const fdcm_match m = p.rec[h];
            t = m.tmpl_idx - p.tmpl_idx_base;
            me = match_anchor(m, p.anchors[t]);
            for (int j = 0; j < n_acc && live; ++j) {
                same += s_tmpl[j] == t;
                live = !(p.radius_on && anchors_near(s_acc[j], me, p));
            }
            if (p.cap > 0 && same >= p.cap) live = false;
        }
        for (;;) {
            const unsigned m = __ballot_sync(0xffffffffu, live);
            if (lane == 0) s_live[warp] = m;
            __syncthreads();
            int ld = -1;
            for (int w = 0; w < n_warps; ++w)
                if (s_live[w]) { ld = w * 32 + __ffs(s_live[w]) - 1; break; }
            if (ld < 0) break;
            if (tid == ld) {
                s_acc[n_acc] = me;
                s_tmpl[n_acc] = t;
                out[n_acc] = p.rec[h];
                live = false;
            }
            __syncthreads();
            const float4 a = s_acc[n_acc];
            const int at = s_tmpl[n_acc];
            ++n_acc;
            if (n_acc == p.top_k) break;
            if (live) {
                same += at == t;
                if ((p.cap > 0 && same >= p.cap) || (p.radius_on && anchors_near(a, me, p))) live = false;
            }
        }
        __syncthreads();
        if (last_chunk) break;
    }
    for (int q = n_acc + tid; q < p.top_k; q += blockDim.x) write_invalid(out + q);
    if (tid == 0) *n_out = n_acc;
}

void launch_select_walk(const SelectLaunch& p, const uint64_t* sorted_keys, const int32_t* sorted_h, fdcm_match* d_out, int* d_n_out,
                        cudaStream_t s) {
    select_walk_kernel<<<1, 1024, 0, s>>>(p, sorted_keys, sorted_h, d_out, d_n_out);
}

constexpr unsigned long long kNoPose = ~0ull;

struct StagedBox { float mnx, mny, mxx, mxy; bool nan; };
__device__ __forceinline__ StagedBox stage_rotated(const float4* __restrict__ lines, int L, float r0, float r1, float r3, float r4,
                                                   bool as_given, const SlopeTableDev& table, float4* apts, uint8_t* bins) {
    const int tid = threadIdx.x, lane = tid & 31;
    bool nan = false;
    for (int q = tid; q < L; q += blockDim.x) {
        const float4 v = __ldg(lines + q);
        float x1 = v.x, y1 = v.y, x2 = v.z, y2 = v.w;
        if (!as_given) {
            x1 = r0 * v.x + r1 * v.y; y1 = r3 * v.x + r4 * v.y;
            x2 = r0 * v.z + r1 * v.w; y2 = r3 * v.z + r4 * v.w;
        }
        nan |= x1 != x1 || y1 != y1 || x2 != x2 || y2 != y2;
        apts[q] = make_float4(x1, y1, x2, y2);
        bins[q] = (uint8_t)bin_of_slope_dev(table, (y2 - y1) / (x2 - x1));
    }
    StagedBox b;
    b.nan = __syncthreads_or(nan) != 0;
    b.mnx = INFINITY; b.mny = INFINITY; b.mxx = -INFINITY; b.mxy = -INFINITY;
    for (int q = lane; q < L; q += 32) {
        const float4 e = apts[q];
        b.mnx = fminf(b.mnx, fminf(e.x, e.z)); b.mxx = fmaxf(b.mxx, fmaxf(e.x, e.z));
        b.mny = fminf(b.mny, fminf(e.y, e.w)); b.mxy = fmaxf(b.mxy, fmaxf(e.y, e.w));
    }
#pragma unroll
    for (int o = 16; o > 0; o >>= 1) {
        b.mnx = fminf(b.mnx, __shfl_xor_sync(0xffffffffu, b.mnx, o)); b.mxx = fmaxf(b.mxx, __shfl_xor_sync(0xffffffffu, b.mxx, o));
        b.mny = fminf(b.mny, __shfl_xor_sync(0xffffffffu, b.mny, o)); b.mxy = fmaxf(b.mxy, __shfl_xor_sync(0xffffffffu, b.mxy, o));
    }
    return b;
}

__device__ __forceinline__ float staged_score(const MapView& map, const float4* apts, const uint8_t* bins, int L, float offx, float offy) {
    const float* planes = map.planes;
    const size_t pitch = (size_t)map.dm.pitch, pe = map.dm.plane_elems;
    return eigen_sum_lazy(L, [&](int q) {
        const float4 e = apts[q];
        const int x1 = (int)(e.x + offx), y1 = (int)(e.y + offy), x2 = (int)(e.z + offx), y2 = (int)(e.w + offy);
        const float* P = planes + (size_t)bins[q] * pe;
        return fabsf(__ldg(P + (size_t)y1 * pitch + x1) - __ldg(P + (size_t)y2 * pitch + x2));
    });
}

__global__ void refine_init_kernel(const __grid_constant__ RefineLaunch p) {
    const int m = blockIdx.x * blockDim.x + threadIdx.x;
    if (m >= (p.d_n ? *p.d_n : p.n)) return;
    RefineState st;
    for (int q = 0; q < 6; ++q) st.c[q] = p.in[m].transform[q];
    st.raw = NAN;
    st.valid = 0;
    p.state[m] = st;
    p.keys[m] = kNoPose;
}

void launch_refine_init(const RefineLaunch& p, cudaStream_t s) {
    refine_init_kernel<<<(unsigned)((p.n + 127) / 128), 128, 0, s>>>(p);
}

__global__ void __launch_bounds__(1024) refine_eval_kernel(const __grid_constant__ MapView map,
                                                           const __grid_constant__ SlopeTableDev table,
                                                           const __grid_constant__ RefineLaunch p,
                                                           const __grid_constant__ RefineLevel lv) {
    extern __shared__ __align__(16) uint8_t s_raw[];
    const int NR = 2 * p.n_r + 1, NT = 2 * p.n_t + 1;
    const int m = blockIdx.x / NR, ir = blockIdx.x % NR;
    if (m >= (p.d_n ? *p.d_n : p.n)) return;
    const int tid = threadIdx.x, lane = tid & 31;
    const RefineState st = p.state[m];
    const int t = p.in[m].tmpl_idx - p.tmpl_idx_base;
    const int l0 = p.offsets[t], L = p.offsets[t + 1] - l0;
    const float2 a = p.anchors[t];
    const RefineRot R = refine_rotation(st.c, a.x, a.y, ir - p.n_r, lv.ci[ir], lv.si[ir]);
    float4* apts = reinterpret_cast<float4*>(s_raw);
    uint8_t* bins = reinterpret_cast<uint8_t*>(apts + L);
    const StagedBox bb = stage_rotated(p.lines + l0, L, R.r0, R.r1, R.r3, R.r4, false, table, apts, bins);
    unsigned long long key = kNoPose;
    if (tid < NT * NT) {
        const int kk = tid / NT, jj = tid - kk * NT;
        const float P2 = R.bx + (float)(jj - p.n_t) * lv.h, P5 = R.by + (float)(kk - p.n_t) * lv.h;
        const float offx = map.shift_x + P2, offy = map.shift_y + P5;
        bool valid = !bb.nan && !(R.r0 != R.r0 || R.r1 != R.r1 || R.r3 != R.r3 || R.r4 != R.r4 || P2 != P2 || P5 != P5);
        if (valid && L > 0)
            valid = 0.f <= bb.mnx + offx && bb.mxx + offx <= (float)(map.dm.W - 1) && 0.f <= bb.mny + offy &&
                    bb.mxy + offy <= (float)(map.dm.H - 1);
        if (valid) {
            const float sc = staged_score(map, apts, bins, L, offx, offy);
            const int di = ir - p.n_r, dk = kk - p.n_t, dj = jj - p.n_t;
            const unsigned order = (unsigned)(di * di + dk * dk + dj * dj) << 15 | (unsigned)((ir * NT + kk) * NT + jj);
            const bool is_nan = sc != sc;
            key = (unsigned long long)(is_nan ? 0x7F800000u : __float_as_uint(sc)) << 32 | (unsigned long long)(order << 1 | (is_nan ? 1u : 0u));
        }
    }
#pragma unroll
    for (int o = 16; o > 0; o >>= 1) {
        const unsigned long long other = __shfl_xor_sync(0xffffffffu, key, o);
        key = other < key ? other : key;
    }
    if (lane == 0 && key != kNoPose) atomicMin(p.keys + m, key);
}

static size_t refine_smem_bytes(int max_lines) { return (size_t)max_lines * 16 + (((size_t)max_lines + 15) & ~(size_t)15); }

cudaError_t launch_refine_eval(const MapView& map, const SlopeTableDev& table, const RefineLaunch& p, const RefineLevel& lv,
                               int max_lines, int smem_optin, cudaStream_t s) {
    const int NR = 2 * p.n_r + 1, NT = 2 * p.n_t + 1;
    const int threads = ((NT * NT + 31) / 32) * 32;
    const size_t smem = refine_smem_bytes(max_lines > 0 ? max_lines : 1);
    if (smem > (size_t)smem_optin) return cudaErrorInvalidValue;
    if (smem > 48 * 1024) {
        const cudaError_t e = cudaFuncSetAttribute(refine_eval_kernel, cudaFuncAttributeMaxDynamicSharedMemorySize, (int)smem);
        if (e != cudaSuccess) return e;
    }
    refine_eval_kernel<<<(unsigned)((int64_t)p.n * NR), threads, smem, s>>>(map, table, p, lv);
    return cudaGetLastError();
}

__global__ void refine_advance_kernel(const __grid_constant__ RefineLaunch p, const __grid_constant__ RefineLevel lv,
                                      fdcm_match* out) {
    const int m = blockIdx.x * blockDim.x + threadIdx.x;
    if (m >= (p.d_n ? *p.d_n : p.n)) return;
    const int tmpl_idx = p.in[m].tmpl_idx;
    const int t = tmpl_idx - p.tmpl_idx_base;
    RefineState st = p.state[m];
    const unsigned long long key = p.keys[m];
    if (key != kNoPose) {
        const unsigned order = (unsigned)key >> 1;
        if ((order >> 15) != 0u) {
            const int NT = 2 * p.n_t + 1, g = (int)(order & 0x7FFFu);
            const int jj = g % NT, kk = (g / NT) % NT, ir = g / (NT * NT);
            const float2 a = p.anchors[t];
            const RefineRot R = refine_rotation(st.c, a.x, a.y, ir - p.n_r, lv.ci[ir], lv.si[ir]);
            st.c[0] = R.r0; st.c[1] = R.r1; st.c[2] = R.bx + (float)(jj - p.n_t) * lv.h;
            st.c[3] = R.r3; st.c[4] = R.r4; st.c[5] = R.by + (float)(kk - p.n_t) * lv.h;
        }
        st.raw = (key & 1ull) ? NAN : __uint_as_float((unsigned)(key >> 32));
        st.valid = 1;
        p.state[m] = st;
        p.keys[m] = kNoPose;
    }
    if (out) {
        fdcm_match r;
        r.tmpl_idx = tmpl_idx;
        r.score = st.valid ? (p.denom ? st.raw / p.denom[t] : st.raw) : NAN;
        for (int q = 0; q < 6; ++q) r.transform[q] = st.c[q];
        out[m] = r;
    }
}

void launch_refine_advance(const RefineLaunch& p, const RefineLevel& lv, fdcm_match* out, cudaStream_t s) {
    refine_advance_kernel<<<(unsigned)((p.n + 127) / 128), 128, 0, s>>>(p, lv, out);
}

constexpr int kDenseThreads = 256;
constexpr int kDenseRowGroup = 8;

template <class Pred>
__device__ __forceinline__ int first_true(int n, Pred pred) {
    int lo = 0, hi = n;
    while (lo < hi) {
        const int mid = (lo + hi) >> 1;
        if (pred(mid)) hi = mid; else lo = mid + 1;
    }
    return lo;
}

__global__ void __launch_bounds__(kDenseThreads) dense_eval_kernel(const __grid_constant__ MapView map,
                                                                   const __grid_constant__ SlopeTableDev table,
                                                                   const __grid_constant__ DenseLaunch p) {
    extern __shared__ __align__(16) uint8_t s_raw[];
    const long long tr = blockIdx.x / p.n_bands;
    const int band = (int)(blockIdx.x - tr * p.n_bands);
    const int r = (int)(tr % p.rotations), t = (int)(tr / p.rotations);
    const int l0 = p.offsets[t], L = p.offsets[t + 1] - l0;
    if (L == 0) return;
    const float2 cs = p.rot[r], a = p.anchors[t];
    const float c = cs.x, s = cs.y;
    float4* apts = reinterpret_cast<float4*>(s_raw);
    uint8_t* bins = reinterpret_cast<uint8_t*>(apts + L);
    const StagedBox bb = stage_rotated(p.lines + l0, L, c, -s, s, c, c == 1.f && s == 0.f, table, apts, bins);
    if (bb.nan) return;
    const float Wm1 = (float)(map.dm.W - 1), Hm1 = (float)(map.dm.H - 1);
    const float shx = map.shift_x, shy = map.shift_y, ax = a.x, ay = a.y;
    const int lo_x = p.lo_x, lo_y = p.lo_y, stride = p.stride;
    auto offx = [=](int u) { return shx + dense_tx(c, s, ax, ay, lo_x + u * stride, shx); };
    auto offy = [=](int v) { return shy + dense_ty(c, s, ax, ay, lo_y + v * stride, shy); };
    const float mnx = bb.mnx, mxx = bb.mxx, mny = bb.mny, mxy = bb.mxy;
    const int ulo = first_true(p.nx, [=](int u) { return 0.f <= mnx + offx(u); });
    const int uhi = first_true(p.nx, [=](int u) { return !(mxx + offx(u) <= Wm1); }) - 1;
    const int vlo = first_true(p.ny, [=](int v) { return 0.f <= mny + offy(v); });
    const int vhi = first_true(p.ny, [=](int v) { return !(mxy + offy(v) <= Hm1); }) - 1;
    if (ulo > uhi || vlo > vhi) return;
    const int lane = threadIdx.x & 31, warp = threadIdx.x >> 5, n_warps = blockDim.x >> 5;
    const int n_chunks = (uhi - ulo + 32) / 32;
    const long long rec0 = ((long long)t * p.rotations + r) * p.cells_y;
    const int cv1 = min(p.cells_y, (band + 1) * p.band);
    for (int cv = band * p.band; cv < cv1; ++cv) {
        const int ra = max(cv * p.cell, vlo), rb = min(cv * p.cell + (p.cell - 1), vhi);
        if (ra > rb) continue;
        const int n_items = ((rb - ra) / kDenseRowGroup + 1) * n_chunks;
        for (int item = warp; item < n_items; item += n_warps) {
            const int grp = item / n_chunks, ch = item - grp * n_chunks;
            const int u = ulo + ch * 32 + lane;
            const int va = ra + grp * kDenseRowGroup, vb = min(va + kDenseRowGroup - 1, rb);
            unsigned long long key = kNoPose;
            if (u <= uhi) {
                const float ox = offx(u);
                for (int v = va; v <= vb; ++v) {
                    const float sc = staged_score(map, apts, bins, L, ox, offy(v));
                    const bool is_nan = sc != sc;
                    const unsigned g = (unsigned)v * (unsigned)p.nx + (unsigned)u;
                    const unsigned long long k =
                        (unsigned long long)(is_nan ? 0x7F800000u : __float_as_uint(sc)) << 32 | (unsigned long long)(g << 1 | (is_nan ? 1u : 0u));
                    key = k < key ? k : key;
                }
            }
            const int cu = u / p.cell;
#pragma unroll
            for (int o = 1; o < 32; o <<= 1) {
                const unsigned long long other = __shfl_down_sync(0xffffffffu, key, o);
                const int ocu = __shfl_down_sync(0xffffffffu, cu, o);
                if (lane + o < 32 && ocu == cu && other < key) key = other;
            }
            const int pcu = __shfl_up_sync(0xffffffffu, cu, 1);
            if ((lane == 0 || pcu != cu) && key != kNoPose) atomicMin(p.keys + (rec0 + cv) * p.cells_x + cu, key);
        }
    }
}

cudaError_t launch_dense_eval(const MapView& map, const SlopeTableDev& table, const DenseLaunch& p, int max_lines, int smem_optin,
                              cudaStream_t s) {
    const size_t smem = refine_smem_bytes(max_lines > 0 ? max_lines : 1);
    if (smem > (size_t)smem_optin) return cudaErrorInvalidValue;
    if (smem > 48 * 1024) {
        const cudaError_t e = cudaFuncSetAttribute(dense_eval_kernel, cudaFuncAttributeMaxDynamicSharedMemorySize, (int)smem);
        if (e != cudaSuccess) return e;
    }
    const long long blocks = (long long)p.n_tmpl * p.rotations * p.n_bands;
    dense_eval_kernel<<<(unsigned)blocks, kDenseThreads, smem, s>>>(map, table, p);
    return cudaGetLastError();
}

__global__ void dense_finish_kernel(const __grid_constant__ MapView map, const __grid_constant__ DenseLaunch p) {
    const long long h = (long long)blockIdx.x * blockDim.x + threadIdx.x;
    if (h >= p.n_rec) return;
    const unsigned long long key = p.keys[h];
    if (key == kNoPose) {
        p.valid[h] = 0;
        return;
    }
    const long long tr = h / ((long long)p.cells_y * p.cells_x);
    const int r = (int)(tr % p.rotations), t = (int)(tr / p.rotations);
    const unsigned g = (unsigned)key >> 1;
    const int u = (int)(g % (unsigned)p.nx), v = (int)(g / (unsigned)p.nx);
    const float2 cs = p.rot[r], a = p.anchors[t];
    fdcm_match m;
    m.tmpl_idx = t + p.tmpl_idx_base;
    const float raw = (key & 1ull) ? NAN : __uint_as_float((unsigned)(key >> 32));
    m.score = p.denom ? raw / p.denom[t] : raw;
    dense_pose(cs.x, cs.y, a.x, a.y, p.lo_x + u * p.stride, p.lo_y + v * p.stride, map.shift_x, map.shift_y, m.transform);
    p.rec[h] = m;
    p.valid[h] = 1;
}

void launch_dense_finish(const MapView& map, const DenseLaunch& p, cudaStream_t s) {
    dense_finish_kernel<<<(unsigned)((p.n_rec + 255) / 256), 256, 0, s>>>(map, p);
}

__global__ void __launch_bounds__(128) evaluate_kernel(const __grid_constant__ MapView map,
                                                       const __grid_constant__ SlopeTableDev table,
                                                       const float4* __restrict__ lines, const int32_t* __restrict__ toff,
                                                       const float2* __restrict__ transl, const int32_t* __restrict__ owner,
                                                       long long n_scores, float* __restrict__ scores) {
    const long long i = (long long)blockIdx.x * blockDim.x + threadIdx.x;
    if (i >= n_scores) return;
    const int t = owner[i];
    const float4* TL = lines + toff[t];
    const int L = toff[t + 1] - toff[t];
    const float2 tr = transl[i];
    const float offx = map.shift_x + tr.x, offy = map.shift_y + tr.y;
    const Rigid I{1.f, 0.f, 0.f, 0.f, 1.f, 0.f};
    scores[i] = eigen_sum_lazy(L, [&](int j) {
        const float4 p = __ldg(TL + j);
        const int bin = bin_of_slope_dev(table, (p.w - p.y) / (p.z - p.x));
        int x1 = (int)(p.x + offx), y1 = (int)(p.y + offy), x2 = (int)(p.z + offx), y2 = (int)(p.w + offy);
        x1 = min(max(x1, 0), map.dm.W - 1); x2 = min(max(x2, 0), map.dm.W - 1);
        y1 = min(max(y1, 0), map.dm.H - 1); y2 = min(max(y2, 0), map.dm.H - 1);
        const float* P = map.planes + (size_t)bin * map.dm.plane_elems;
        return fabsf(__ldg(P + (size_t)y1 * map.dm.pitch + x1) - __ldg(P + (size_t)y2 * map.dm.pitch + x2));
    });
    (void)I;
}

void launch_evaluate(const MapView& map, const SlopeTableDev& table, const float4* d_lines, const int32_t* d_toff,
                     const float2* d_transl, const int32_t* d_troff, const int32_t* d_owner, int64_t n_scores,
                     float* d_scores, cudaStream_t s) {
    (void)d_troff;
    if (n_scores <= 0) return;
    evaluate_kernel<<<(unsigned)((n_scores + 127) / 128), 128, 0, s>>>(map, table, d_lines, d_toff, d_transl, d_owner,
                                                                        n_scores, d_scores);
}

__global__ void classify_kernel(const __grid_constant__ SlopeTableDev table, const float4* __restrict__ lines, int n,
                                int32_t* __restrict__ bins) {
    const int i = blockIdx.x * blockDim.x + threadIdx.x;
    if (i >= n) return;
    const float4 p = lines[i];
    bins[i] = bin_of_slope_dev(table, (p.w - p.y) / (p.z - p.x));
}

void launch_classify(const SlopeTableDev& table, const float4* d_lines, int n, int32_t* d_bins, cudaStream_t s) {
    if (n <= 0) return;
    classify_kernel<<<(n + 127) / 128, 128, 0, s>>>(table, d_lines, n, d_bins);
}

}
```

### openfdcm_b200/distributed.py

```python
import ctypes as C

import numpy as np
import torch
import torch.distributed as dist

from . import _lib
from ._lib import MATCH_DTYPE, check, lib, ptr


class Communicator:

    def __init__(self, unique_id, rank, world, device):
        uid = np.frombuffer(bytes(unique_id), np.uint8).copy()
        assert uid.size == 128
        h = C.c_void_p(0)
        check(lib().fdcm_comm_init(ptr(uid), int(rank), int(world), int(device), C.byref(h)))
        self._h, self.rank, self.world, self.device = h, int(rank), int(world), int(device)

    @staticmethod
    def unique_id():
        uid = np.zeros(128, np.uint8)
        check(lib().fdcm_comm_unique_id(ptr(uid)))
        return uid.tobytes()

    @classmethod
    def from_torch(cls, device, group=None):
        rank, world = dist.get_rank(group), dist.get_world_size(group)
        box = [cls.unique_id() if rank == 0 else None]
        dist.broadcast_object_list(box, src=0, group=group)
        return cls(box[0], rank, world, device)

    def __del__(self):
        h, self._h = getattr(self, "_h", None), None
        if h and lib is not None:
            lib().fdcm_comm_destroy(h)

    def shard(self, n_items):
        b, e = C.c_int32(0), C.c_int32(0)
        check(lib().fdcm_comm_shard(int(n_items), self.rank, self.world, C.byref(b), C.byref(e)))
        return b.value, e.value

    def search_topk(self, featuremap, shard, scene, searcher, optimizer, penalty, k, tmpl_idx_base, *, select=None):
        from . import _records
        s = None if scene is None else _records(scene)
        p = _lib.SearchParams(searcher.max_tmpl_lines, searcher.max_scene_lines, int(optimizer.batch_size),
                              0 if penalty is None else penalty.kind, 0.0 if penalty is None else float(penalty.tau),
                              int(k), int(tmpl_idx_base), 0, 0.0, 0.0, 0.0, 0.0)
        out = np.zeros(int(k), MATCH_DTYPE)
        n = C.c_int64(0)
        n_scene = _lib.FDCM_SCENE_RESIDENT if s is None else s.shape[0]
        if select is None:
            check(lib().fdcm_comm_search_topk(self._h, featuremap._h, shard._h, ptr(s), n_scene, C.byref(p), ptr(out), int(k), C.byref(n)))
        else:
            sp = select._params()
            check(lib().fdcm_comm_search_select(self._h, featuremap._h, shard._h, ptr(s), n_scene, C.byref(p), C.byref(sp), ptr(out), int(k),
                                                C.byref(n)))
        return out[: n.value].copy()

    def rebuild_broadcast(self, featuremap, scene, root=0):
        from . import _records
        r = _records(scene)
        check(lib().fdcm_comm_rebuild_broadcast(self._h, featuremap._h, ptr(r), r.shape[0], int(root)))
        featuremap._refresh()


def shard_range(n_items, rank, world):
    base, rem = divmod(n_items, world)
    begin = rank * base + min(rank, rem)
    return begin, begin + base + (1 if rank < rem else 0)


def shard_templates(templates, rank, world):
    b, e = shard_range(len(templates), rank, world)
    return templates[b:e], b


def shard_scenes(n_scenes, rank, world):
    return list(range(rank, n_scenes, world))


def merge_topk_records(per_rank, k):
    allm = np.concatenate([np.asarray(r, MATCH_DTYPE) for r in per_rank]) if per_rank else np.zeros(0, MATCH_DTYPE)
    order = np.argsort(allm["score"], kind="stable")
    return allm[order[:k]]


def allgather_topk(local_topk, k, device=None, group=None):
    world = dist.get_world_size(group) if dist.is_initialized() else 1
    local = np.zeros(k, MATCH_DTYPE)
    n = min(k, len(local_topk))
    local[:n] = local_topk[:n]
    local["score"][n:] = np.inf
    local["tmpl_idx"][n:] = -1
    if world == 1:
        return merge_topk_records([local[:n]], k)
    buf = torch.from_numpy(local.view(np.uint8).copy())
    if device is not None:
        buf = buf.to(device, non_blocking=False)
    out = torch.empty(world * buf.numel(), dtype=torch.uint8, device=buf.device)
    dist.all_gather_into_tensor(out, buf, group=group)
    rec = out.cpu().numpy().view(MATCH_DTYPE).reshape(world, k)
    return merge_topk_records([r[r["tmpl_idx"] >= 0] for r in rec], k)


def broadcast_featuremap(featuremap, src=0, group=None):
    ptr, nbytes = featuremap.device_ptr()
    n = nbytes // 4

    class _Blob:
        __cuda_array_interface__ = {"shape": (n,), "typestr": "<f4", "data": (ptr, False), "version": 3}

    t = torch.as_tensor(_Blob(), device=f"cuda:{featuremap.device}")
    dist.broadcast(t, src=src, group=group)
    torch.cuda.synchronize(featuremap.device)
```

Measured before the change: 1.830 million.

## Store DT3 planes in 8x4 tiled layout for search gathers

Changes the feature-map storage from row-major to an 8-wide by 4-tall tiled layout, and the search kernels now read through a tiled index. The integral kernel writes directly into the tiled buffer. A row-major mirror is rebuilt on demand for device_ptr users and download paths, and a new view_written API re-tiles after external writes. The intent is better cache-line locality for the scattered endpoint lookups in scoring, at the cost of extra memory, extra tile/untile kernels and more complex address arithmetic.

```diff
diff --git a/include/fdcm_b200.h b/include/fdcm_b200.h
--- a/include/fdcm_b200.h
+++ b/include/fdcm_b200.h
@@ -89,6 +89,7 @@
 fdcm_status fdcm_dt3_download_mask(const fdcm_dt3* map, int32_t plane, uint8_t* dst);
 fdcm_status fdcm_dt3_scene_bins(const fdcm_dt3* map, int32_t* bins);
 fdcm_status fdcm_dt3_device_ptr(const fdcm_dt3* map, void** planes, uint64_t* n_bytes);
+fdcm_status fdcm_dt3_view_written(fdcm_dt3* map);
 
 fdcm_status fdcm_dt3_minmax_translation(const fdcm_dt3* map, const float* tmpl_xyxy, int32_t n_lines,
                                         const float align_vec[2], float out_min_max[2]);
diff --git a/openfdcm_b200/__init__.py b/openfdcm_b200/__init__.py
--- a/openfdcm_b200/__init__.py
+++ b/openfdcm_b200/__init__.py
@@ -120,6 +120,9 @@
         p, n = C.c_void_p(0), C.c_uint64(0)
         check(lib().fdcm_dt3_device_ptr(self._h, C.byref(p), C.byref(n)))
         return p.value, n.value
+
+    def view_written(self):
+        check(lib().fdcm_dt3_view_written(self._h))
 
     def rebuild(self, scene, wait=True):
         r = _records(scene)
diff --git a/openfdcm_b200/_lib.py b/openfdcm_b200/_lib.py
--- a/openfdcm_b200/_lib.py
+++ b/openfdcm_b200/_lib.py
@@ -69,6 +69,7 @@
     "fdcm_dt3_download_mask": (C.c_int, [_P, C.c_int32, _P]),
     "fdcm_dt3_scene_bins": (C.c_int, [_P, _P]),
     "fdcm_dt3_device_ptr": (C.c_int, [_P, C.POINTER(_P), C.POINTER(C.c_uint64)]),
+    "fdcm_dt3_view_written": (C.c_int, [_P]),
     "fdcm_dt3_minmax_translation": (C.c_int, [_P, _P, C.c_int32, _P, _P]),
     "fdcm_dt3_evaluate": (C.c_int, [_P, _P, _P, C.c_int32, _P, _P, _P]),
     "fdcm_dt3_classify": (C.c_int, [_P, _P, C.c_int32, _P]),
diff --git a/openfdcm_b200/csrc/common.cuh b/openfdcm_b200/csrc/common.cuh
--- a/openfdcm_b200/csrc/common.cuh
+++ b/openfdcm_b200/csrc/common.cuh
@@ -13,7 +13,15 @@
     int D, H, W, pitch;
     int wwords;
     size_t plane_elems;
+    size_t tiled_plane_elems;
 };
+
+__host__ __device__ __forceinline__ unsigned tiled_offset(unsigned pitch, unsigned x, unsigned y) {
+    return (y & ~3u) * (pitch - 8u) + ((x & ~7u) * 3u + (y * 8u + x));
+}
+__host__ __device__ __forceinline__ size_t tiled_index(const MapDims& dm, int plane, int x, int y) {
+    return (size_t)plane * dm.tiled_plane_elems + tiled_offset((unsigned)dm.pitch, (unsigned)x, (unsigned)y);
+}
 
 struct PropParams {
     int n_steps;
diff --git a/openfdcm_b200/csrc/dt3_kernels.cu b/openfdcm_b200/csrc/dt3_kernels.cu
--- a/openfdcm_b200/csrc/dt3_kernels.cu
+++ b/openfdcm_b200/csrc/dt3_kernels.cu
@@ -227,6 +227,19 @@
     for (int d = 0; d < dm.D; ++d) planes[(size_t)d * dm.plane_elems + i] = v[d];
 }
 
+__global__ void tile_kernel(const float* __restrict__ planes, float* __restrict__ tiled, MapDims dm) {
+    const int x = blockIdx.x * 32 + threadIdx.x, y = blockIdx.y * 8 + threadIdx.y, d = blockIdx.z;
+    if (x >= dm.W || y >= dm.H) return;
+    tiled[tiled_index(dm, d, x, y)] = planes[(size_t)d * dm.plane_elems + (size_t)y * dm.pitch + x];
+}
+
+__global__ void untile_kernel(const float* __restrict__ tiled, float* __restrict__ dst, MapDims dm, int plane0, size_t dst_plane,
+                              int dst_pitch) {
+    const int x = blockIdx.x * 32 + threadIdx.x, y = blockIdx.y * 8 + threadIdx.y, p = blockIdx.z;
+    if (x >= dm.W || y >= dm.H) return;
+    dst[(size_t)p * dst_plane + (size_t)y * dst_pitch + x] = tiled[tiled_index(dm, plane0 + p, x, y)];
+}
+
 static inline unsigned cdiv(size_t a, size_t b) { return (unsigned)((a + b - 1) / b); }
 
 void launch_raster(const float* d_lines, const int32_t* d_bins, int n_lines, const MapDims& dm, uint32_t* d_mask,
@@ -262,6 +275,15 @@
     sqrt_kernel<<<cdiv(total, 256), 256, 0, s>>>(d_planes, total);
 }
 
+void launch_tile(const float* d_planes, float* d_tiled, const MapDims& dm, cudaStream_t s) {
+    tile_kernel<<<dim3(cdiv(dm.W, 32), cdiv(dm.H, 8), dm.D), dim3(32, 8), 0, s>>>(d_planes, d_tiled, dm);
+}
+
+void launch_untile(const float* d_tiled, float* d_dst, const MapDims& dm, int plane0, int n_planes, size_t dst_plane, int dst_pitch,
+                   cudaStream_t s) {
+    untile_kernel<<<dim3(cdiv(dm.W, 32), cdiv(dm.H, 8), n_planes), dim3(32, 8), 0, s>>>(d_tiled, d_dst, dm, plane0, dst_plane, dst_pitch);
+}
+
 void launch_propagate(float* d_planes, const MapDims& dm, const PropParams& pp, bool sqrt_first, cudaStream_t s) {
     const unsigned grid = cdiv(dm.plane_elems, 128);
     switch (dm.D) {
diff --git a/openfdcm_b200/csrc/fdcm_api.cu b/openfdcm_b200/csrc/fdcm_api.cu
--- a/openfdcm_b200/csrc/fdcm_api.cu
+++ b/openfdcm_b200/csrc/fdcm_api.cu
@@ -239,7 +239,7 @@
     SlopeTableDev table_dev{};
     PropParams prop{};
     IntegralParams integ{};
-    DevBuf planes, mask, stack, lines, bins, band_info, band_spill, integ_items;
+    DevBuf planes, tiled, mask, stack, lines, bins, band_info, band_spill, integ_items;
     IntegralPlanDev integ_plan{};
     int plan_W = -1, plan_H = -1, plan_D = -1, plan_pitch = -1;
     const void* plan_planes = nullptr;
@@ -248,6 +248,8 @@
     cudaEvent_t ev_fork = nullptr, ev_join = nullptr;
     cudaEvent_t ev_written = nullptr;
     bool band_path = false, band_l1 = false;
+    mutable bool row_major_view = false;
+    mutable DevBuf s_download;
     mutable std::mutex search_mutex;
     mutable DevBuf s_scene, s_sorted_len, s_sorted_idx, s_hyp_off, s_rec, s_valid, s_hyp, s_counters, s_topk_score, s_topk_idx,
         s_topk_out, s_topk_n, s_keys, s_keys2, s_idx, s_perm, s_sort_tmp;
@@ -277,7 +279,7 @@
 
     ~fdcm_dt3() {
         cudaSetDevice(device);
-        for (DevBuf* b : {&planes, &mask, &stack, &lines, &bins, &band_info, &band_spill, &integ_items, &s_scene, &s_sorted_len, &s_sorted_idx, &s_hyp_off, &s_rec,
+        for (DevBuf* b : {&planes, &tiled, &s_download, &mask, &stack, &lines, &bins, &band_info, &band_spill, &integ_items, &s_scene, &s_sorted_len, &s_sorted_idx, &s_hyp_off, &s_rec,
                           &s_valid, &s_hyp, &s_counters, &s_topk_score, &s_topk_idx, &s_topk_out, &s_topk_n, &s_keys, &s_keys2, &s_idx,
                           &s_perm, &s_sort_tmp, &s_sel_keys, &s_sel_keys2, &s_sel_vals, &s_sel_vals2, &s_sel_surv, &s_sel_acc,
                           &s_sel_tmp, &s_ref_state, &s_ref_keys, &s_ref_io, &s_denom, &s_dense_keys, &s_dense_rot})
@@ -474,6 +476,7 @@
     dm.pitch = (dm.W + 31) / 32 * 32;
     dm.wwords = dm.pitch / 32;
     dm.plane_elems = (size_t)dm.H * dm.pitch;
+    dm.tiled_plane_elems = (size_t)((dm.H + 3) / 4 * 4) * dm.pitch;
     m->dm = dm;
     m->exact = 2.0 * (double)(dm.W - 1) * (double)(dm.W - 1) < 16777216.0;
 
@@ -528,6 +531,7 @@
 
     const size_t n_px = (size_t)D * dm.plane_elems;
     CUDA_TRY(m->planes.reserve(n_px * sizeof(float)));
+    CUDA_TRY(m->tiled.reserve((size_t)D * dm.tiled_plane_elems * sizeof(float)));
     CUDA_TRY(m->mask.reserve((size_t)D * dm.H * dm.wwords * sizeof(uint32_t) + 256));
     if (dt_band_smem_bytes(dm) > 200 * 1024) return fail(FDCM_ERR_INVALID, "feature size too large for the band kernels");
     const bool band_path = m->exact && m->params.distance != FDCM_L1;
@@ -549,6 +553,17 @@
     m->h_build_scene.assign(scene, scene + 4 * (size_t)n_lines);
     m->s_resident_is_build = true;
     return upload_search_scene(m, scene, n_lines, SceneFilter{false, 0, 0, 0, 0}, s);
+}
+
+static fdcm_status mirror_row_major(const fdcm_dt3* m, cudaStream_t s) {
+    if (!m->row_major_view || m->stage != 0 || m->n_lines == 0) return FDCM_OK;
+    const MapDims& dm = m->dm;
+    {
+        KernelScope k("untile", 2.0 * dm.D * dm.H * dm.W * 4.0, s);
+        launch_untile(m->tiled.as<float>(), m->planes.as<float>(), dm, 0, dm.D, dm.plane_elems, dm.pitch, s);
+    }
+    CUDA_TRY(cudaGetLastError());
+    return FDCM_OK;
 }
 
 static fdcm_status run_build_kernels(fdcm_dt3* m, cudaStream_t s) {
@@ -674,11 +689,15 @@
             KernelScope k("integral", 2 * N, s, 1);
             IntegralPlanDev pl = m->integ_plan;
             pl.counter = reinterpret_cast<int*>(m->mask.as<unsigned char>() + mask_bytes);
-            launch_integral_tma(m->planes.as<float>(), dm, m->integ, pl, m->n_sms, s);
-        }
+            launch_integral_tma(m->tiled.as<float>(), dm, m->integ, pl, m->n_sms, s);
+        }
+    }
+    if (m->stage != 0) {
+        KernelScope k("tile", 2 * N, s);
+        launch_tile(m->planes.as<float>(), m->tiled.as<float>(), dm, s);
     }
     CUDA_TRY(cudaGetLastError());
-    return FDCM_OK;
+    return mirror_row_major(m, s);
 }
 
 static fdcm_status validate_params(const fdcm_dt3_params* p) {
@@ -836,9 +855,11 @@
     if (fdcm_status st = get_stream(m->device, &s)) return st;
     std::lock_guard<std::mutex> lk(m->search_mutex);
     if (fdcm_status st = map_wait(m, s)) return st;
-    const float* src = m->planes.as<float>() + (size_t)plane * m->dm.plane_elems;
-    CUDA_TRY(cudaMemcpy2DAsync(dst, (size_t)m->dm.W * 4, src, (size_t)m->dm.pitch * 4, (size_t)m->dm.W * 4, m->dm.H,
-                               cudaMemcpyDeviceToHost, s));
+    const size_t bytes = (size_t)m->dm.W * m->dm.H * sizeof(float);
+    CUDA_TRY(m->s_download.reserve(bytes));
+    launch_untile(m->tiled.as<float>(), m->s_download.as<float>(), m->dm, plane, 1, 0, m->dm.W, s);
+    CUDA_TRY(cudaGetLastError());
+    CUDA_TRY(cudaMemcpyAsync(dst, m->s_download.p, bytes, cudaMemcpyDeviceToHost, s));
     CUDA_TRY(cudaStreamSynchronize(s));
     return FDCM_OK;
 }
@@ -869,8 +890,36 @@
 
 extern "C" fdcm_status fdcm_dt3_device_ptr(const fdcm_dt3* m, void** planes, uint64_t* n_bytes) {
     if (!m || !planes) return fail(FDCM_ERR_INVALID, "null argument");
+    {
+        std::lock_guard<std::mutex> lk(m->search_mutex);
+        if (!m->row_major_view) {
+            CUDA_TRY(cudaSetDevice(m->device));
+            cudaStream_t s;
+            if (fdcm_status st = get_stream(m->device, &s)) return st;
+            if (fdcm_status st = map_wait(m, s)) return st;
+            m->row_major_view = true;
+            if (fdcm_status st = mirror_row_major(m, s)) return st;
+            if (fdcm_status st = map_written(const_cast<fdcm_dt3*>(m), s)) return st;
+        }
+    }
     *planes = m->planes.p;
     if (n_bytes) *n_bytes = (uint64_t)m->dm.D * m->dm.plane_elems * 4;
+    return FDCM_OK;
+}
+
+extern "C" fdcm_status fdcm_dt3_view_written(fdcm_dt3* m) {
+    if (!m) return fail(FDCM_ERR_INVALID, "map is null");
+    if (!m->row_major_view) return fail(FDCM_ERR_INVALID, "view_written without fdcm_dt3_device_ptr");
+    if (m->n_lines == 0) return FDCM_OK;
+    CUDA_TRY(cudaSetDevice(m->device));
+    cudaStream_t s;
+    if (fdcm_status st = get_stream(m->device, &s)) return st;
+    std::lock_guard<std::mutex> lk(m->search_mutex);
+    if (fdcm_status st = map_wait(m, s)) return st;
+    launch_tile(m->planes.as<float>(), m->tiled.as<float>(), m->dm, s);
+    CUDA_TRY(cudaGetLastError());
+    if (fdcm_status st = map_written(m, s)) return st;
+    CUDA_TRY(cudaStreamSynchronize(s));
     return FDCM_OK;
 }
 
@@ -884,7 +933,7 @@
 
 static MapView map_view(const fdcm_dt3* m) {
     MapView v;
-    v.planes = m->planes.as<float>();
+    v.planes = m->tiled.as<float>();
     v.dm = m->dm;
     v.shift_x = m->shift[0];
     v.shift_y = m->shift[1];
@@ -2034,9 +2083,10 @@
     if (st == FDCM_OK) st = prepare_and_upload(m, scene_xyxy, n_lines, s);
     if (st == FDCM_OK && comm->rank == root) st = run_build_kernels(m, s);
     if (st == FDCM_OK && n_lines > 0) {
-        const size_t bytes = (size_t)m->dm.D * m->dm.plane_elems * sizeof(float);
-        ncclResult_t r = nccl_api().Broadcast(m->planes.p, m->planes.p, bytes, ncclChar, root, comm->comm, s);
+        const size_t bytes = (size_t)m->dm.D * m->dm.tiled_plane_elems * sizeof(float);
+        ncclResult_t r = nccl_api().Broadcast(m->tiled.p, m->tiled.p, bytes, ncclChar, root, comm->comm, s);
         if (r != ncclSuccess) st = fail(FDCM_ERR_CUDA, std::string("ncclBroadcast: ") + nccl_api().GetErrorString(r));
+        if (st == FDCM_OK && comm->rank != root) st = mirror_row_major(m, s);
     }
     if (st == FDCM_OK) st = upload_build_scene(m, scene_xyxy, n_lines, s);
     if (st == FDCM_OK) st = map_written(m, s);
diff --git a/openfdcm_b200/csrc/integral_tma.cu b/openfdcm_b200/csrc/integral_tma.cu
--- a/openfdcm_b200/csrc/integral_tma.cu
+++ b/openfdcm_b200/csrc/integral_tma.cu
@@ -23,7 +23,7 @@
 
 __global__ void __launch_bounds__(kIThreads, 4)
 integral_tma_kernel(const __grid_constant__ CUtensorMap map_y, const __grid_constant__ CUtensorMap map_x,
-                    float* __restrict__ planes, MapDims dm, const __grid_constant__ IntegralParams ip,
+                    float* __restrict__ tiled, MapDims dm, const __grid_constant__ IntegralParams ip,
                     const int4* __restrict__ items, int n_items,
                     int* __restrict__ counter) {
     extern __shared__ __align__(128) float stages[];
@@ -59,7 +59,8 @@
         const int mode = ip.mode[d];
         const float rslope = mode == 1 ? ip.ry[d] : ip.rx[d];
         auto R = [&](int i) { return (int)roundf((float)i * rslope); };
-        float* P = planes + (size_t)d * dm.plane_elems;
+        float* P = tiled + (size_t)d * dm.tiled_plane_elems;
+        const unsigned pitch = (unsigned)dm.pitch;
         const int n_major = mode == 1 ? dm.W : dm.H;
         const int nblk = b_hi - b_lo;
 
@@ -102,41 +103,40 @@
                 const int Ra = __shfl_sync(0xffffffffu, Rl, 0), Rb = __shfl_sync(0xffffffffu, Rl, nk - 1);
                 const int Rmin = min(Ra, Rb);
                 const float* tile = stages + (size_t)st * kIStageFloats + tid - Rmin + ((c0 + Rmin) & 3);
-                const int ystep = rev ? -dm.pitch : dm.pitch;
-                float* row = P + (long long)(rev ? dm.H - 1 - i0 : i0) * dm.pitch + c;
+                const unsigned rowl = tiled_offset(pitch, 0u, (unsigned)(rev ? dm.H - 1 - i0 - lane : i0 + lane));
                 const int tstep = rev ? -kIYBoxW : kIYBoxW;
                 tile += rev ? (kIRB - 1) * kIYBoxW : 0;
                 const bool inside = (unsigned)(c + Ra) < (unsigned)dm.W && (unsigned)(c + Rb) < (unsigned)dm.W;
                 const bool fast = __all_sync(0xffffffffu, inside && have);
                 mbar_wait_backoff(full0 + 8u * st, ph, 40);
                 uint32_t ta = smem_u32(tile);
-                asm volatile("" : "+r"(ta), "+l"(row));
-                __builtin_assume(__isGlobal(row));
+                asm volatile("" : "+r"(ta));
+                __builtin_assume(__isGlobal(P));
                 const int tsb = rev ? -kIYBoxW * 4 : kIYBoxW * 4;
                 constexpr int kHalf = kIRB / 2;
                 if (fast && nk == kIRB) {
 #pragma unroll
                     for (int k0 = 0; k0 < kIRB; k0 += kHalf) {
                         float v[kHalf];
-                        int go[kHalf];
+                        unsigned go[kHalf];
 #pragma unroll
                         for (int i = 0; i < kHalf; ++i) {
                             const int k = k0 + i;
                             const int Rk = __shfl_sync(0xffffffffu, Rl, k);
                             v[i] = lds_f32(ta + (uint32_t)(Rk << 2) + (uint32_t)(k * tsb));
-                            go[i] = k * ystep + Rk;
+                            go[i] = __shfl_sync(0xffffffffu, rowl, k) + tiled_offset(pitch, (unsigned)(c + Rk), 0u);
                         }
 #pragma unroll
                         for (int i = 0; i < kHalf; ++i) {
                             acc = v[i] + acc;
-                            row[go[i]] = acc;
+                            P[go[i]] = acc;
                         }
                     }
                 } else {
 #pragma unroll
                     for (int k0 = 0; k0 < kIRB; k0 += kHalf) {
                         float v[kHalf];
-                        int go[kHalf];
+                        unsigned go[kHalf];
                         unsigned in = 0u;
 #pragma unroll
                         for (int i = 0; i < kHalf; ++i) {
@@ -145,7 +145,7 @@
                             const bool ok = k < nk && (unsigned)(c + Rk) < (unsigned)dm.W;
                             v[i] = 0.f;
                             if (ok) v[i] = lds_f32(ta + (uint32_t)(Rk << 2) + (uint32_t)(k * tsb));
-                            go[i] = k * ystep + Rk;
+                            go[i] = __shfl_sync(0xffffffffu, rowl, k) + tiled_offset(pitch, (unsigned)(c + Rk), 0u);
                             in |= ok ? 1u << i : 0u;
                         }
 #pragma unroll
@@ -153,7 +153,7 @@
                             const bool ok = (in >> i) & 1u;
                             const bool st_ok = ok && have;
                             acc = st_ok ? v[i] + acc : (ok ? v[i] : acc);
-                            if (st_ok) row[go[i]] = acc;
+                            if (ok) P[go[i]] = acc;
                             if (k0 + i < nk) have = ok;
                         }
                     }
@@ -274,7 +274,7 @@
                     {
                         constexpr int kG = 4;
                         const int r0 = full_lo + warp * 4 + sub;
-                        float* g4 = P + (long long)(ybase + r0) * dm.pitch + xb + 4 * l8;
+                        const unsigned x4 = (unsigned)(xb + 4 * l8);
 #pragma unroll
                         for (int h = 0; h < kICW / (kIConsumerWarps * 4 * kG); ++h) {
                             float4 v[kG];
@@ -286,11 +286,10 @@
 #pragma unroll
                             for (int i = 0; i < kG; ++i) {
                                 const int r = r0 + (h * kG + i) * kIConsumerWarps * 4;
-                                if (r < full_hi) *reinterpret_cast<float4*>(g4 + (h * kG + i) * kIConsumerWarps * 4 * dm.pitch) = v[i];
-                            }
-                        }
-                    }
-                    float* gcol = P + (long long)ybase * dm.pitch + x;
+                                if (r < full_hi) *reinterpret_cast<float4*>(P + tiled_offset(pitch, x4, (unsigned)(ybase + r))) = v[i];
+                            }
+                        }
+                    }
 #pragma unroll
                     for (int part = 0; part < 2; ++part) {
                         constexpr int kR = kIRB / kIConsumerWarps;
@@ -304,15 +303,15 @@
 #pragma unroll
                         for (int i = 0; i < kR; ++i) {
                             const int r = rb + i * kIConsumerWarps;
-                            if (r < re && (unsigned)(r - off_m) < (unsigned)kICW) gcol[r * dm.pitch] = w[i];
+                            if (r < re && (unsigned)(r - off_m) < (unsigned)kICW) P[tiled_offset(pitch, (unsigned)x, (unsigned)(ybase + r))] = w[i];
                         }
                     }
                 } else {
-                    float* gp = P + (long long)(ybase + warp) * dm.pitch + x;
                     const float* tp = tile + warp * kIXBoxW + lane + xoff;
 #pragma unroll 4
-                    for (int r = warp; r < kIXBoxH; r += kIConsumerWarps, gp += (size_t)kIConsumerWarps * dm.pitch, tp += kIConsumerWarps * kIXBoxW)
-                        if (col_ok && (unsigned)(r - off_m) < (unsigned)kICW && (unsigned)(ybase + r) < (unsigned)dm.H) *gp = *tp;
+                    for (int r = warp; r < kIXBoxH; r += kIConsumerWarps, tp += kIConsumerWarps * kIXBoxW)
+                        if (col_ok && (unsigned)(r - off_m) < (unsigned)kICW && (unsigned)(ybase + r) < (unsigned)dm.H)
+                            P[tiled_offset(pitch, (unsigned)x, (unsigned)(ybase + r))] = *tp;
                 }
                 fence_proxy_async();
                 __syncwarp();
@@ -331,7 +330,7 @@
            encode_planes_map(map_x, planes, dm.W, dm.H, dm.D, dm.pitch, kIXBoxW, kIXBoxH, 1);
 }
 
-void launch_integral_tma(float* d_planes, const MapDims& dm, const IntegralParams& ip, const IntegralPlanDev& plan, int n_sms,
+void launch_integral_tma(float* d_tiled, const MapDims& dm, const IntegralParams& ip, const IntegralPlanDev& plan, int n_sms,
                          cudaStream_t s) {
     if (plan.n_items <= 0) return;
     const size_t smem = integral_tma_smem_bytes();
@@ -339,7 +338,7 @@
     int per_sm = 2;
     if (cudaOccupancyMaxActiveBlocksPerMultiprocessor(&per_sm, integral_tma_kernel, kIThreads, smem) != cudaSuccess || per_sm < 1) per_sm = 2;
     const int grid = plan.n_items < per_sm * n_sms ? plan.n_items : per_sm * n_sms;
-    integral_tma_kernel<<<grid, kIThreads, smem, s>>>(plan.map_y, plan.map_x, d_planes, dm, ip, plan.items4,
+    integral_tma_kernel<<<grid, kIThreads, smem, s>>>(plan.map_y, plan.map_x, d_tiled, dm, ip, plan.items4,
                                                       plan.n_items, plan.counter);
 }
 
diff --git a/openfdcm_b200/csrc/kernels.h b/openfdcm_b200/csrc/kernels.h
--- a/openfdcm_b200/csrc/kernels.h
+++ b/openfdcm_b200/csrc/kernels.h
@@ -12,6 +12,9 @@
 void launch_transpose_square(float* d_planes, const MapDims& dm, cudaStream_t s);
 void launch_sqrt(float* d_planes, const MapDims& dm, cudaStream_t s);
 void launch_propagate(float* d_planes, const MapDims& dm, const PropParams& pp, bool sqrt_first, cudaStream_t s);
+void launch_tile(const float* d_planes, float* d_tiled, const MapDims& dm, cudaStream_t s);
+void launch_untile(const float* d_tiled, float* d_dst, const MapDims& dm, int plane0, int n_planes, size_t dst_plane, int dst_pitch,
+                   cudaStream_t s);
 
 struct IntegralPlanDev {
     const int4* items4;
@@ -23,7 +26,7 @@
 int integral_strip_chains();
 int integral_tile_steps();
 bool integral_tma_encode(const void* planes, const MapDims& dm, CUtensorMap* map_y, CUtensorMap* map_x);
-void launch_integral_tma(float* d_planes, const MapDims& dm, const IntegralParams& ip, const IntegralPlanDev& plan, int n_sms,
+void launch_integral_tma(float* d_tiled, const MapDims& dm, const IntegralParams& ip, const IntegralPlanDev& plan, int n_sms,
                          cudaStream_t s);
 
 int dt_band_count(const MapDims& dm);
diff --git a/openfdcm_b200/csrc/search_kernels.cu b/openfdcm_b200/csrc/search_kernels.cu
--- a/openfdcm_b200/csrc/search_kernels.cu
+++ b/openfdcm_b200/csrc/search_kernels.cu
@@ -239,7 +239,7 @@
         if (isfinite(min_mul) && isfinite(max_mul)) {
             const float* planes = map.planes;
             const unsigned pitch = (unsigned)map.dm.pitch;
-            const unsigned last = (unsigned)(map.dm.plane_elems - 1);
+            const unsigned last = (unsigned)(map.dm.tiled_plane_elems - 1);
             const int maxm = (int)min(max(trunc_ll(max_mul), -70000LL), 70000LL), minm = (int)min(max(trunc_ll(min_mul), -70000LL), 70000LL);
             auto score_of = [&](int mult) -> float {
                 const float m = (float)mult;
@@ -247,8 +247,9 @@
                 return eigen_sum_lazy(L, [&](int i) {
                     const float4 a = apts[i];
                     const int x1 = (int)(a.x + offx), y1 = (int)(a.y + offy), x2 = (int)(a.z + offx), y2 = (int)(a.w + offy);
-                    const unsigned i1 = min((unsigned)y1 * pitch + (unsigned)x1, last), i2 = min((unsigned)y2 * pitch + (unsigned)x2, last);
-                    const float* P = planes + (size_t)bins[i] * map.dm.plane_elems;
+                    const unsigned i1 = min(tiled_offset(pitch, (unsigned)x1, (unsigned)y1), last);
+                    const unsigned i2 = min(tiled_offset(pitch, (unsigned)x2, (unsigned)y2), last);
+                    const float* P = planes + (size_t)bins[i] * map.dm.tiled_plane_elems;
                     return fabsf(__ldg(P + i1) - __ldg(P + i2));
                 });
             };
@@ -743,13 +744,10 @@
 }
 
 __device__ __forceinline__ float staged_score(const MapView& map, const float4* apts, const uint8_t* bins, int L, float offx, float offy) {
-    const float* planes = map.planes;
-    const size_t pitch = (size_t)map.dm.pitch, pe = map.dm.plane_elems;
     return eigen_sum_lazy(L, [&](int q) {
         const float4 e = apts[q];
         const int x1 = (int)(e.x + offx), y1 = (int)(e.y + offy), x2 = (int)(e.z + offx), y2 = (int)(e.w + offy);
-        const float* P = planes + (size_t)bins[q] * pe;
-        return fabsf(__ldg(P + (size_t)y1 * pitch + x1) - __ldg(P + (size_t)y2 * pitch + x2));
+        return fabsf(__ldg(map.planes + tiled_index(map.dm, bins[q], x1, y1)) - __ldg(map.planes + tiled_index(map.dm, bins[q], x2, y2)));
     });
 }
 
@@ -996,8 +994,7 @@
         int x1 = (int)(p.x + offx), y1 = (int)(p.y + offy), x2 = (int)(p.z + offx), y2 = (int)(p.w + offy);
         x1 = min(max(x1, 0), map.dm.W - 1); x2 = min(max(x2, 0), map.dm.W - 1);
         y1 = min(max(y1, 0), map.dm.H - 1); y2 = min(max(y2, 0), map.dm.H - 1);
-        const float* P = map.planes + (size_t)bin * map.dm.plane_elems;
-        return fabsf(__ldg(P + (size_t)y1 * map.dm.pitch + x1) - __ldg(P + (size_t)y2 * map.dm.pitch + x2));
+        return fabsf(__ldg(map.planes + tiled_index(map.dm, bin, x1, y1)) - __ldg(map.planes + tiled_index(map.dm, bin, x2, y2)));
     });
     (void)I;
 }
diff --git a/openfdcm_b200/distributed.py b/openfdcm_b200/distributed.py
--- a/openfdcm_b200/distributed.py
+++ b/openfdcm_b200/distributed.py
@@ -112,4 +112,7 @@
 
     t = torch.as_tensor(_Blob(), device=f"cuda:{featuremap.device}")
     dist.broadcast(t, src=src, group=group)
+    if dist.get_rank(group) != src:
+        torch.cuda.current_stream(t.device).synchronize()
+        featuremap.view_written()
     torch.cuda.synchronize(featuremap.device)
```

Result: faster. 1.852 million (median of 6 runs) (+1.2%).
